# abb128/april-asr

Measured on AMD Instinct MI355X. Metric: audio_seconds_per_second (concurrent 16 kHz sessions x 1/RTF), aprilv0_en-us-sized streaming RNN-T, higher is better.
Workload: dtype f32

## Files before the change

### april_asr_amd/__init__.py

```python
import ctypes as C
import math
import struct
import weakref
from enum import IntEnum
from typing import Callable, List, Sequence

import numpy as np

from . import _ffi

__all__ = ["Result", "Token", "Model", "Session", "SessionGroup", "Bias", "Lm", "lm_info", "VadEvent", "resampler_taps", "decode_host", "vad_plan", "vad_host", "vad_events_host",
           "DtmfEvent", "dtmf_plan", "dtmf_tables", "dtmf_host", "dtmf_decide_host", "dtmf_events_host",
           "ToneEvent", "tone_plan", "tone_tables", "tone_host", "tone_decide_host", "tone_events_host", "tone_name",
           "snapshot_info"]


class Result(IntEnum):
    PARTIAL_RECOGNITION = 1
    FINAL_RECOGNITION = 2
    ERROR_CANT_KEEP_UP = 3
    SILENCE = 4


class VadEvent:
# ... 350 lines not shown
        k = len(rows_list)
        opts = (_ffi.AprilxVadOptions * k)(*[_vad_options(o) for o in options])
        n = np.array([len(r) for r in rows_list], np.int32)
        fr = np.zeros(k, np.int32) if first_row is None else np.ascontiguousarray(first_row, np.int32)
        rows = np.ascontiguousarray(np.concatenate([np.asarray(r, np.float32).reshape(len(r), -1) for r in rows_list]), np.float32)
        assert rows.shape[1] == self.dims.mel
        st = (_ffi.AprilxVadState * k)(*(states if states is not None else [vad_reset_state() for _ in range(k)]))
        b = np.zeros(int(n.sum()), np.uint8); e = np.zeros(int(n.sum()), np.float32)
        rc = self._L.aprilx_run_vad(self._handle, k, C.addressof(opts), n.ctypes.data, fr.ctypes.data, rows.ctypes.data, C.addressof(st), b.ctypes.data, e.ctypes.data)
        if rc != 0:
            raise ValueError("aprilx_run_vad refused its arguments")
        cuts = np.cumsum(n)[:-1]
        return np.split(b, cuts), np.split(e, cuts), [st[i] for i in range(k)]

    def run_dtmf(self, options, frames_list, powers: bool = True):
        k = len(frames_list)
        opts = (_ffi.AprilxDtmfOptions * k)(*[_dtmf_options(o) for o in options])
        n = np.array([len(f) for f in frames_list], np.int32)
        fr = np.ascontiguousarray(np.concatenate([np.asarray(f, np.int16).reshape(len(f), -1) for f in frames_list]), np.int16)
        codes = np.zeros(int(n.sum()), np.uint8); pw = np.zeros((int(n.sum()), 9), np.float32)
        if self._L.aprilx_run_dtmf(self._handle, C.addressof(opts), k, n.ctypes.data, fr.ctypes.data, codes.ctypes.data, pw.ctypes.data if powers else None) != 0:
            raise ValueError("aprilx_run_dtmf refused its arguments")
        cuts = np.cumsum(n)[:-1]
        return np.split(codes, cuts), np.split(pw, cuts)

    def run_dtmf_decide(self, options, powers9):
        q = np.ascontiguousarray(powers9, np.float32).reshape(-1, 9)
        codes = np.zeros(len(q), np.uint8)
        if self._L.aprilx_run_dtmf_decide(self._handle, C.byref(_dtmf_options(options)), len(q), q.ctypes.data, codes.ctypes.data) != 0:
            raise ValueError("aprilx_run_dtmf_decide refused its arguments")
        return codes

    def run_tones(self, options, frames_list, powers: bool = True):
        k = len(frames_list)
        opts = (_ffi.AprilxToneOptions * k)(*[_tone_options(o) for o in options])
        n = np.array([len(f) for f in frames_list], np.int32)
        fr = np.ascontiguousarray(np.concatenate([np.asarray(f, np.int16).reshape(len(f), -1) for f in frames_list]), np.int16)
        plan = tone_plan(self.dims.sample_rate, self.dims.fft_size, max(1, self.dims.frame_shift * 1000 // self.dims.sample_rate), options[0])
        rec = np.zeros((int(n.sum()), 2), np.uint16); pw = np.zeros((int(n.sum()), plan.F + 1), np.float32)
        if self._L.aprilx_run_tones(self._handle, C.addressof(opts), k, n.ctypes.data, fr.ctypes.data, rec.ctypes.data, pw.ctypes.data if powers else None) != 0:
            raise ValueError("aprilx_run_tones refused its arguments")
        cuts = np.cumsum(n)[:-1]
        return np.split(rec, cuts), np.split(pw, cuts)

    def run_tone_decide(self, options, powers):
        q = np.ascontiguousarray(powers, np.float32)
        q = q.reshape(len(q), -1)
        rec = np.zeros((len(q), 2), np.uint16)
        if self._L.aprilx_run_tone_decide(self._handle, C.byref(_tone_options(options)), len(q), q.ctypes.data, rec.ctypes.data) != 0:
            raise ValueError("aprilx_run_tone_decide refused its arguments")
        return rec

    def tone_stats(self, device_index: int = 0):
        return self._detector_stats(self._L.aprilx_model_tone_stats, device_index)

    def _detector_stats(self, entry, device_index):
        l, f, ms = C.c_uint64(0), C.c_uint64(0), C.c_double(0)
        if entry(self._handle, device_index, C.byref(l), C.byref(f), C.byref(ms)) != 0:
            raise ValueError("no such device")
        return int(l.value), int(f.value), float(ms.value)

    def dtmf_stats(self, device_index: int = 0):
        return self._detector_stats(self._L.aprilx_model_dtmf_stats, device_index)

    def vad_stats(self, device_index: int = 0):
        return self._detector_stats(self._L.aprilx_model_vad_stats, device_index)

    def snapshot_stats(self, device_index: int = 0):
        g, s, gm, sm = C.c_uint64(0), C.c_uint64(0), C.c_double(0), C.c_double(0)
        if self._L.aprilx_model_snapshot_stats(self._handle, device_index, C.byref(g), C.byref(s), C.byref(gm), C.byref(sm)) != 0:
            raise ValueError("no such device")
        return int(g.value), int(s.value), float(gm.value), float(sm.value)

    def stats(self, device_index: int = 0):
        s = _ffi.AprilxStats()
        self._L.aprilx_model_stats(self._handle, device_index, C.byref(s))
        return s

    def ramp_stats(self, device_index: int = 0):
        h, e = C.c_uint64(0), C.c_uint64(0)
        if self._L.aprilx_model_ramp_stats(self._handle, device_index, C.byref(h), C.byref(e)) != 0:
            raise ValueError("aprilx_model_ramp_stats refused the call")
        return int(h.value), int(e.value)

    def feed_latencies(self, device_index: int = 0, reset: bool = False) -> np.ndarray:
        n = int(self._L.aprilx_model_feed_latency(self._handle, device_index, None, 0, 0))
        out = np.zeros(n, np.float64)
        if n:
            n = int(self._L.aprilx_model_feed_latency(self._handle, device_index, out.ctypes.data, n, 1 if reset else 0))
        elif reset:
            self._L.aprilx_model_feed_latency(self._handle, device_index, None, 0, 1)
        return out[:n]

    def profile(self, enable):
        self._L.aprilx_model_profile(self._handle, int(enable))


BIAS_STRICT = 1


class Bias:

    def __init__(self, model: Model, phrases, boost: float = 2.0, flags: int = 0):
        self._L = model._L
        items = [(p, boost) if isinstance(p, (str, bytes)) else (p[0], p[1]) for p in phrases]
        raw = [p.encode("utf-8") if isinstance(p, str) else bytes(p) for p, _ in items]
        arr = (C.c_char_p * max(len(raw), 1))(*raw)
        boosts = (C.c_float * max(len(raw), 1))(*[float(b) for _, b in items])
        err = C.create_string_buffer(256)
        self._handle = self._L.aprilx_bias_create_ex(model._handle, len(raw), arr, boosts, int(flags), err, 256)
        self.message = err.value.decode("utf-8", "replace")
        if not self._handle:
            raise ValueError("bias set refused: " + self.message)
        st, ed = C.c_int32(0), C.c_int64(0)
        self.dropped = int(self._L.aprilx_bias_info(self._handle, C.byref(st), C.byref(ed)))
        self.states, self.n_edges = int(st.value), int(ed.value)
        self.flags = int(self._L.aprilx_bias_flags(self._handle))
        self.strict = bool(self.flags & BIAS_STRICT)

    def edges(self, state: int):
        n = int(self._L.aprilx_bias_edges(self._handle, int(state), None, None, None, 0))
        if n < 0:
            raise ValueError("no state %d" % state)
        tok = np.zeros(n, np.int32); nxt = np.zeros(n, np.int32); bonus = np.zeros(n, np.float32)
        if n:
            assert self._L.aprilx_bias_edges(self._handle, int(state), tok.ctypes.data, nxt.ctypes.data, bonus.ctypes.data, n) == n
        return tok, nxt, bonus

    def csr(self):
        parts = [self.edges(s) for s in range(self.states)]
        off = np.zeros(self.states + 1, np.int32)
        off[1:] = np.cumsum([p[0].size for p in parts])
        return (off,) + tuple(np.concatenate([p[i] for p in parts]) if parts else np.zeros(0) for i in range(3))

    def close(self):
        if getattr(self, "_handle", None):
            self._L.aprilx_bias_free(self._handle)
            self._handle = None

    def __del__(self):
        try:
            self.close()
        except Exception:
            pass


class Lm:

    def __init__(self, model: Model, text, order: int = 5):
        self._L = model._L
        raw = text.encode("utf-8") if isinstance(text, str) else bytes(text)
        err = C.create_string_buffer(256)
        self._handle = self._L.aprilx_lm_create(model._handle, raw, len(raw), int(order), err, 256)
        self.message = err.value.decode("utf-8", "replace")
        if not self._handle:
            raise ValueError("language model refused: " + self.message)
        for k, v in lm_info(self).items():
            setattr(self, k, v)

    def arrays(self):
        nn, na = self.nodes, self.arcs
        d = dict(node_off=np.zeros(nn + 1, np.int32), back=np.zeros(nn, np.int32), bow=np.zeros(nn, np.float32),
                 arc_byte=np.zeros(na, np.uint8), arc_logp=np.zeros(na, np.float32), arc_next=np.zeros(na, np.int32))
        unk = C.c_float(0)
        rc = self._L.aprilx_lm_arrays(self._handle, *[d[k].ctypes.data for k in ("node_off", "back", "bow", "arc_byte", "arc_logp", "arc_next")], C.byref(unk), nn, na)
        assert rc == 0
# ... 647 lines not shown
```

### april_asr_amd/_ffi.py

```python
import ctypes as C
import os

_HERE = os.path.dirname(os.path.abspath(__file__))
LIB_PATH = os.environ.get("APRIL_ASR_LIB") or os.path.join(_HERE, "libaprilasr.so")


class AprilSpeakerID(C.Structure):
    _fields_ = [("data", C.c_uint8 * 16)]


class AprilToken(C.Structure):
    _fields_ = [("token", C.c_char_p), ("logprob", C.c_float), ("flags", C.c_int),
                ("time_ms", C.c_size_t), ("reserved", C.c_void_p)]


HANDLER = C.CFUNCTYPE(None, C.c_void_p, C.c_int, C.c_size_t, C.POINTER(AprilToken))


class AprilConfig(C.Structure):
    _fields_ = [("speaker", AprilSpeakerID), ("handler", HANDLER), ("userdata", C.c_void_p), ("flags", C.c_int)]


class AprilxDims(C.Structure):
    _fields_ = [(n, C.c_int32) for n in ("n_layers", "d_model", "hidden", "ffn", "joiner", "vocab", "mel", "seg",
# ... 50 lines not shown
VAD_HANDLER = C.CFUNCTYPE(None, C.c_void_p, C.c_int, C.c_uint64)


class AprilxDtmfOptions(C.Structure):
    _fields_ = [("size", C.c_uint32), ("min_level_dbfs", C.c_float), ("twist_hi_db", C.c_float), ("twist_lo_db", C.c_float), ("rel_peak_db", C.c_float),
                ("min_share", C.c_float), ("min_tone_ms", C.c_uint32), ("min_pause_ms", C.c_uint32), ("flags", C.c_uint32)]


class AprilxDtmfInfo(C.Structure):
    _fields_ = [("Wd", C.c_int32), ("on_frames", C.c_int32), ("off_frames", C.c_int32), ("held", C.c_uint32),
                ("frames_seen", C.c_uint64), ("tone_frames", C.c_uint64), ("digits", C.c_uint64)]


class AprilxDtmfPlan(C.Structure):
    _fields_ = [("Wd", C.c_int32), ("half_w", C.c_float), ("min_power", C.c_float), ("twist_hi", C.c_float), ("twist_lo", C.c_float),
                ("rel_peak", C.c_float), ("min_share", C.c_float), ("on_frames", C.c_int32), ("off_frames", C.c_int32), ("reserved", C.c_int32)]


class AprilxDtmfMachine(C.Structure):
    _fields_ = [("held", C.c_int32), ("cand", C.c_int32), ("run", C.c_int32)]


DTMF_HANDLER = C.CFUNCTYPE(None, C.c_void_p, C.c_int, C.c_char, C.c_uint64)


class AprilxToneOptions(C.Structure):
    _fields_ = [("size", C.c_uint32), ("min_level_dbfs", C.c_float), ("second_db", C.c_float), ("min_share", C.c_float), ("tol_hz", C.c_uint32),
                ("min_tone_ms", C.c_uint32), ("min_pause_ms", C.c_uint32), ("flags", C.c_uint32)]


class AprilxToneInfo(C.Structure):
    _fields_ = [("W", C.c_int32), ("k_lo", C.c_int32), ("F", C.c_int32), ("on_frames", C.c_int32), ("off_frames", C.c_int32),
                ("held_f1", C.c_uint32), ("held_f2", C.c_uint32), ("reserved", C.c_uint32),
                ("frames_seen", C.c_uint64), ("tonal_frames", C.c_uint64), ("tones", C.c_uint64)]


class AprilxTonePlan(C.Structure):
    _fields_ = [("W", C.c_int32), ("k_lo", C.c_int32), ("F", C.c_int32), ("half_w", C.c_float), ("min_power", C.c_float), ("second_ratio", C.c_float),
                ("min_share", C.c_float), ("bin_hz", C.c_float), ("tol_hz", C.c_int32), ("on_frames", C.c_int32), ("off_frames", C.c_int32),
                ("reserved", C.c_int32)]


class AprilxToneMachine(C.Structure):
    _fields_ = [("held", C.c_int32), ("h1", C.c_int32), ("h2", C.c_int32), ("c1", C.c_int32), ("c2", C.c_int32), ("run", C.c_int32)]


TONE_HANDLER = C.CFUNCTYPE(None, C.c_void_p, C.c_int, C.c_uint32, C.c_uint32, C.c_uint64)


class AprilxInputFormat(C.Structure):
    _fields_ = [("size", C.c_uint32), ("encoding", C.c_uint32), ("channels", C.c_uint32), ("channel", C.c_int32)]


class AprilxSnapshotInfo(C.Structure):
    _fields_ = ([("size", C.c_uint32), ("version", C.c_uint32), ("blob_size", C.c_uint64), ("params_hash", C.c_uint64), ("token_hash", C.c_uint64),
                 ("bias_hash", C.c_uint64), ("bias_edges", C.c_int64), ("chunks", C.c_uint64), ("frames_seen", C.c_uint64), ("now_ms", C.c_uint64),
                 ("rows_written", C.c_uint64)]
                + [(n, C.c_int32) for n in ("n_layers", "d_model", "hidden", "ffn", "joiner", "vocab", "mel", "segment_size", "segment_step", "sample_rate",
                                            "frame_shift_ms", "blank_id")]
                + [(n, C.c_uint32) for n in ("precision", "f16_tile", "input_rate", "confidence_k", "has_format", "has_search_options", "has_vad", "has_dtmf",
                                             "has_tones", "has_bias", "bias_flags")]
                + [("bias_states", C.c_int32), ("ring_rows", C.c_uint32), ("reserved", C.c_uint32), ("format", AprilxInputFormat), ("search", AprilxSearchOptions),
                   ("vad", AprilxVadOptions), ("dtmf", AprilxDtmfOptions), ("tones", AprilxToneOptions), ("name", C.c_char * 64), ("description", C.c_char * 128)])


EXPORTED_REFERENCE_SYMBOLS = [
    "aam_api_init", "aam_create_model", "aam_get_name", "aam_get_description", "aam_get_language",
    "aam_get_sample_rate", "aam_free", "aas_create_session", "aas_feed_pcm16", "aas_flush",
    "aas_realtime_get_speedup", "aas_free",
]
EXPORTED_ENGINE_SYMBOLS = [
    "aprilx_model_dims", "aprilx_model_token", "aprilx_model_blob_size", "aprilx_model_export_blob",
    "aprilx_model_from_blob", "aprilx_model_save_blob", "aprilx_model_save_blob_f16", "aprilx_model_load_blob",
    "aprilx_broadcast_get_id", "aprilx_model_broadcast", "aprilx_model_load_info", "aprilx_feed_many", "aprilx_flush_many", "aprilx_session_drain", "aprilx_feed_many_pipelined", "aprilx_drain_many",
    "aprilx_run_encoder", "aprilx_run_decoder", "aprilx_run_joiner", "aprilx_run_fbank", "aprilx_run_decide", "aprilx_plan_gemm", "aprilx_gemm_plan_debug", "aprilx_run_gemm", "aprilx_stream_form",
    "aprilx_session_trace_logits", "aprilx_session_chunks", "aprilx_session_read_frames", "aprilx_session_context", "aprilx_model_stats", "aprilx_model_profile", "aprilx_model_feed_latency",
    "aprilx_greedy_create", "aprilx_greedy_step", "aprilx_greedy_finish", "aprilx_greedy_free", "aprilx_probe_file", "aprilx_model_load_host", "aprilx_model_fbank_tables", "aprilx_counting_handler",
    "aprilx_session_set_input_rate", "aprilx_session_input_rate", "aprilx_resampler_taps", "aprilx_resample",
    "aprilx_session_set_confidence", "aprilx_session_confidence", "aprilx_run_confidence",
    "aprilx_bias_create", "aprilx_bias_free", "aprilx_bias_info", "aprilx_bias_edges", "aprilx_session_set_bias", "aprilx_session_bias_state",
    "aprilx_run_decide_biased", "aprilx_greedy_set_bias", "aprilx_greedy_bias_state",
    "aprilx_bias_create_ex", "aprilx_bias_flags", "aprilx_run_confidence_biased",
    "aprilx_session_set_search_options", "aprilx_session_search_options", "aprilx_run_decide_opts", "aprilx_greedy_set_search_options",
    "aprilx_ramp_window", "aprilx_model_ramp_stats",
    "aprilx_session_set_input_format", "aprilx_session_input_format", "aprilx_session_feed_bytes", "aprilx_feed_many_bytes",
    "aprilx_decode_host", "aprilx_decode", "aprilx_model_decode_stats",
    "aprilx_session_set_vad", "aprilx_session_vad", "aprilx_vad_plan_tables", "aprilx_vad_host", "aprilx_vad_events_host", "aprilx_run_vad",
    "aprilx_model_vad_stats",
    "aprilx_session_set_dtmf", "aprilx_session_dtmf", "aprilx_dtmf_plan", "aprilx_dtmf_tables", "aprilx_dtmf_host", "aprilx_dtmf_decide_host",
    "aprilx_dtmf_events_host", "aprilx_run_dtmf", "aprilx_run_dtmf_decide", "aprilx_model_dtmf_stats",
    "aprilx_session_set_tones", "aprilx_session_tones", "aprilx_tone_plan", "aprilx_tone_tables", "aprilx_tone_host", "aprilx_tone_decide_host",
    "aprilx_tone_events_host", "aprilx_tone_name", "aprilx_run_tones", "aprilx_run_tone_decide", "aprilx_model_tone_stats",
    "aprilx_session_snapshot", "aprilx_session_restore", "aprilx_snapshot_info", "aprilx_snapshot_many", "aprilx_restore_many", "aprilx_model_snapshot_stats",
    "aprilx_lm_create", "aprilx_lm_free", "aprilx_lm_info", "aprilx_lm_arrays", "aprilx_lm_score_host", "aprilx_session_set_lm", "aprilx_session_lm_state",
    "aprilx_greedy_set_lm", "aprilx_greedy_lm_state", "aprilx_model_lm_stats", "aprilx_run_decide_lm", "aprilx_run_confidence_lm",
]

_lib = None
_inited = False


def lib():
    global _lib
    if _lib is not None:
        return _lib
    if not os.path.exists(LIB_PATH):
        raise ImportError("libaprilasr.so is not built: run `python -c 'import __graft_entry__ as g; g.build()'` "
                          "or `make -C april_asr_amd/csrc` (hipcc, gfx950). There is no CPU fallback.")
    L = C.CDLL(LIB_PATH)
    vp, sz = C.c_void_p, C.c_size_t
    L.aam_api_init.argtypes = [C.c_int]; L.aam_api_init.restype = None
    L.aam_create_model.argtypes = [C.c_char_p]; L.aam_create_model.restype = vp
    for f in ("aam_get_name", "aam_get_description", "aam_get_language"):
        getattr(L, f).argtypes = [vp]; getattr(L, f).restype = C.c_char_p
    L.aam_get_sample_rate.argtypes = [vp]; L.aam_get_sample_rate.restype = sz
    L.aam_free.argtypes = [vp]; L.aam_free.restype = None
    L.aas_create_session.argtypes = [vp, AprilConfig]; L.aas_create_session.restype = vp
    L.aas_feed_pcm16.argtypes = [vp, vp, sz]; L.aas_feed_pcm16.restype = None
    L.aas_flush.argtypes = [vp]; L.aas_flush.restype = None
    L.aas_realtime_get_speedup.argtypes = [vp]; L.aas_realtime_get_speedup.restype = C.c_float
    L.aas_free.argtypes = [vp]; L.aas_free.restype = None
    L.aprilx_model_dims.argtypes = [vp, C.POINTER(AprilxDims)]; L.aprilx_model_dims.restype = C.c_int
    L.aprilx_model_token.argtypes = [vp, C.c_int32]; L.aprilx_model_token.restype = C.c_char_p
    L.aprilx_model_blob_size.argtypes = [vp]; L.aprilx_model_blob_size.restype = sz
    L.aprilx_model_export_blob.argtypes = [vp, vp, sz]; L.aprilx_model_export_blob.restype = C.c_int
    L.aprilx_model_from_blob.argtypes = [vp, sz, C.c_int]; L.aprilx_model_from_blob.restype = vp
    L.aprilx_model_save_blob.argtypes = [vp, C.c_char_p]; L.aprilx_model_save_blob.restype = C.c_int
    L.aprilx_model_save_blob_f16.argtypes = [vp, C.c_char_p]; L.aprilx_model_save_blob_f16.restype = C.c_int
    L.aprilx_model_load_blob.argtypes = [C.c_char_p]; L.aprilx_model_load_blob.restype = vp
    L.aprilx_broadcast_get_id.argtypes = [vp, sz]; L.aprilx_broadcast_get_id.restype = C.c_int
    L.aprilx_model_broadcast.argtypes = [vp, C.c_int, C.c_int, vp]; L.aprilx_model_broadcast.restype = vp
    L.aprilx_model_load_info.argtypes = [vp, C.POINTER(AprilxLoadInfo)]; L.aprilx_model_load_info.restype = C.c_int
    L.aprilx_feed_many.argtypes = [sz, C.POINTER(vp), C.POINTER(vp), C.POINTER(sz)]; L.aprilx_feed_many.restype = None
    L.aprilx_flush_many.argtypes = [sz, C.POINTER(vp)]; L.aprilx_flush_many.restype = None
    L.aprilx_session_drain.argtypes = [vp]; L.aprilx_session_drain.restype = None
    L.aprilx_feed_many_pipelined.argtypes = [sz, C.POINTER(vp), C.POINTER(vp), C.POINTER(sz), C.c_int]; L.aprilx_feed_many_pipelined.restype = None
    L.aprilx_drain_many.argtypes = [sz, C.POINTER(vp)]; L.aprilx_drain_many.restype = None
    L.aprilx_run_encoder.argtypes = [vp, C.c_int] + [vp] * 6; L.aprilx_run_encoder.restype = C.c_int
    L.aprilx_run_decoder.argtypes = [vp, C.c_int, vp, vp]; L.aprilx_run_decoder.restype = C.c_int
    L.aprilx_run_joiner.argtypes = [vp, C.c_int, vp, vp, vp]; L.aprilx_run_joiner.restype = C.c_int
    L.aprilx_run_fbank.argtypes = [vp, C.c_int, vp, vp]; L.aprilx_run_fbank.restype = C.c_int
    L.aprilx_plan_gemm.argtypes = [C.c_int] * 6 + [vp]; L.aprilx_plan_gemm.restype = C.c_int
    L.aprilx_gemm_plan_debug.argtypes = [vp, vp]; L.aprilx_gemm_plan_debug.restype = C.c_int
    L.aprilx_run_gemm.argtypes = [vp] * 5; L.aprilx_run_gemm.restype = C.c_int
    L.aprilx_ramp_window.argtypes = [C.c_int] * 3 + [vp, C.c_int]; L.aprilx_ramp_window.restype = C.c_int
    L.aprilx_model_ramp_stats.argtypes = [vp, C.c_int, C.POINTER(C.c_uint64), C.POINTER(C.c_uint64)]; L.aprilx_model_ramp_stats.restype = C.c_int
    L.aprilx_stream_form.argtypes = [C.c_int] * 6; L.aprilx_stream_form.restype = C.c_int
    L.aprilx_run_decide.argtypes = [vp, C.c_int, C.c_int, vp, C.c_float, vp, C.c_int, vp, vp]; L.aprilx_run_decide.restype = C.c_int
    L.aprilx_session_trace_logits.argtypes = [vp, vp, sz, C.POINTER(sz)]; L.aprilx_session_trace_logits.restype = None
    L.aprilx_session_chunks.argtypes = [vp]; L.aprilx_session_chunks.restype = C.c_uint64
    L.aprilx_session_read_frames.argtypes = [vp, C.c_uint64, C.c_int, C.c_void_p]; L.aprilx_session_read_frames.restype = C.c_uint64
    L.aprilx_session_context.argtypes = [vp, vp, vp]; L.aprilx_session_context.restype = None
    L.aprilx_model_stats.argtypes = [vp, C.c_int, C.POINTER(AprilxStats)]; L.aprilx_model_stats.restype = None
    L.aprilx_model_feed_latency.argtypes = [vp, C.c_int, vp, C.c_int, C.c_int]; L.aprilx_model_feed_latency.restype = C.c_int
    L.aprilx_model_profile.argtypes = [vp, C.c_int]; L.aprilx_model_profile.restype = None
    L.aprilx_greedy_create.argtypes = [vp, HANDLER, vp]; L.aprilx_greedy_create.restype = vp
    L.aprilx_greedy_step.argtypes = [vp, C.c_int32, C.c_float, C.c_float, C.c_float, sz, C.POINTER(C.c_int32)]
    L.aprilx_greedy_step.restype = C.c_int
    L.aprilx_greedy_finish.argtypes = [vp]; L.aprilx_greedy_finish.restype = None
    L.aprilx_greedy_free.argtypes = [vp]; L.aprilx_greedy_free.restype = None
    L.aprilx_model_load_host.argtypes = [C.c_char_p]; L.aprilx_model_load_host.restype = vp
    L.aprilx_model_fbank_tables.argtypes = [vp, vp, vp]; L.aprilx_model_fbank_tables.restype = C.c_int
    L.aprilx_probe_file.argtypes = [C.c_char_p, C.c_char_p, sz]; L.aprilx_probe_file.restype = C.c_int
    L.aprilx_session_set_input_rate.argtypes = [vp, C.c_uint32]; L.aprilx_session_set_input_rate.restype = C.c_int
    L.aprilx_session_input_rate.argtypes = [vp]; L.aprilx_session_input_rate.restype = C.c_uint32
    L.aprilx_resampler_taps.argtypes = [C.c_uint32, C.c_uint32, vp, vp, sz]; L.aprilx_resampler_taps.restype = C.c_int
    L.aprilx_resample.argtypes = [vp, C.c_uint32, vp, sz, vp, sz]; L.aprilx_resample.restype = C.c_int64
    L.aprilx_session_set_confidence.argtypes = [vp, C.c_int]; L.aprilx_session_set_confidence.restype = C.c_int
    L.aprilx_session_confidence.argtypes = [vp]; L.aprilx_session_confidence.restype = C.c_int
    L.aprilx_run_confidence.argtypes = [vp, C.c_int, vp, C.c_int, vp]; L.aprilx_run_confidence.restype = C.c_int
    L.aprilx_bias_create.argtypes = [vp, sz, C.POINTER(C.c_char_p), C.POINTER(C.c_float), C.c_char_p, sz]; L.aprilx_bias_create.restype = vp
    L.aprilx_bias_create_ex.argtypes = [vp, sz, C.POINTER(C.c_char_p), C.POINTER(C.c_float), C.c_uint32, C.c_char_p, sz]; L.aprilx_bias_create_ex.restype = vp
    L.aprilx_bias_flags.argtypes = [vp]; L.aprilx_bias_flags.restype = C.c_int
    L.aprilx_run_confidence_biased.argtypes = [vp, C.c_int, vp, C.c_int, vp, vp, vp]; L.aprilx_run_confidence_biased.restype = C.c_int
    L.aprilx_bias_free.argtypes = [vp]; L.aprilx_bias_free.restype = None
    L.aprilx_lm_create.argtypes = [vp, vp, sz, C.c_int, C.c_char_p, sz]; L.aprilx_lm_create.restype = vp
    L.aprilx_lm_free.argtypes = [vp]; L.aprilx_lm_free.restype = None
    L.aprilx_lm_info.argtypes = [vp, C.POINTER(C.c_int32), C.POINTER(C.c_int32), C.POINTER(C.c_int64), C.POINTER(C.c_int32), C.POINTER(C.c_int32)]; L.aprilx_lm_info.restype = C.c_int
    L.aprilx_lm_arrays.argtypes = [vp] * 7 + [C.POINTER(C.c_float), sz, sz]; L.aprilx_lm_arrays.restype = C.c_int
    L.aprilx_lm_score_host.argtypes = [vp, C.c_int32, C.c_int32, C.POINTER(C.c_float), C.POINTER(C.c_int32)]; L.aprilx_lm_score_host.restype = C.c_int
    L.aprilx_session_set_lm.argtypes = [vp, vp, C.c_float, C.c_float]; L.aprilx_session_set_lm.restype = C.c_int
    L.aprilx_session_lm_state.argtypes = [vp, C.POINTER(C.c_int32), C.POINTER(C.c_int32)]; L.aprilx_session_lm_state.restype = C.c_int
    L.aprilx_greedy_set_lm.argtypes = [vp, vp, C.c_float, C.c_float]; L.aprilx_greedy_set_lm.restype = C.c_int
    L.aprilx_greedy_lm_state.argtypes = [vp]; L.aprilx_greedy_lm_state.restype = C.c_int
    L.aprilx_model_lm_stats.argtypes = [vp, C.c_int, C.POINTER(C.c_uint64), C.POINTER(C.c_int32), C.POINTER(C.c_uint64)]; L.aprilx_model_lm_stats.restype = C.c_int
    L.aprilx_run_decide_lm.argtypes = [vp, C.c_int, C.c_int, vp, C.c_float, vp, C.c_int, vp, vp, vp, vp, vp, vp, vp, C.c_float, C.c_float]; L.aprilx_run_decide_lm.restype = C.c_int
    L.aprilx_run_confidence_lm.argtypes = [vp, C.c_int, vp, C.c_int, vp, vp, vp, vp, C.c_float, C.c_float, vp]; L.aprilx_run_confidence_lm.restype = C.c_int
    L.aprilx_bias_info.argtypes = [vp, C.POINTER(C.c_int32), C.POINTER(C.c_int64)]; L.aprilx_bias_info.restype = C.c_int
    L.aprilx_bias_edges.argtypes = [vp, C.c_int32, vp, vp, vp, sz]; L.aprilx_bias_edges.restype = C.c_int
    L.aprilx_session_set_bias.argtypes = [vp, vp]; L.aprilx_session_set_bias.restype = C.c_int
    L.aprilx_session_bias_state.argtypes = [vp, C.POINTER(C.c_int32), C.POINTER(C.c_int32)]; L.aprilx_session_bias_state.restype = C.c_int
    L.aprilx_run_decide_biased.argtypes = [vp, C.c_int, C.c_int, vp, C.c_float, vp, C.c_int, vp, vp, vp, vp]; L.aprilx_run_decide_biased.restype = C.c_int
    L.aprilx_greedy_set_bias.argtypes = [vp, vp]; L.aprilx_greedy_set_bias.restype = C.c_int
    L.aprilx_greedy_bias_state.argtypes = [vp]; L.aprilx_greedy_bias_state.restype = C.c_int
    L.aprilx_session_set_search_options.argtypes = [vp, C.POINTER(AprilxSearchOptions)]; L.aprilx_session_set_search_options.restype = C.c_int
    L.aprilx_session_search_options.argtypes = [vp, C.POINTER(AprilxSearchOptions)]; L.aprilx_session_search_options.restype = C.c_int
    L.aprilx_run_decide_opts.argtypes = [vp, C.c_int, C.c_int, vp, C.c_float, vp, C.c_int, vp, vp, vp, vp, vp]; L.aprilx_run_decide_opts.restype = C.c_int
    L.aprilx_greedy_set_search_options.argtypes = [vp, C.POINTER(AprilxSearchOptions)]; L.aprilx_greedy_set_search_options.restype = C.c_int
    L.aprilx_session_set_input_format.argtypes = [vp, C.POINTER(AprilxInputFormat)]; L.aprilx_session_set_input_format.restype = C.c_int
    L.aprilx_session_input_format.argtypes = [vp, C.POINTER(AprilxInputFormat)]; L.aprilx_session_input_format.restype = C.c_int
    L.aprilx_session_feed_bytes.argtypes = [vp, vp, sz]; L.aprilx_session_feed_bytes.restype = C.c_int
    L.aprilx_feed_many_bytes.argtypes = [sz, C.POINTER(vp), C.POINTER(vp), C.POINTER(sz), C.c_int]; L.aprilx_feed_many_bytes.restype = C.c_int
    L.aprilx_decode_host.argtypes = [C.POINTER(AprilxInputFormat), vp, sz, vp, sz]; L.aprilx_decode_host.restype = C.c_int64
    L.aprilx_decode.argtypes = [vp, C.POINTER(AprilxInputFormat), vp, sz, vp, sz]; L.aprilx_decode.restype = C.c_int64
    L.aprilx_model_decode_stats.argtypes = [vp, C.c_int, C.POINTER(C.c_uint64), C.POINTER(C.c_uint64), C.POINTER(C.c_double)]; L.aprilx_model_decode_stats.restype = C.c_int
    L.aprilx_session_set_vad.argtypes = [vp, C.POINTER(AprilxVadOptions), VAD_HANDLER, vp]; L.aprilx_session_set_vad.restype = C.c_int
    L.aprilx_session_vad.argtypes = [vp, C.POINTER(AprilxVadOptions), C.POINTER(AprilxVadInfo)]; L.aprilx_session_vad.restype = C.c_int
    L.aprilx_vad_plan_tables.argtypes = [vp, C.c_int, C.c_int, C.c_int, C.c_int, C.POINTER(AprilxVadOptions), C.POINTER(AprilxVadPlan)]; L.aprilx_vad_plan_tables.restype = C.c_int
    L.aprilx_vad_host.argtypes = [C.POINTER(AprilxVadPlan), C.c_int, C.c_int, vp, C.POINTER(AprilxVadState), vp, vp]; L.aprilx_vad_host.restype = C.c_int
    L.aprilx_vad_events_host.argtypes = [C.POINTER(AprilxVadPlan), C.c_int, C.c_uint64, vp, sz, C.POINTER(C.c_int32), vp, vp, C.c_int]; L.aprilx_vad_events_host.restype = C.c_int
    L.aprilx_run_vad.argtypes = [vp, C.c_int, vp, vp, vp, vp, vp, vp, vp]; L.aprilx_run_vad.restype = C.c_int
    L.aprilx_model_vad_stats.argtypes = [vp, C.c_int, C.POINTER(C.c_uint64), C.POINTER(C.c_uint64), C.POINTER(C.c_double)]; L.aprilx_model_vad_stats.restype = C.c_int
    L.aprilx_session_set_dtmf.argtypes = [vp, C.POINTER(AprilxDtmfOptions), DTMF_HANDLER, vp]; L.aprilx_session_set_dtmf.restype = C.c_int
    L.aprilx_session_dtmf.argtypes = [vp, C.POINTER(AprilxDtmfOptions), C.POINTER(AprilxDtmfInfo)]; L.aprilx_session_dtmf.restype = C.c_int
    L.aprilx_dtmf_plan.argtypes = [C.c_int, C.c_int, C.c_int, C.POINTER(AprilxDtmfOptions), C.POINTER(AprilxDtmfPlan)]; L.aprilx_dtmf_plan.restype = C.c_int
    L.aprilx_dtmf_tables.argtypes = [C.c_int, C.c_int, vp, sz]; L.aprilx_dtmf_tables.restype = C.c_int
    L.aprilx_dtmf_host.argtypes = [C.POINTER(AprilxDtmfPlan), vp, C.c_int, vp, sz, vp, vp]; L.aprilx_dtmf_host.restype = C.c_int
    L.aprilx_dtmf_decide_host.argtypes = [C.POINTER(AprilxDtmfPlan), vp]; L.aprilx_dtmf_decide_host.restype = C.c_int
    L.aprilx_dtmf_events_host.argtypes = [C.POINTER(AprilxDtmfPlan), C.c_int, C.c_uint64, vp, sz, C.c_int, C.POINTER(AprilxDtmfMachine), vp, vp, vp, C.c_int]
    L.aprilx_dtmf_events_host.restype = C.c_int
    L.aprilx_run_dtmf.argtypes = [vp, vp, C.c_int, vp, vp, vp, vp]; L.aprilx_run_dtmf.restype = C.c_int
    L.aprilx_run_dtmf_decide.argtypes = [vp, C.POINTER(AprilxDtmfOptions), C.c_int, vp, vp]; L.aprilx_run_dtmf_decide.restype = C.c_int
    L.aprilx_model_dtmf_stats.argtypes = [vp, C.c_int, C.POINTER(C.c_uint64), C.POINTER(C.c_uint64), C.POINTER(C.c_double)]; L.aprilx_model_dtmf_stats.restype = C.c_int
    L.aprilx_session_set_tones.argtypes = [vp, C.POINTER(AprilxToneOptions), TONE_HANDLER, vp]; L.aprilx_session_set_tones.restype = C.c_int
    L.aprilx_session_tones.argtypes = [vp, C.POINTER(AprilxToneOptions), C.POINTER(AprilxToneInfo)]; L.aprilx_session_tones.restype = C.c_int
    L.aprilx_tone_plan.argtypes = [C.c_int, C.c_int, C.c_int, C.POINTER(AprilxToneOptions), C.POINTER(AprilxTonePlan)]; L.aprilx_tone_plan.restype = C.c_int
    L.aprilx_tone_tables.argtypes = [C.c_int, C.c_int, vp, sz]; L.aprilx_tone_tables.restype = C.c_int
    L.aprilx_tone_host.argtypes = [C.POINTER(AprilxTonePlan), vp, C.c_int, vp, sz, vp, vp]; L.aprilx_tone_host.restype = C.c_int
    L.aprilx_tone_decide_host.argtypes = [C.POINTER(AprilxTonePlan), vp]; L.aprilx_tone_decide_host.restype = C.c_int64
# ... 25 lines not shown
```

### april_asr_amd/csrc/engine.cc

```cpp
#include "engine.h"
#include <array>
#include <algorithm>
#include <cmath>
#include <chrono>
#include <cstdlib>
#include <cstring>
#include "common.h"
#include "env.h"
#include "rowepi_forms.h"

namespace aprilx {

static size_t align64(size_t x) { return (x + 63) & ~(size_t)63; }

void plan_layout(const NetDims &d, bool has_dec_conv_b, PackedLayout &L)
{
    L.dims = d;
    L.has_dec_conv_b = has_dec_conv_b;
    L.vocab_pad = (d.vocab + 31) & ~31;
    size_t off = 0;
    auto take = [&](size_t n) { size_t o = off; off = align64(off + n); return o; };
    L.k3 = (d.conv_ch[1] * 9 + 63) & ~63;
    L.conv_w[0] = take((size_t)d.conv_ch[0] * 9); L.conv_b[0] = take((size_t)d.conv_ch[0]);
    L.conv_w[1] = take((size_t)d.conv_ch[1] * d.conv_ch[0] * 9); L.conv_b[1] = take((size_t)d.conv_ch[1]);
    L.conv_w[2] = take((size_t)L.k3 * d.conv_ch[2]); L.conv_b[2] = take((size_t)d.conv_ch[2]);
    L.w_embed = take((size_t)d.embed_in * d.d_model); L.b_embed = take((size_t)d.d_model);
    L.layers.resize((size_t)d.n_layers);
    for (auto &l : L.layers) {
        l.wg = take((size_t)2 * d.d_model * 4 * d.hidden); l.bg = take((size_t)4 * d.hidden);
        l.whr = take((size_t)d.hidden * d.d_model);
        l.wff1 = take((size_t)d.d_model * d.ffn); l.bff1 = take((size_t)d.ffn);
        l.wff2 = take((size_t)d.ffn * d.d_model); l.bff2 = take((size_t)d.d_model);
    }
    L.w_encproj = take((size_t)d.d_model * d.joiner); L.b_encproj = take((size_t)d.joiner);
    L.emb = take((size_t)d.vocab * d.d_model);
    L.dec_conv = take((size_t)d.d_model * (d.d_model / d.dec_groups) * d.context);
    L.dec_conv_b = take((size_t)d.d_model);
    L.w_decproj = take((size_t)d.d_model * d.joiner); L.b_decproj = take((size_t)d.joiner);
    L.w_out = take((size_t)d.joiner * L.vocab_pad); L.b_out = take((size_t)L.vocab_pad);
    L.total = off;
}

std::vector<std::pair<size_t, size_t>> gemm_sections(const PackedLayout &L)
{
    const NetDims &d = L.dims;
    std::vector<std::pair<size_t, size_t>> v;
    v.emplace_back(L.w_embed, (size_t)d.embed_in * d.d_model);
    for (const PackedLayout::Layer &o : L.layers) {
        v.emplace_back(o.wg, (size_t)2 * d.d_model * 4 * d.hidden); v.emplace_back(o.whr, (size_t)d.hidden * d.d_model);
        v.emplace_back(o.wff1, (size_t)d.d_model * d.ffn); v.emplace_back(o.wff2, (size_t)d.ffn * d.d_model);
    }
    v.emplace_back(L.w_encproj, (size_t)d.d_model * d.joiner); v.emplace_back(L.w_decproj, (size_t)d.d_model * d.joiner);
    v.emplace_back(L.w_out, (size_t)d.joiner * L.vocab_pad);
    return v;
}

static void pack_mfma(const float *W, int K, int N, int Npad, const std::vector<int> *colmap, float *dst)
{
    const int KB = K / 16, NTt = Npad / 16;
    for (int t = 0; t < NTt; ++t)
        for (int kb = 0; kb < KB; ++kb)
            for (int lane = 0; lane < 64; ++lane) {
                const int np = t * 16 + (lane & 15);
                const int src = np < N ? (colmap ? (*colmap)[(size_t)np] : np) : -1;
                float *o = dst + (((size_t)t * KB + kb) * 64 + lane) * 4;
                for (int j = 0; j < 4; ++j) {
                    const int k = kb * 16 + (lane >> 4) * 4 + j;
                    o[j] = src >= 0 ? W[(size_t)k * N + src] : 0.0f;
                }
            }
}

void pack_weights(const HostModel &m, PackedLayout &L, std::vector<float> &blob)
{
    const NetDims &d = L.dims;
    blob.assign(L.total, 0.0f);
    float *B = blob.data();
    for (int i = 0; i < 3; ++i) {
        if (i < 2) memcpy(B + L.conv_w[i], m.conv_w[i].data(), m.conv_w[i].size() * 4);
        memcpy(B + L.conv_b[i], m.conv_b[i].data(), m.conv_b[i].size() * 4);
    }
    {
        const int kreal = d.conv_ch[1] * 9, c2 = d.conv_ch[2];
        std::vector<float> w3((size_t)L.k3 * c2, 0.0f);
        for (int o = 0; o < c2; ++o) for (int k = 0; k < kreal; ++k) w3[(size_t)k * c2 + o] = m.conv_w[2][(size_t)o * kreal + k];
        pack_mfma(w3.data(), L.k3, c2, c2, nullptr, B + L.conv_w[2]);
    }
    {
        const int c2 = d.conv_ch[2], F = d.f_out;
// ... 88 lines not shown
    HIP_CHECK(hipStreamCreateWithFlags(&s_stream_, hipStreamNonBlocking));
    search_stream_ = stream_;
    for (int i = 0; i < 32; ++i) { hipEvent_t e; HIP_CHECK(hipEventCreateWithFlags(&e, hipEventDisableTiming)); join_ev_.push_back(e); }
    split_streams_ = std::max(0, std::min(2, env_int("APRIL_SPLIT_STREAMS", 2)));
    const NetDims &d = L_.dims;
    w_ = dmalloc<float>(L_.total);
    if (blob_device) HIP_CHECK(hipMemcpy(w_, blob_device, L_.total * 4, hipMemcpyDeviceToDevice));
    else if (blob_host) HIP_CHECK(hipMemcpy(w_, blob_host, L_.total * 4, hipMemcpyHostToDevice));

    const size_t S = (size_t)cfg_.max_slots, MB = (size_t)cfg_.max_batch;
    ring_frames_ = std::max(P_.segment_size * 32, env_int("APRIL_RING_FRAMES", 8192));
    h_ = dmalloc<float>((size_t)d.n_layers * S * d.d_model);
    c_ = dmalloc<float>((size_t)d.n_layers * S * d.hidden);
    if (!env_str("APRIL_RING_FRAMES")) {
        size_t free_b = 0, total_b = 0;
        if (hipMemGetInfo(&free_b, &total_b) == hipSuccess && free_b > 0) {
            const size_t per_frame = S * (size_t)d.mel * sizeof(float);
            const size_t fit = (free_b / 4) / per_frame;
            if (fit < (size_t)ring_frames_) {
                const int shrunk = std::max(P_.segment_size * 32, (int)std::min<size_t>(fit, 8192) / 64 * 64);
                LOGW("engine: %zu MB of feature rings (%d frames x %zu slots) exceed a quarter of the %zu MB free on device %d: %d frames per session",
                     per_frame * (size_t)ring_frames_ >> 20, ring_frames_, S, free_b >> 20, cfg_.device, shrunk);
                ring_frames_ = shrunk;
            }
        } else (void)hipGetLastError();
        float *p = nullptr;
        if (hipMalloc((void **)&p, S * ring_frames_ * d.mel * sizeof(float)) == hipSuccess) ring_ = p;
        else {
            (void)hipGetLastError();
            const size_t asked = S * (size_t)ring_frames_ * d.mel * sizeof(float);
            ring_frames_ = std::max(P_.segment_size * 32, 2048);
            LOGW("engine: no room for %zu MB of feature rings, falling back to %d frames per session", asked >> 20, ring_frames_);
        }
    }
    if (!ring_) ring_ = dmalloc<float>(S * ring_frames_ * d.mel);
    eout_ = dmalloc<float>(S * d.joiner);
    dout_ = dmalloc<float>(S * d.joiner);
    gstate_ = dmalloc<GreedyState>(S);
    HIP_CHECK(hipMemset(h_, 0, (size_t)d.n_layers * S * d.d_model * 4));
    HIP_CHECK(hipMemset(c_, 0, (size_t)d.n_layers * S * d.hidden * 4));
    HIP_CHECK(hipMemset(ring_, 0, S * ring_frames_ * d.mel * 4));
    HIP_CHECK(hipMemset(eout_, 0, S * d.joiner * 4));
    HIP_CHECK(hipMemset(dout_, 0, S * d.joiner * 4));
    {
        std::vector<GreedyState> init(S);
        for (auto &g : init) { g.ctx0 = P_.blank_id; g.ctx1 = P_.blank_id; g.last_tok = -1; g.last_emit_ms = 0; }
        HIP_CHECK(hipMemcpy(gstate_, init.data(), S * sizeof(GreedyState), hipMemcpyHostToDevice));
    }
    cls_ = dmalloc<uint8_t>((size_t)d.vocab);
    HIP_CHECK(hipMemcpy(cls_, tok_class.data(), (size_t)d.vocab, hipMemcpyHostToDevice));

    kz_embed_ = pick_kz(d.embed_in, d.d_model);
    kz_hr_ = pick_kz(d.hidden, d.d_model);
    kz_ff2_ = pick_kz(d.ffn, d.d_model);
    kz_proj_ = pick_kz(d.d_model, d.joiner);
    kz_out_ = pick_kz(d.joiner, L_.vocab_pad);
    {
        const bool want = cfg_.precision == 1 && env_int("APRIL_F16_TILE", 1) != 0;
        f16_tile_ = want && d.d_model % 128 == 0 && d.hidden % 128 == 0 && d.ffn % 128 == 0 && d.hidden % 16 == 0;
        if (f16_tile_) {
            kzx_hr_ = pick_kz(d.hidden, d.d_model, 32); kzx_ff2_ = pick_kz(d.ffn, d.d_model, 32);
            for (int p = 0; p < 2; ++p) y16_buf_[p] = dmalloc<uint16_t>(MB * d.d_model);
            y16_ = y16_buf_[0];
            for (int p = 0; p < 2; ++p) { xb16_buf_[p] = dmalloc<uint16_t>(MB * d.d_model); u16_buf_[p] = dmalloc<uint16_t>(MB * d.hidden); ff16_buf_[p] = dmalloc<uint16_t>(MB * d.ffn); }
            xb16_ = xb16_buf_[0]; u16_ = u16_buf_[0]; ff16_ = ff16_buf_[0];
            h16_ = dmalloc<uint16_t>((size_t)d.n_layers * S * d.d_model);
            HIP_CHECK(hipMemset(h16_, 0, (size_t)d.n_layers * S * d.d_model * 2));
        }
    }
    ws_mstride_ = cfg_.max_batch;
    const size_t ws_n = (size_t)std::max({kz_embed_ * d.d_model, kz_hr_ * d.d_model, kz_ff2_ * d.d_model, kz_proj_ * d.joiner, kz_out_ * L_.vocab_pad});
    ws_ = dmalloc<float>(ws_n * MB);
    ws_g_ = dmalloc<float>((size_t)std::max(kz_proj_ * d.joiner, kz_out_ * L_.vocab_pad) * MB);
    xin_ = dmalloc<float>(MB * d.embed_in);
    a3_ = dmalloc<float>(MB * d.f_out * L_.k3);
    HIP_CHECK(hipMemset(a3_, 0, MB * d.f_out * L_.k3 * 4));
    for (int p = 0; p < 2; ++p) { y_buf_[p] = dmalloc<float>(MB * d.d_model); ssq_buf_[p] = dmalloc<float>(MB * (d.d_model / SSQ_COLS)); }
    y_ = y_buf_[0]; ssq_ = ssq_buf_[0];
    ws_fe_ = dmalloc<float>((size_t)kz_embed_ * d.d_model * MB);
    ws_sr_ = dmalloc<float>((size_t)std::max(kz_proj_ * d.joiner, d.d_model) * MB);
    for (int p = 0; p < 2; ++p) { xb_buf_[p] = dmalloc<float>(MB * d.d_model); u_buf_[p] = dmalloc<float>(MB * d.hidden); ff_buf_[p] = dmalloc<float>(MB * d.ffn); }
    xb_ = xb_buf_[0]; u_ = u_buf_[0]; ff_ = ff_buf_[0];
    ramp_mode_ = env_int("APRIL_RAMP_MERGE", 1);
    if (ramp_mode_ < 0 || ramp_mode_ > 2) ramp_mode_ = 1;
    ramp_d_ = dmalloc<RampState>(1); HIP_CHECK(hipMemset(ramp_d_, 0, sizeof(RampState)));
    de_ = dmalloc<float>(MB * d.d_model);
    HIP_CHECK(hipMemset(de_, 0, MB * d.d_model * 4));
    logits_ = dmalloc<float>(3 * MB * d.vocab);
    logits_h_ = hmalloc<float>(3 * MB * d.vocab);
    ring_cap_ = std::max<size_t>((size_t)1 << 20, 3 * MB * 8 + 2 * S); ring_h_ = hmalloc<int>(2 * ring_cap_);
    step_cap_ = 1 << 14; step_off_h_ = hmalloc<int>((size_t)2 * step_cap_); rec_off_h_ = hmalloc<int>((size_t)2 * step_cap_);
    rec_cap_ = std::max<size_t>((size_t)1 << 20, 3 * MB * 8); rec_d_ = dmalloc<StepRecord>(2 * rec_cap_); rec_h_ = hmalloc<StepRecord>(2 * rec_cap_);
    for (int i = 0; i < 2; ++i) HIP_CHECK(hipEventCreateWithFlags(&flight_done_[i], hipEventDisableTiming));
    counter_d_ = dmalloc<int>(1);
    for (int p = 0; p < 2; ++p) {
        rec_off_buf_[p] = dmalloc<int>(1); flags_buf_[p] = dmalloc<int>(8); step_buf_[p] = dmalloc<int>(4 * MB);
        HIP_CHECK(hipMemset(rec_off_buf_[p], 0, 4)); HIP_CHECK(hipMemset(flags_buf_[p], 0, 32));
    }
    rec_off_d_ = rec_off_buf_[0]; flags_d_ = flags_buf_[0]; step_d_ = step_buf_[0];
    active_d_ = dmalloc<int>(MB); dirty_d_ = dmalloc<int>(MB);
    dec_slots_d_ = dmalloc<int>(std::max(S, MB));
    HIP_CHECK(hipMemset(counter_d_, 0, 4));

    upload_tables(ft);
    use_graphs_ = env_int("APRIL_NO_GRAPHS", 0) == 0;
    if (const int n = env_int("APRIL_GRAPH_CACHE_CAP", 0))
        step_graphs_.cap = lm_graphs_.cap = lm_search_graphs_.cap = sw_plan_cap_ = (size_t)std::max(n, 2), sw_graphs_.cap = 4 * sw_plan_cap_;
    free_.reserve(S);
    for (int i = cfg_.max_slots - 1; i >= 0; --i) free_.push_back(i);
    LOGI("engine: device %d, %d slots, max batch %d, weights %.1f MB, kz(embed,hr,ff2,proj,out)=%d,%d,%d,%d,%d",
         cfg_.device, cfg_.max_slots, cfg_.max_batch, L_.total * 4.0 / 1e6, kz_embed_, kz_hr_, kz_ff2_, kz_proj_, kz_out_);
}

void Engine::finish_weights()
{
    HipLegacyLock legacy;
    HIP_CHECK(hipSetDevice(cfg_.device));
    if (cfg_.precision == 1 && !wh_) {
        wh_ = dmalloc<uint16_t>(L_.total);
        for (const auto &sec : gemm_sections(L_)) launch_cvt_f16(w_ + sec.first, wh_ + sec.first, sec.second, nullptr);
        if (f16_tile_) {
            const NetDims &d = L_.dims;
            wx_ = dmalloc<uint16_t>(L_.total);
            for (const PackedLayout::Layer &o : L_.layers) {
                launch_repack_x32(w_ + o.wg, wx_ + o.wg, 2 * d.d_model, 4 * d.hidden, nullptr);
                launch_repack_x32(w_ + o.whr, wx_ + o.whr, d.hidden, d.d_model, nullptr);
                launch_repack_x32(w_ + o.wff1, wx_ + o.wff1, d.d_model, d.ffn, nullptr);
                launch_repack_x32(w_ + o.wff2, wx_ + o.wff2, d.ffn, d.d_model, nullptr);
            }
        }
        HIP_CHECK(hipDeviceSynchronize());
    }
    if (!conv_wt_) {
        const NetDims &d = L_.dims;
        conv_wt_ = dmalloc<float>((size_t)9 * d.conv_ch[0] + (size_t)9 * d.conv_ch[0] * d.conv_ch[1]);
        launch_conv_weight_transpose(w_ + L_.conv_w[0], w_ + L_.conv_w[1], d.conv_ch[0], d.conv_ch[1], conv_wt_, conv_wt_ + (size_t)9 * d.conv_ch[0], nullptr);
        HIP_CHECK(hipDeviceSynchronize());
    }
    build_dec_table();
}

void Engine::build_dec_table()
{
    if (dec_table_) return;
    const NetDims &d = L_.dims;
    const size_t limit_mb = (size_t)std::max(0, env_int("APRIL_DEC_TABLE_MB", 2048));
    const size_t rows = (size_t)d.vocab * (size_t)d.vocab;
    if (d.context != 2 || rows * (size_t)d.joiner * 4 > limit_mb * 1024 * 1024 || rows * (size_t)d.joiner * 4 >= ((size_t)1 << 32)) return;
    const int MB = cfg_.max_batch;
    float *table = dmalloc<float>(rows * (size_t)d.joiner);
    std::vector<int> iota((size_t)MB), ctx((size_t)MB * 2);
    for (int i = 0; i < MB; ++i) iota[(size_t)i] = i;
    int *ctx_d = dmalloc<int>((size_t)MB * 2);
    HIP_CHECK(hipMemcpy(dec_slots_d_, iota.data(), (size_t)MB * 4, hipMemcpyHostToDevice));
    for (size_t base = 0; base < rows; base += (size_t)MB) {
        const int n = (int)std::min<size_t>((size_t)MB, rows - base);
        for (int i = 0; i < n; ++i) { const size_t r = base + (size_t)i; ctx[(size_t)2 * i] = (int)(r / (size_t)d.vocab); ctx[(size_t)2 * i + 1] = (int)(r % (size_t)d.vocab); }
        HIP_CHECK(hipMemcpy(ctx_d, ctx.data(), (size_t)n * 8, hipMemcpyHostToDevice));
        DecEmbedArgs a; a.dec = dec_params(); a.ctx = ctx_d; a.M = n; a.out = de_; a.ldo = d.d_model;
        launch_dec_embed(a, stream_);
        run_decproj(n, dec_slots_d_, nullptr, nullptr, 1, table + base * (size_t)d.joiner);
        HIP_CHECK(hipStreamSynchronize(stream_));
    }
    (void)hipFree(ctx_d);
    dec_table_ = table;
    LOGI("engine: decoder table %zu rows x %d (%.0f MB)", rows, d.joiner, rows * (double)d.joiner * 4 / 1e6);
}

Engine::~Engine()
{
    HipLegacyLock legacy;
    (void)hipSetDevice(cfg_.device);
    (void)hipStreamSynchronize(f_stream_); (void)hipStreamSynchronize(stream_); (void)hipStreamSynchronize(s_stream_);
    dump_stream_trace();
    if (ramp_d_ && ramp_eligible_.load() > 0) {
        unsigned h = 0;
        if (hipMemcpy(&h, &ramp_d_->hosted, sizeof h, hipMemcpyDeviceToHost) == hipSuccess) LOGI("engine: ramp merge: %u of %llu hostable split feeds were hosted by their predecessor", h, (unsigned long long)ramp_eligible_.load());
    }
    for (StreamTrace &t : trace_) for (hipEvent_t e : t.ev) if (e) (void)hipEventDestroy(e);
    if (trace_base_) (void)hipEventDestroy(trace_base_);
    for (hipEvent_t e : join_ev_) (void)hipEventDestroy(e);
    for (auto &e : ev_pool_) { (void)hipEventDestroy(e.a); (void)hipEventDestroy(e.b); }
    drop_graphs(); free_sw_plans(); if (gclk_slots_) (void)hipFree(gclk_slots_);
    if (lm_stream_) { (void)hipStreamSynchronize(lm_stream_); (void)hipStreamDestroy(lm_stream_); }
    for (hipEvent_t e : lm_events_) (void)hipEventDestroy(e);
    if (zargs_h_) { (void)hipHostFree(zargs_h_); (void)hipFree(zargs_d_); }
    for (int i = 0; i < 3; ++i) if (zargs_done_[i]) (void)hipEventDestroy(zargs_done_[i]);
    for (void *p : {(void *)lm_now_d_, (void *)lm_rows_d_, (void *)lm_rec_off_d_}) if (p) (void)hipFree(p);
    conf_k_.release(); bias_set_.release(); bias_desc_.release(); opt_.release();
    if (conf_d_) (void)hipFree(conf_d_);
    if (conf_h_) (void)hipHostFree(conf_h_);
    for (auto &b : bias_sets_) if (b.dev) (void)hipFree(b.dev);
    if (bias_state_d_) (void)hipFree(bias_state_d_);
    lm_slot_.release(); lm_desc_.release();
    for (auto &e : lm_models_) if (e.dev) (void)hipFree(e.dev);
    if (lm_state_d_) (void)hipFree(lm_state_d_);
    for (void *p : {(void *)vad_state_d_, (void *)pass_out_d_}) if (p) (void)hipFree(p);
    for (PassBlock &k : pass_blocks_) (void)hipHostFree(k.h);
    if (snap_d_) (void)hipFree(snap_d_);
    if (snap_h_) (void)hipHostFree(snap_h_);
    if (ws_g_) (void)hipFree(ws_g_);
    if (conv_wt_) (void)hipFree(conv_wt_);
    if (dec_table_) (void)hipFree(dec_table_);
    if (p_lm_) (void)hipFree(p_lm_);
    for (int p = 0; p < 2; ++p)
        for (void *q : {(void *)eout_lm_buf_[p], (void *)y16_buf_[p], (void *)y_buf_[p], (void *)ssq_buf_[p], (void *)xb_buf_[p], (void *)u_buf_[p], (void *)ff_buf_[p],
                        (void *)xb16_buf_[p], (void *)u16_buf_[p], (void *)ff16_buf_[p], (void *)rec_off_buf_[p], (void *)flags_buf_[p], (void *)step_buf_[p]}) if (q) (void)hipFree(q);
    if (ws_fe_) (void)hipFree(ws_fe_);
    if (ws_sr_) (void)hipFree(ws_sr_);
    for (void *p : {(void *)wx_, (void *)h16_, (void *)ramp_d_}) if (p) (void)hipFree(p);
    for (void *p : {(void *)w_, (void *)wh_, (void *)h_, (void *)c_, (void *)ring_, (void *)eout_, (void *)dout_, (void *)gstate_, (void *)cls_, (void *)ws_, (void *)xin_,
                    (void *)a3_, (void *)de_, (void *)logits_, (void *)rec_d_, (void *)counter_d_,
                    (void *)active_d_, (void *)dirty_d_, (void *)dec_slots_d_,
                    (void *)ds_pcm_[0], (void *)ds_pcm_[1]})
        if (p) (void)hipFree(p);
    for (void *p : {(void *)ring_h_, (void *)step_off_h_, (void *)rec_off_h_, (void *)rec_h_, (void *)logits_h_, (void *)hs_pcm_[0], (void *)hs_pcm_[1]})
        if (p) (void)hipHostFree(p);
    for (int b = 0; b < 2; ++b) if (fb_done_[b]) (void)hipEventDestroy(fb_done_[b]);
    for (int b = 0; b < 2; ++b) if (flight_done_[b]) (void)hipEventDestroy(flight_done_[b]);
    for (void *p : table_allocs_) (void)hipFree(p);
    (void)hipStreamDestroy(stream_); (void)hipStreamDestroy(f_stream_); (void)hipStreamDestroy(s_stream_);
}

void Engine::upload_tables(const FbankHostTables &ft)
{
    auto up = [&](const void *src, size_t bytes) {
        void *p = nullptr;
        HIP_CHECK(hipMalloc(&p, std::max<size_t>(bytes, 16)));
        if (bytes) HIP_CHECK(hipMemcpy(p, src, bytes, hipMemcpyHostToDevice));
        table_allocs_.push_back(p);
        return p;
    };
    ft_.window = (const float *)up(ft.window.data(), ft.window.size() * 4);
    ft_.mel = (const float *)up(ft.mel.data(), ft.mel.size() * 4);
    ft_.mel_lo = (const int *)up(ft.mel_lo.data(), ft.mel_lo.size() * 4);
    ft_.mel_hi = (const int *)up(ft.mel_hi.data(), ft.mel_hi.size() * 4);
    ft_.nfct = (int)ft.factors.size();
    for (int k = 0; k < ft_.nfct; ++k) {
        ft_.fct[k] = ft.factors[(size_t)k];
        ft_.tw[k] = (const double *)up(ft.tw[(size_t)k].data(), ft.tw[(size_t)k].size() * 8);
        ft_.tws[k] = ft.tws[(size_t)k].empty() ? nullptr : (const double *)up(ft.tws[(size_t)k].data(), ft.tws[(size_t)k].size() * 8);
    }
    ft_.padded = ft.padded; ft_.nbins = ft.nbins;
    pad_value_ = ft.pad_value;
}

int Engine::alloc_slot()
{
    std::lock_guard<std::mutex> g(slot_mu_);
    if (free_.empty() && !zero_pending_.empty()) zero_pending_slots();
    if (free_.empty()) return -1;
    const int s = free_.back();
    free_.pop_back();
    ++live_;
    return s;
}

void Engine::zero_pending_slots()
{
    if (zero_pending_.empty()) return;
    if (hipSetDevice(cfg_.device) == hipSuccess) {
        std::lock_guard<std::mutex> cg(capture_mu_);
        m_touched();
        const NetDims &d = L_.dims;
        for (size_t o = 0; o < zero_pending_.size(); o += 64) {
            ZeroSlotArgs z;
            z.h = h_; z.c = c_; z.n_layers = d.n_layers; z.slots = (size_t)cfg_.max_slots; z.d_model = d.d_model; z.hidden = d.hidden;
            z.eout = eout_; z.dout = dout_; z.joiner = d.joiner; z.state = gstate_; z.blank = P_.blank_id; z.h16 = h16_;
            z.n_list = (int)std::min<size_t>(64, zero_pending_.size() - o);
            for (int i = 0; i < z.n_list; ++i) z.list[i] = zero_pending_[o + (size_t)i];
            launch_zero_slot(z, stream_);
        }
    }
    for (int s : zero_pending_) free_.push_back(s);
    zero_pending_.clear();
}

void Engine::free_slot(int slot)
{
    set_slot_confidence(slot, 0); set_slot_bias(slot, nullptr); set_slot_lm(slot, nullptr, 0.0f, 0.0f); set_slot_search_options(slot, SearchOpt{0u, 0.0f});
    std::lock_guard<std::mutex> g(slot_mu_);
    zero_pending_.push_back(slot);
    --live_;
    if (zero_pending_.size() >= 256) zero_pending_slots();
}

void Engine::sync_streams()
{
    HIP_CHECK(hipStreamSynchronize(f_stream_)); HIP_CHECK(hipStreamSynchronize(stream_)); HIP_CHECK(hipStreamSynchronize(s_stream_));
}

void Engine::sync()
{
    m_touched();
    sync_streams();
    f_unseen_by_m_ = s_unseen_by_m_ = m_unseen_by_f_ = m_unseen_by_s_ = false;
    if (profiling_) collect_timing();
}

template <typename Chain> static hipGraphExec_t capture_graph(hipStream_t st, Chain &&chain)
{
    hipGraph_t graph = nullptr;
    hipGraphExec_t exec = nullptr;
    HipLegacyLock capture_guard;
    HIP_CHECK(hipStreamBeginCapture(st, hipStreamCaptureModeRelaxed));
    chain();
    HIP_CHECK(hipStreamEndCapture(st, &graph));
    HIP_CHECK(hipGraphInstantiate(&exec, graph, nullptr, nullptr, 0));
    HIP_CHECK(hipGraphDestroy(graph));
    return exec;
}

void GraphCache::clear()
{
    if (!map_.empty()) LOGI("engine: %s graphs emptied (%zu entries)", name, map_.size());
    for (auto &g : map_) (void)hipGraphExecDestroy(g.second);
    map_.clear(); uses_.clear();
}

template <typename Chain> hipGraphExec_t Engine::cached_graph(GraphCache &cache, const GraphCache::Key &key, hipStream_t st, Chain &&chain)
{
    if (!cache.find(key)) cache.insert(key, capture_graph(st, chain));
    return cache.find(key);
}

template <typename Capture> void Engine::capture_both_parities(Capture &&capture)
{
    const int par = flight_parity_;
    m_touched();
    for (int q : {1 - par, par}) { select_parity(q); capture(); }
}

Engine::StreamTrace *Engine::trace_slot()
{
    static const char *path = env_str("APRIL_STREAM_TRACE");
    if (!path) return nullptr;
    if (!trace_base_) { HIP_CHECK(hipEventCreate(&trace_base_)); HIP_CHECK(hipEventRecord(trace_base_, stream_)); }
    if (trace_.size() >= 4096) return nullptr;
    trace_.emplace_back();
    StreamTrace &t = trace_.back();
    for (hipEvent_t &e : t.ev) HIP_CHECK(hipEventCreate(&e));
    return &t;
}

void Engine::dump_stream_trace()
{
    const char *path = env_str("APRIL_STREAM_TRACE");
    if (!path || trace_.empty()) return;
    FILE *f = fopen(path, "w");
    if (!f) return;
    fprintf(f, "# one line per split feed; times in us since the first split feed; FE = index fetch + conv + embed on stream F, LY = layer wavefront on M, SR = encoder_proj + search on S\n");
    fprintf(f, "# feed sessions chunks  FE_start FE_end  LY_start LY_end  SR_start SR_end   overlap: FE inside the previous feed's LY window? SR inside the next feed's LY window?\n");
    std::vector<std::array<float, 6>> ts;
    for (StreamTrace &t : trace_) {
        std::array<float, 6> a{};
        bool ok = t.used;
        for (int i = 0; i < 6 && ok; ++i) ok = hipEventElapsedTime(&a[(size_t)i], trace_base_, t.ev[i]) == hipSuccess;
        if (ok) ts.push_back(a); else (void)hipGetLastError();
    }
    for (size_t i = 0; i < ts.size(); ++i) {
        const auto &a = ts[i];
        const bool fe_in_prev = i > 0 && a[0] * 1e3f < ts[i - 1][3] * 1e3f && a[1] * 1e3f > ts[i - 1][2] * 1e3f;
        const bool sr_in_next = i + 1 < ts.size() && a[5] > ts[i + 1][2] && a[4] < ts[i + 1][3];
        fprintf(f, "%4zu %5d %2d  %10.1f %10.1f  %10.1f %10.1f  %10.1f %10.1f   %s %s\n", i, trace_[i].m, trace_[i].T, a[0] * 1e3, a[1] * 1e3, a[2] * 1e3, a[3] * 1e3, a[4] * 1e3, a[5] * 1e3,
                fe_in_prev ? "FE<prevLY" : "-", sr_in_next ? "SR<nextLY" : "-");
    }
    fclose(f);
}

void Engine::join(hipStream_t waiter, hipStream_t src)
{
    hipEvent_t e = join_ev_[join_pos_++ % join_ev_.size()];
    HIP_CHECK(hipEventRecord(e, src));
    HIP_CHECK(hipStreamWaitEvent(waiter, e, 0));
}

void Engine::general_prologue()
{
    m_touched();
    if (f_unseen_by_m_) { join(stream_, f_stream_); f_unseen_by_m_ = false; }
    if (s_unseen_by_m_) { join(stream_, s_stream_); s_unseen_by_m_ = false; }
    m_unseen_by_f_ = m_unseen_by_s_ = true;
    flight_tail_s_ = false;
}

void Engine::set_profiling(bool on) { std::lock_guard<std::mutex> cg(capture_mu_); sync(); profiling_ = on; }
void Engine::reset_timing() { for (auto &t : timing_) t = KernelTiming(); }
void Engine::set_gates_clock(bool on)
{
    std::lock_guard<std::mutex> cg(capture_mu_);
    HIP_CHECK(hipSetDevice(cfg_.device));
    sync();
    if (on) {
        if (!gclk_slots_) gclk_slots_ = dmalloc<unsigned long long>((size_t)GCLK_SLOTS * STAMP_WORDS);
        HIP_CHECK(hipMemsetAsync(gclk_slots_, 0, (size_t)GCLK_SLOTS * STAMP_WORDS * 8, stream_));
        HIP_CHECK(hipStreamSynchronize(stream_));
        gclk_ms_ = 0; gclk_launches_ = 0; gclk_rows_ = 0;
        for (int i = 0; i < 4; ++i) { gclk_ms_n_[i] = 0; gclk_launches_n_[i] = 0; }
        gclk_ = true;
        return;
    }
    collect_gates_clock(); gclk_ = false;
}
void Engine::collect_gates_clock()
{
    if (!gclk_ || !gclk_slots_) return;
    std::vector<unsigned long long> h((size_t)GCLK_SLOTS * STAMP_WORDS);
    HIP_CHECK(hipMemcpyAsync(h.data(), gclk_slots_, h.size() * 8, hipMemcpyDeviceToHost, stream_)); HIP_CHECK(hipStreamSynchronize(stream_));
    for (auto &kv : sw_plans_)
        for (size_t i = 0; i < kv.second.stamp_slots.size(); ++i) {
            const auto &sl = kv.second.stamp_slots[i];
            const unsigned long long ticks = h[(size_t)sl.first * STAMP_WORDS + 2], n = h[(size_t)sl.first * STAMP_WORDS + 3];
            gclk_ms_ += (double)ticks * 1e-5; gclk_launches_ += (long)n; gclk_rows_ += (long)n * sl.second;
            const int bn = std::min(std::max(kv.second.stamp_n[i], 1), 4) - 1;
            gclk_ms_n_[bn] += (double)ticks * 1e-5; gclk_launches_n_[bn] += (long)n;
        }
}
void Engine::timed_begin(int cls)
{
    ++launch_count_;
    if (!profiling_) return;
    if (ev_used_ == ev_pool_.size()) { Ev e; HIP_CHECK(hipEventCreate(&e.a)); HIP_CHECK(hipEventCreate(&e.b)); e.cls = cls; ev_pool_.push_back(e); }
    ev_pool_[ev_used_].cls = cls;
    if (cls == T_GATES) gemm_profile_next_launch(ev_pool_[ev_used_].a, ev_pool_[ev_used_].b);
    else HIP_CHECK(hipEventRecord(ev_pool_[ev_used_].a, stream_));
}
void Engine::timed_end(int cls)
{
    if (!profiling_) return;
    if (cls == T_GATES) {
        if (gemm_profile_pending()) { gemm_profile_next_launch(nullptr, nullptr); return; }
    } else HIP_CHECK(hipEventRecord(ev_pool_[ev_used_].b, stream_));
    ++ev_used_;
}
void Engine::collect_timing()
{
    for (size_t i = 0; i < ev_used_; ++i) {
        float ms = 0;
        if (hipEventElapsedTime(&ms, ev_pool_[i].a, ev_pool_[i].b) == hipSuccess) { timing_[ev_pool_[i].cls].ms += ms; timing_[ev_pool_[i].cls].launches++; }
    }
    ev_used_ = 0;
}

const uint8_t *Engine::fbank(int n_frames, const FbankFrameDesc *desc, const std::pair<const int16_t *, size_t> *parts, size_t n_parts, size_t n_pcm, HostPool *pool,
                             const FrontPass &pass)
{
    if (n_frames <= 0) return nullptr;
    const int n_rs = std::max(pass.n_rs, 0), n_dc = std::max(pass.n_dc, 0), n_vd = std::max(pass.n_vd, 0), n_dt = std::max(pass.n_dt, 0);
// ... 530 lines not shown
            zargs_pos_ += items.size(); items.clear();
        };
        auto by_len = [&](auto make) {
            for (int pass = 0; pass < 2; ++pass) {
                for (const Act &x : act) if (((x.t1 - x.t0) == blk) == (pass == 0)) items.push_back(make(x));
                flush();
            }
        };
        by_len([&](const Act &x) { return args_gates(x.l, (size_t)x.t0 * m, (x.t1 - x.t0) * m, GATES_X); });
        for (int i = 0; i < blk; ++i) {
            for (const Act &x : act) if (x.t0 + i < x.t1) items.push_back(args_gates(x.l, (size_t)(x.t0 + i) * m, m, GATES_H));
            flush();
            for (const Act &x : act) if (x.t0 + i < x.t1) items.push_back(args_whr(x.l, (size_t)(x.t0 + i) * m, m));
            flush();
        }
        by_len([&](const Act &x) { return args_ff1(x.l, (size_t)x.t0 * m, (x.t1 - x.t0) * m); });
        by_len([&](const Act &x) { return args_ff2(x.l, (size_t)x.t0 * m, (x.t1 - x.t0) * m); });
        plan_end[(size_t)W] = plan.size();
    }
    lap(0);
    if (zargs_pos_ > first)
        HIP_CHECK(hipMemcpyAsync(zargs_d_ + first, zargs_h_ + first, (zargs_pos_ - first) * sizeof(GemmArgs), hipMemcpyHostToDevice, cs));
    lap(1);
    for (int W = 0; W <= NB + L; ++W) {
        if (W < NB) encoder_front((size_t)W * blk * m, (std::min(T, (W + 1) * blk) - W * blk) * m, step_d_ + 3 * MB, nullptr, cs, ws_);
        lap(2);
        for (size_t k = W ? plan_end[(size_t)W - 1] : 0; k < plan_end[(size_t)W]; ++k) launch_gemm_z(zargs_h_ + plan[k].off, plan[k].n, zargs_d_ + plan[k].off, cs);
        lap(3);
        const int bp = W - L - 1;
        if (bp >= 0) {
            const int t0 = bp * blk, t1 = std::min(T, t0 + blk), len = t1 - t0;
            lm_stage_proj(m, t0, t1, cs, ws_);
            hipEvent_t e = lm_events_[1 + (size_t)(bp % (int)(lm_events_.size() - 1))];
            HIP_CHECK(hipEventRecord(e, cs));
            HIP_CHECK(hipStreamWaitEvent(stream_, e, 0));
            BlockSetupArgs bs;
            bs.now_src = step_d_ + 2 * MB + (size_t)t0 * m; bs.now_dst = lm_now_d_; bs.rows_dst = lm_rows_d_; bs.row0 = t0 * m; bs.count = len * m;
            bs.rec_off_step = rec_off_d_; bs.rec_off_block = lm_rec_off_d_; bs.rec_add = t0 * 3 * m; bs.flags = flags_d_; bs.n_flags = 8;
            launch_block_setup(bs, stream_);
            lap(4);
            auto search = [&]() {
                for (int i = 0; i < len; ++i) {
                    GreedyIo io;
                    io.gen = i + 1; io.now = lm_now_d_ + (size_t)i * m; io.eout = eout_lm_; io.eout_rows = lm_rows_d_ + (size_t)i * m;
                    io.rec_off = lm_rec_off_d_; io.rec_slot0 = i * 3;
                    io.dump = dump_logits ? logits_ + (size_t)(t0 + i) * 3 * m * d.vocab : nullptr;
                    run_greedy_rounds(m, io);
                }
            };
            if (!use_graphs_ || dump_logits) { search(); continue; }
            const GraphCache::Key key = graph_key(m, len);
            if (!lm_search_graphs_.find(key) && lm_search_graphs_.full()) { HIP_CHECK(hipStreamSynchronize(stream_));  lm_search_graphs_.clear(); }
            HIP_CHECK(hipGraphLaunch(cached_graph(lm_search_graphs_, key, stream_, search), stream_));
            lap(5);
        }
    }
    HIP_CHECK(hipEventRecord(zargs_done_[zslot], cs));
    zargs_busy_[zslot] = true;
    if (timing) fprintf(stderr, "lm wavefront %d x %d: host us: args %.0f, arg copy %.0f, front end %.0f, layer launches %.0f, proj + events + setup %.0f, search graph %.0f\n",
                        m, T, tacc[0], tacc[1], tacc[2], tacc[3], tacc[4], tacc[5]);
}

static bool lm_gates_split_on()
{
    static const bool on = env_int("APRIL_GATES_SPLIT", 1) != 0;
    return on;
}

Engine::SwPlan &Engine::sw_plan(int m, int T)
{
    const GraphCache::Key key = sw_key(m, T);
    auto it = sw_plans_.find(key);
    if (it != sw_plans_.end()) return it->second;
    if (sw_plans_.size() >= sw_plan_cap_) {
        sync();
        HipLegacyLock evict_guard;
        collect_gates_clock(); free_sw_plans();
        if (gclk_slots_) { HIP_CHECK(hipMemsetAsync(gclk_slots_, 0, (size_t)GCLK_SLOTS * STAMP_WORDS * 8, stream_)); HIP_CHECK(hipStreamSynchronize(stream_)); }
        gclk_used_ = 0;
    }
    SwPlan &p = sw_plans_[key];
    build_sw_chain(p, p.one, m, T, false);
    if (ramp_mode_ != 0 && !gclk_) build_sw_chain(p, p.split, m, T, true);
    return p;
}

std::vector<RampStep> ramp_window(int L, int T, int R, int max_problems)
{
    std::vector<RampStep> w;
    if (L <= 2 * R || T < 1 || R < 1) return w;
    for (int j = 1; j <= R; ++j) {
        RampStep s; s.macro = L + T - 1 - R + j;
        for (int l = 0; l < L; ++l) { const int t = s.macro - 1 - l; if (t >= 0 && t < T) ++s.own; }
        for (int t = 0; t < j; ++t) s.guests.push_back(std::make_pair(j - 1 - t, t));
        if (s.own + (int)s.guests.size() > max_problems) return std::vector<RampStep>();
        w.push_back(s);
    }
    return w;
}

void Engine::ramp_counts(uint64_t *hosted, uint64_t *eligible)
{
    unsigned h = 0;
    {
        HipLegacyLock legacy;
        if (hipSetDevice(cfg_.device) == hipSuccess) HIP_CHECK(hipMemcpy(&h, &ramp_d_->hosted, sizeof h, hipMemcpyDeviceToHost));
    }
    *hosted = h; *eligible = ramp_eligible_.load(std::memory_order_relaxed);
}

void Engine::build_sw_chain(SwPlan &p, SwPlan::Chain &c, int m, int T, bool ramp)
{
    const NetDims &d = L_.dims;
    const int L = d.n_layers;
    const int par = flight_parity_;
    auto needs_rows = [&](int kind, int n) {
        if (kind != 1 && kind != 3) return 0;
        GemmArgs g = kind == 1 ? args_whr(0, 0, m) : args_ff2(0, 0, m);
        g.force_fullk = 0; g.zcount = n;
        const GemmPlan p = gemm_plan(g);
        return p.mode == GM_TILE && !p.fused ? p.planes : 0;
    };
    std::vector<RampStep> window;
    if (ramp && m <= RAMP_MAX_M && T <= RAMP_MAX_T) {
        window = ramp_window(L, T, RAMP_R);
        for (const RampStep &s : window) if (needs_rows(1, s.own + (int)s.guests.size()) || needs_rows(3, s.own + (int)s.guests.size())) { window.clear(); break; }
    }
    if (ramp) p.hosts = !window.empty();
    std::vector<GemmArgs> items;
    std::vector<RowArgs> rows;
    for (int W = 0; W <= T + L; ++W) {
        const RampStep *host = nullptr; int wj = 0;
        for (size_t j = 0; j < window.size(); ++j) if (window[j].macro == W) { host = &window[j]; wj = (int)j; }
        if (host && wj == 0) { SwPlan::Batch b; b.off = c.host.size(); b.n = 0; b.macro = W; b.kind = 4; b.roff = c.rhost.size(); b.rn = 0; c.batches.push_back(b); }
        for (int kind = 0; kind < 4; ++kind) {
            items.clear(); rows.clear();
            int n_act = 0;
            for (int l = 0; l < L; ++l) { const int t = W - 1 - l; if (t >= 0 && t < T) ++n_act; }
            if (n_act == 0) continue;
            if (host) n_act += (int)host->guests.size();
            const int planes = needs_rows(kind, n_act);
            const bool split = planes > 0;
            auto problem = [&](int l, int t, const int *run_flag) {
                const size_t r0 = (size_t)t * m;
                GemmArgs g = kind == 0 ? args_gates(l, r0, m, GATES_ALL) : kind == 1 ? args_whr(l, r0, m) : kind == 2 ? args_ff1(l, r0, m) : args_ff2(l, r0, m);
                if (kind == 0 && cfg_.precision == 0) g.tile_ok = gates_tile_rows((long)m * n_act) ? 2 : 0;
                if (run_flag) { g.run_flag = run_flag; g.run_gen = 1; }
                if (split) {
                    float *ws = ws_ + r0 * d.d_model;
                    rows.push_back(row_form(g, ws, ws_mstride_, planes));
                    g = partial_form(g, ws, ws_mstride_);
                } else if (f16_tile_) g.force_fullk = 0;
                items.push_back(g);
            };
            for (int l = 0; l < L; ++l) {
                const int t = W - 1 - l;
                if (t < 0 || t >= T) continue;
                problem(l, t, ramp && W <= RAMP_R ? &ramp_d_->head_live[par] : nullptr);
            }
            if (host) {
                select_parity(1 - par);
                for (const auto &lt : host->guests) problem(lt.first, lt.second, &ramp_d_->guest_live[par][wj][lt.second]);
                select_parity(par);
            }
            std::vector<int> groups;
            {
                int left = (int)items.size();
                const bool cut = kind == 0 && cfg_.precision == 0 && left >= 4 && !gates_tile_rows((long)m * n_act) && lm_gates_split_on();
                while (cut && left > 0) { const int take = (left == 4 || left == 2) ? 2 : (left >= 3 ? 3 : left); groups.push_back(take); left -= take; }
                if (groups.empty()) groups.push_back((int)items.size());
            }
            size_t first = 0;
            for (size_t gi = 0; gi < groups.size(); ++gi) {
                const int gn = groups[gi];
                if (kind == 0 && !ramp && gclk_ && gclk_slots_ && gclk_used_ < GCLK_SLOTS) {
                    p.stamp_slots.push_back(std::make_pair(gclk_used_, (long)m * gn)); p.stamp_n.push_back(gn);
                    for (int i = 0; i < gn; ++i) items[first + (size_t)i].stamp = gclk_slots_ + (size_t)gclk_used_ * STAMP_WORDS;
                    ++gclk_used_;
                } else if (kind == 0 && !ramp && gclk_ && gclk_slots_ && !gclk_warned_) {
                    gclk_warned_ = true; LOGW("engine: the gates clock is out of stamp slots (%d): the gates launches of further plans are not timed", GCLK_SLOTS);
                }
                SwPlan::Batch b; b.off = c.host.size(); b.n = gn; b.macro = W; b.kind = kind; b.roff = c.rhost.size(); b.rn = gi == 0 ? (int)rows.size() : 0;
                c.host.resize(c.host.size() + (size_t)gn);
                stage_gemm_z(items.data() + first, gn, c.host.data() + b.off);
                if (gi == 0) c.rhost.insert(c.rhost.end(), rows.begin(), rows.end());
                c.batches.push_back(b);
                first += (size_t)gn;
            }
        }
    }
    m_touched();
    c.dev = dmalloc<GemmArgs>(c.host.size());
    HIP_CHECK(hipMemcpyAsync(c.dev, c.host.data(), c.host.size() * sizeof(GemmArgs), hipMemcpyHostToDevice, stream_));
    if (!c.rhost.empty()) {
        c.rdev = dmalloc<RowArgs>(c.rhost.size());
        HIP_CHECK(hipMemcpyAsync(c.rdev, c.rhost.data(), c.rhost.size() * sizeof(RowArgs), hipMemcpyHostToDevice, stream_));
    }
}

void Engine::free_sw_plans()
{
    if (!sw_plans_.empty()) LOGI("engine: feed wavefront plans emptied (%zu plans)", sw_plans_.size());
    for (auto &p : sw_plans_) for (SwPlan::Chain *c : {&p.second.one, &p.second.split}) { if (c->dev) (void)hipFree(c->dev); if (c->rdev) (void)hipFree(c->rdev); }
    sw_graphs_.clear(); sw_plans_.clear();
}

void Engine::run_sw_chain(int m, int T, bool dump_logits, const SwPlan &p, int part, hipStream_t st)
{
    const NetDims &d = L_.dims;
    const int MB = cfg_.max_batch;
    if (part < 0 || part == 0) {
        launch_advance(advance_args(m, T), st);
        encoder_front(0, m * T, step_d_ + 3 * MB, nullptr, st, part == 0 ? ws_fe_ : ws_);
    }
    if (part < 0 || part == 1) {
        static const int cls_of[4] = {T_GATES, T_GEMM_OTHER, T_GEMM_OTHER, T_GEMM_OTHER};
        const SwPlan::Chain &c = p.layers(part == 1);
        for (size_t bi = 0; bi < c.batches.size(); ++bi) {
            const SwPlan::Batch &b = c.batches[bi];
            if (b.kind == 4) { launch_ramp_latch(ramp_d_, flight_parity_, m, st); continue; }
            timed_begin(cls_of[b.kind]); launch_gemm_z(c.host.data() + b.off, b.n, c.dev + b.off, st); timed_end(cls_of[b.kind]);
            if (b.rn > 0) { timed_begin(T_ROW); launch_row_z(c.rhost.data() + b.roff, b.rn, c.rdev + b.roff, st); timed_end(T_ROW); }
        }
        if (part < 0) lm_stage_proj(m, 0, T, st, ws_);
    }
    if (part < 0 || part == 2) {
        if (part == 2) lm_stage_proj(m, 0, T, st, ws_sr_);
        hipStream_t keep = search_stream_;
        search_stream_ = st;
        for (int t = 0; t < T; ++t) run_greedy_rounds(m, dump_logits, t, eout_lm_ + (size_t)t * m * d.joiner);
        search_stream_ = keep;
    }
}

int Engine::lm_step(int m, int T, const int *slots, const int *ring_tails, const int *now_ms, float *logits_out, int mode)
{
    const int rows = m * T;
    if (m <= 0 || T <= 0 || rows > cfg_.max_batch || !flight_has_room(rows + m, 1)) { LOGE("engine: layer-major step %d x %d does not fit (max batch %d)", m, T, cfg_.max_batch); abort(); }
    HIP_CHECK(hipSetDevice(cfg_.device));
    const NetDims &d = L_.dims;
    if (!p_lm_) {
        p_lm_ = dmalloc<float>((size_t)cfg_.max_batch * 4 * d.hidden);
        for (int p = 0; p < 2; ++p) eout_lm_buf_[p] = dmalloc<float>((size_t)cfg_.max_batch * d.joiner);
        eout_lm_ = eout_lm_buf_[flight_parity_];
    }
    if (!lm_stream_) {
        HIP_CHECK(hipStreamCreateWithFlags(&lm_stream_, hipStreamNonBlocking));
        for (int i = 0; i < 9; ++i) { hipEvent_t e; HIP_CHECK(hipEventCreateWithFlags(&e, hipEventDisableTiming)); lm_events_.push_back(e); }
        for (int i = 0; i < 3; ++i) HIP_CHECK(hipEventCreateWithFlags(&zargs_done_[i], hipEventDisableTiming));
        lm_now_d_ = dmalloc<int>((size_t)cfg_.max_batch); lm_rows_d_ = dmalloc<int>((size_t)cfg_.max_batch); lm_rec_off_d_ = dmalloc<int>(1);
    }
    const int k = stage_step(m, T, slots, ring_tails, now_ms);
    std::lock_guard<std::mutex> cg(capture_mu_);
    mode == 1 ? run_feed_wavefront(m, T, logits_out != nullptr) : run_layer_major(m, T, logits_out != nullptr);
    if (logits_out) read_back_logits(k, rows, logits_out);
    return k;
}

void Engine::run_feed_wavefront(int m, int T, bool dump_logits)
{
    sw_plan(m, T);
    const bool graphs = use_graphs_ && !profiling_ && !dump_logits && (sw_graphs_.find(sw_key(m, T)) || sw_graphs_.find(sw_key(m, T, 1)) || sw_graphs_.use(m, T) >= 2);
    const bool split = graphs && split_streams_ > 0 && overlap_hint_ && flight_steps_ == 1 && !gclk_;
    const hipStream_t on[3] = {split_streams_ >= 2 ? f_stream_ : stream_, stream_, s_stream_};
    if (graphs && !sw_graphs_.find(sw_key(m, T, split ? 1 : 0)))
        capture_both_parities([&]() {
            const SwPlan &pl = sw_plan(m, T);
            if (split) for (int part = 0; part < 3; ++part) cached_graph(sw_graphs_, sw_key(m, T, 1 + part), on[part], [&]() { run_sw_chain(m, T, false, pl, part, on[part]); });
            else cached_graph(sw_graphs_, sw_key(m, T), stream_, [&]() { run_sw_chain(m, T, false, pl, -1, stream_); });
        });
    if (split) { launch_split_feed(m, T, on[0]); return; }
    general_prologue();
    if (graphs) { HIP_CHECK(hipGraphLaunch(sw_graphs_.find(sw_key(m, T)), stream_)); return; }
    launch_count_ = 0; run_sw_chain(m, T, dump_logits, sw_plan(m, T), -1, stream_); kernels_per_step_ = (launch_count_ + 1 + T - 1) / T;
}

void Engine::launch_split_feed(int m, int T, hipStream_t fe)
{
    if (fe == f_stream_) {
        if (m_unseen_by_f_) { join(f_stream_, stream_); m_unseen_by_f_ = false; }
    } else if (f_unseen_by_m_) { join(stream_, f_stream_); f_unseen_by_m_ = false; }
    if (m_unseen_by_s_) { join(s_stream_, stream_); m_unseen_by_s_ = false; }
    StreamTrace *tr = trace_slot();
    auto part = [&](int i, hipStream_t st) {
        if (tr) HIP_CHECK(hipEventRecord(tr->ev[2 * i], st));
        HIP_CHECK(hipGraphLaunch(sw_graphs_.find(sw_key(m, T, 1 + i)), st));
        if (tr) HIP_CHECK(hipEventRecord(tr->ev[2 * i + 1], st));
    };
    part(0, fe);
    if (ramp_mode_ != 0) {
        const bool hostable = ramp_mode_ == 1 && fe == f_stream_ && m_quiet_.load(std::memory_order_acquire);
        if (hostable) ramp_eligible_.fetch_add(1, std::memory_order_relaxed);
        launch_ramp_ready(ramp_d_, flight_parity_, m, T, hostable ? 1 : 0, fe);
    }
    if (fe == f_stream_) { join(stream_, f_stream_); f_unseen_by_m_ = false; }
    part(1, stream_);
    if (ramp_mode_ != 0) m_quiet_.store(true, std::memory_order_release);
    join(s_stream_, stream_); part(2, s_stream_);
    if (tr) { tr->m = m; tr->T = T; tr->used = true; }
    s_unseen_by_m_ = true; flight_tail_s_ = true;
    if (fe != f_stream_) m_unseen_by_f_ = true;
}

void Engine::run_layer_major(int m, int T, bool dump_logits)
{
    general_prologue();
    const bool wavefront = lm_wavefront_on() && !profiling_ && T > LM_WAVEFRONT_MIN_CHUNKS &&
                           gemm_plan(args_whr(0, 0, m)).fused && gemm_plan(args_ff2(0, 0, m)).fused;
    if (wavefront) { run_lm_wavefront(m, T, dump_logits); return; }
    if (!use_graphs_ || profiling_ || dump_logits) { launch_count_ = 0; run_lm_chain(m, T, dump_logits); kernels_per_step_ = launch_count_ + 1; return; }
    const GraphCache::Key key = graph_key(m, T);
    if (!lm_graphs_.find(key) && lm_graphs_.full()) { sync(); lm_graphs_.clear(); }
    HIP_CHECK(hipGraphLaunch(cached_graph(lm_graphs_, key, stream_, [&]() { run_lm_chain(m, T, false); }), stream_));
}

int Engine::stage_step(int m, int T, const int *slots, const int *ring_tails, const int *now_ms)
{
    const size_t rows = (size_t)m * (size_t)std::max(T, 1);
    const int k = next_step_index(); int *blk = ring_h_ + ring_pos_;
    memcpy(blk, slots, (size_t)m * 4); memcpy(blk + m, ring_tails, rows * 4); memcpy(blk + m + rows, now_ms, rows * 4);
    for (int t = 0; t < T; ++t) memcpy(blk + m + 2 * rows + (size_t)t * m, slots, (size_t)m * 4);
    step_off_h_[k] = (int)ring_pos_; rec_off_h_[k] = (int)rec_pos_;
    ring_pos_ += (size_t)m + (T ? 3 : 2) * rows; rec_pos_ += 3 * rows;
    if (conf_k_.on()) note_conf_step(k, slots, m, 3 * rows);
    return k;
}

void Engine::read_back_logits(int k, int rows, float *out)
{
    const size_t n = (size_t)3 * rows * L_.dims.vocab;
    HIP_CHECK(hipMemcpyAsync(logits_h_, logits_, n * 4, hipMemcpyDeviceToHost, stream_));
    HIP_CHECK(hipMemcpyAsync(rec_h_ + rec_off_h_[k], rec_d_ + rec_off_h_[k], (size_t)3 * rows * sizeof(StepRecord), hipMemcpyDeviceToHost, stream_));
    sync();
    memcpy(out, logits_h_, n * 4);
}

void Engine::drop_graphs()
{
    for (GraphCache *c : {&step_graphs_, &lm_graphs_, &lm_search_graphs_, &sw_graphs_}) c->clear();
}

BiasDesc Engine::upload_bias(const BiasSet &set, void **dev, hipStream_t st)
{
    auto pad = [](size_t b) { return (b + 15) & ~(size_t)15; };
    const size_t ns = set.state_off.size() * 4, ne = std::max<size_t>(set.edge_tok.size(), 1) * 4;
    char *p = nullptr;
    HIP_CHECK(hipMalloc((void **)&p, pad(ns) + 3 * pad(ne)));
    BiasDesc d;
    d.state_off = (const int32_t *)p; d.edge_tok = (const int32_t *)(p + pad(ns)); d.edge_next = (const int32_t *)(p + pad(ns) + pad(ne));
    d.edge_bonus = (const float *)(p + pad(ns) + 2 * pad(ne)); d.n_states = set.states(); d.flags = (int32_t)set.flags;
    HIP_CHECK(hipMemcpyAsync((void *)d.state_off, set.state_off.data(), ns, hipMemcpyHostToDevice, st));
    if (!set.edge_tok.empty()) {
        const size_t b = set.edge_tok.size() * 4;
        HIP_CHECK(hipMemcpyAsync((void *)d.edge_tok, set.edge_tok.data(), b, hipMemcpyHostToDevice, st));
        HIP_CHECK(hipMemcpyAsync((void *)d.edge_next, set.edge_next.data(), b, hipMemcpyHostToDevice, st));
        HIP_CHECK(hipMemcpyAsync((void *)d.edge_bonus, set.edge_bonus.data(), b, hipMemcpyHostToDevice, st));
    }
    *dev = p;
    return d;
}

void Engine::apply_slot_tables()
{
    std::lock_guard<std::mutex> bg(bias_q_.mutex());
    const auto bias_todo = bias_q_.take_locked();
    std::lock_guard<std::mutex> lg(lm_q_.mutex());
    const auto lm_todo = lm_q_.take_locked();
    const auto conf_todo = conf_q_.take();
    const auto opt_todo = opt_q_.take();
    const size_t S = (size_t)cfg_.max_slots;
    auto in_range = [S](int slot) { return slot >= 0 && (size_t)slot < S; };
    const bool conf_first = !conf_k_.on() && std::any_of(conf_todo.begin(), conf_todo.end(), [](const std::pair<int, int> &t) { return t.second > 0; });
    const bool bias_first = !bias_set_.on() && std::any_of(bias_todo.begin(), bias_todo.end(), [](const std::pair<int, int> &t) { return t.second >= 0; });
    const bool opt_first = !opt_.on() && std::any_of(opt_todo.begin(), opt_todo.end(), [](const std::pair<int, SearchOpt> &t) { return t.second.endpoint_ms != 0; });
    const bool lm_first = !lm_slot_.on() && std::any_of(lm_todo.begin(), lm_todo.end(), [](const std::pair<int, LmSlot> &t) { return t.second.model >= 0; });
    std::lock_guard<std::mutex> cg(capture_mu_);
    if (conf_first || bias_first || opt_first || lm_first) {
        HipLegacyLock legacy;
        sync();
        drop_graphs();
        if (conf_first) {
            conf_k_.alloc(S, 0);
            conf_d_ = dmalloc<ConfRecord>(2 * rec_cap_); conf_h_ = hmalloc<ConfRecord>(2 * rec_cap_);
            LOGI("engine: confidences on (side ring %.0f MB on the device and pinned)", 2.0 * rec_cap_ * sizeof(ConfRecord) / 1e6);
// ... 66 lines not shown
                lm_desc_.h[i] = LmDesc();
                e.set.reset();
                models = true;
            }
        }
        for (const auto &t : lm_todo) {
            if (!in_range(t.first)) continue;
            lm_slot_.h[t.first] = t.second;
            HIP_CHECK(hipMemcpyAsync(lm_state_d_ + t.first, &lm_slot_.h[t.first].start, 4, hipMemcpyHostToDevice, stream_));
        }
        if (models) lm_desc_.upload(stream_);
        lm_slot_.upload(stream_);
    }
}

LmDesc Engine::upload_lm(const LmSet &set, void **dev, hipStream_t st)
{
    auto pad = [](size_t b) { return (b + 15) & ~(size_t)15; };
    const size_t nn = (size_t)set.nodes(), na = std::max<size_t>((size_t)set.arcs(), 1), nt = std::max<size_t>(set.tok_bytes.size(), 1), nv = set.tok_off.size();
    const size_t sz[8] = {pad((nn + 1) * 4), pad(nn * 4), pad(nn * 4), pad(na * 4), pad(na * 4), pad(na), pad(nv * 4), pad(nt)};
    size_t off[9] = {0};
    for (int i = 0; i < 8; ++i) off[i + 1] = off[i] + sz[i];
    char *p = nullptr;
    HIP_CHECK(hipMalloc((void **)&p, off[8]));
    LmDesc d;
    d.node_off = (const int32_t *)(p + off[0]); d.back = (const int32_t *)(p + off[1]); d.bow = (const float *)(p + off[2]);
    d.arc_logp = (const float *)(p + off[3]); d.arc_next = (const int32_t *)(p + off[4]); d.arc_byte = (const uint8_t *)(p + off[5]);
    d.tok_off = (const int32_t *)(p + off[6]); d.tok_bytes = (const uint8_t *)(p + off[7]);
    d.n_nodes = set.nodes(); d.start = set.start; d.unk_logp = set.unk_logp;
    auto put = [&](const void *dst, const void *src, size_t bytes) { if (bytes) HIP_CHECK(hipMemcpyAsync((void *)dst, src, bytes, hipMemcpyHostToDevice, st)); };
    put(d.node_off, set.node_off.data(), (nn + 1) * 4); put(d.back, set.back.data(), nn * 4); put(d.bow, set.bow.data(), nn * 4);
    put(d.arc_logp, set.arc_logp.data(), set.arc_logp.size() * 4); put(d.arc_next, set.arc_next.data(), set.arc_next.size() * 4); put(d.arc_byte, set.arc_byte.data(), set.arc_byte.size());
    put(d.tok_off, set.tok_off.data(), nv * 4); put(d.tok_bytes, set.tok_bytes.data(), set.tok_bytes.size());
    *dev = p;
    return d;
}

int Engine::read_lm_state(int slot)
{
    if (!lm_q_.ever()) return 0;
    std::lock_guard<std::mutex> lg(lm_q_.mutex());
    if (lm_q_.pending_locked(slot)) { const int i = lm_slot_model_[(size_t)slot]; return i >= 0 ? lm_models_[(size_t)i].set->start : 0; }
    HipLegacyLock legacy;
    HIP_CHECK(hipSetDevice(cfg_.device));
    sync_streams();
    int v = 0;
    if (lm_state_d_) HIP_CHECK(hipMemcpy(&v, lm_state_d_ + slot, 4, hipMemcpyDeviceToHost));
    return v;
}

int Engine::read_bias_state(int slot)
{
    if (!bias_q_.ever()) return 0;
    std::lock_guard<std::mutex> bg(bias_q_.mutex());
    if (bias_q_.pending_locked(slot)) return 0;
    HipLegacyLock legacy;
    HIP_CHECK(hipSetDevice(cfg_.device));
    sync_streams();
    int v = 0;
    if (bias_state_d_) HIP_CHECK(hipMemcpy(&v, bias_state_d_ + slot, 4, hipMemcpyDeviceToHost));
    return v;
}

void Engine::note_conf_step(int k, const int *slots, int m, size_t records)
{
    bool any = false;
    for (int i = 0; i < m && !any; ++i) any = conf_k_.h[slots[i]] != 0;
    if (!any) return;
    const size_t first = (size_t)rec_off_h_[k];
    if (!conf_spans_.empty() && conf_spans_.back().first + conf_spans_.back().second == first) conf_spans_.back().second += records;
    else conf_spans_.push_back(std::make_pair(first, records));
}

void Engine::select_parity(int p)
{
    flight_parity_ = p;
    xb_ = xb_buf_[p]; u_ = u_buf_[p]; ff_ = ff_buf_[p]; xb16_ = xb16_buf_[p]; u16_ = u16_buf_[p]; ff16_ = ff16_buf_[p];
    y_ = y_buf_[p]; ssq_ = ssq_buf_[p]; y16_ = y16_buf_[p]; step_d_ = step_buf_[p]; flags_d_ = flags_buf_[p]; rec_off_d_ = rec_off_buf_[p]; eout_lm_ = eout_lm_buf_[p];
}

void Engine::begin_flight()
{
    HIP_CHECK(hipSetDevice(cfg_.device));
    const int p = flight_parity_ = next_parity_; next_parity_ ^= 1;
    if (flight_open_[p]) { HIP_CHECK(hipEventSynchronize(flight_done_[p])); flight_open_[p] = false; }
    if (conf_q_.has_pending() || bias_q_.has_pending() || opt_q_.has_pending() || lm_q_.has_pending()) apply_slot_tables();
    conf_spans_.clear();
    ring_base_ = (size_t)p * ring_cap_; rec_base_ = (size_t)p * rec_cap_;
    ring_pos_ = ring_base_; rec_pos_ = rec_base_; flight_steps_ = 0;
    select_parity(p);
    flight_tail_s_ = false;
    { std::lock_guard<std::mutex> g(slot_mu_); zero_pending_slots(); }
}

bool Engine::flight_has_room(int rows, int nsteps) const
{
    return flight_steps_ + nsteps <= step_cap_ && ring_pos_ + (size_t)3 * rows + (size_t)cfg_.max_slots <= ring_base_ + ring_cap_ && rec_pos_ + (size_t)3 * rows <= rec_base_ + rec_cap_;
}

int Engine::step(int m, const int *slots, const int *ring_tails, const int *now_ms, float *logits_out)
{
    if (m <= 0 || m > cfg_.max_batch || !flight_has_room(m, 1)) { LOGE("engine: step of %d rows does not fit (max batch %d)", m, cfg_.max_batch); abort(); }
    const int k = stage_step(m, 0, slots, ring_tails, now_ms);
    std::lock_guard<std::mutex> cg(capture_mu_);
    general_prologue();
    const GraphCache::Key key = graph_key(m);
    if (use_graphs_ && !profiling_ && !logits_out && (step_graphs_.find(key) || step_graphs_.use(m) >= 2)) {
        if (!step_graphs_.find(key)) {
            if (step_graphs_.full()) { sync(); step_graphs_.clear(); }
            capture_both_parities([&]() { cached_graph(step_graphs_, graph_key(m), stream_, [&]() { run_chain(m, false); }); });
        }
        HIP_CHECK(hipGraphLaunch(step_graphs_.find(key), stream_));
        return k;
    }
    launch_count_ = 0; run_chain(m, logits_out != nullptr); kernels_per_step_ = launch_count_ + 1;
    if (logits_out) read_back_logits(k, m, logits_out);
    return k;
}

void Engine::decode_rows(int n, const int *slots, int op)
{
    if (n <= 0) return;
    if (dec_table_ && op == 0) return;
    HIP_CHECK(hipSetDevice(cfg_.device));
    const NetDims &d = L_.dims;
    const int MB = cfg_.max_batch;
    std::lock_guard<std::mutex> cg(capture_mu_);
    general_prologue();
    for (int o = 0; o < n; o += MB) {
        const int m = std::min(MB, n - o);
        if (ring_pos_ + (size_t)m > ring_base_ + ring_cap_) { LOGE("engine: index ring exhausted"); abort(); }
        int *blk = ring_h_ + ring_pos_;
        memcpy(blk, slots + o, (size_t)m * 4);
        ring_pos_ += (size_t)m;
        HIP_CHECK(hipMemcpyAsync(dec_slots_d_, blk, (size_t)m * 4, hipMemcpyHostToDevice, stream_));
        DecRowsArgs a; a.slot_idx = dec_slots_d_; a.M = m; a.op = op; a.blank = P_.blank_id; a.state = gstate_; a.dec = dec_params(); a.de_out = dec_table_ ? nullptr : de_; a.ld_de = d.d_model;
        a.bias_state = bias_state_d_;
        a.lm_slot = lm_slot_.d; a.lm_state = lm_state_d_;
        timed_begin(T_DEC); launch_dec_rows(a, stream_); timed_end(T_DEC);
        if (!dec_table_) run_decproj(m, dec_slots_d_, nullptr, nullptr, 1);
    }
}

int Engine::close_flight()
{
    HIP_CHECK(hipSetDevice(cfg_.device));
    std::lock_guard<std::mutex> cg(capture_mu_);
    hipStream_t tail = s_stream_;
    if (!(flight_tail_s_ && s_unseen_by_m_)) {
        tail = stream_;
        if (f_unseen_by_m_) { join(stream_, f_stream_); f_unseen_by_m_ = false; }
        if (s_unseen_by_m_) { join(stream_, s_stream_); s_unseen_by_m_ = false; }
    } else if (pass_bytes_flight_) join(s_stream_, f_stream_);
    pass_bytes_flight_ = false;
    if (rec_pos_ > rec_base_) HIP_CHECK(hipMemcpyAsync(rec_h_ + rec_base_, rec_d_ + rec_base_, (rec_pos_ - rec_base_) * sizeof(StepRecord), hipMemcpyDeviceToHost, tail));
    for (const auto &sp : conf_spans_) {
        HIP_CHECK(hipMemcpyAsync(conf_h_ + sp.first, conf_d_ + sp.first, sp.second * sizeof(ConfRecord), hipMemcpyDeviceToHost, tail));
        conf_copied_.fetch_add(sp.second, std::memory_order_relaxed);
    }
    conf_spans_.clear();
    HIP_CHECK(hipEventRecord(flight_done_[flight_parity_], tail));
    flight_open_[flight_parity_] = true;
    return flight_parity_;
}

bool Engine::flight_done(int parity)
{
    const hipError_t e = hipEventQuery(flight_done_[parity]);
    if (e == hipSuccess) return true;
    if (e != hipErrorNotReady) HIP_CHECK(e);
    (void)hipGetLastError();
    return false;
}

void Engine::wait_flight(int parity)
{
    HIP_CHECK(hipSetDevice(cfg_.device));
    HIP_CHECK(hipEventSynchronize(flight_done_[parity]));
    if (profiling_) sync();
}

void Engine::end_flight() { wait_flight(close_flight()); }

void Engine::zero_slots(int n)
{
    const NetDims &d = L_.dims;
    for (int i = 0; i < n; ++i) {
        ZeroSlotArgs z;
        z.h = h_; z.c = c_; z.n_layers = d.n_layers; z.slots = (size_t)cfg_.max_slots; z.d_model = d.d_model; z.hidden = d.hidden;
        z.eout = eout_; z.dout = dout_; z.joiner = d.joiner; z.state = gstate_; z.blank = P_.blank_id; z.slot = i; z.h16 = h16_;
        launch_zero_slot(z, stream_);
    }
    HIP_CHECK(hipStreamSynchronize(stream_));
}

void Engine::debug_encoder(int n, const float *x, const float *h, const float *c, float *eout, float *h2, float *c2)
{
    std::lock_guard<std::mutex> cg(capture_mu_);
    HipLegacyLock legacy;
    HIP_CHECK(hipSetDevice(cfg_.device));
    const NetDims &d = L_.dims;
    const size_t S = (size_t)cfg_.max_slots;
    if (n > cfg_.max_batch || n > cfg_.max_slots) { LOGE("debug_encoder: n too large"); abort(); }
    std::vector<int> slots((size_t)n);
    for (int i = 0; i < n; ++i) slots[(size_t)i] = i;
    float *xd = dmalloc<float>((size_t)n * d.seg * d.mel);
    HIP_CHECK(hipMemcpy(xd, x, (size_t)n * d.seg * d.mel * 4, hipMemcpyHostToDevice));
    for (int i = 0; i < n; ++i)
        for (int l = 0; l < d.n_layers; ++l) {
            HIP_CHECK(hipMemcpy(h_ + ((size_t)l * S + i) * d.d_model, h + ((size_t)i * d.n_layers + l) * d.d_model, (size_t)d.d_model * 4, hipMemcpyHostToDevice));
            HIP_CHECK(hipMemcpy(c_ + ((size_t)l * S + i) * d.hidden, c + ((size_t)i * d.n_layers + l) * d.hidden, (size_t)d.hidden * 4, hipMemcpyHostToDevice));
        }
    HIP_CHECK(hipMemcpy(step_d_, slots.data(), (size_t)n * 4, hipMemcpyHostToDevice));
    if (f16_tile_)
        for (int l = 0; l < d.n_layers; ++l) launch_cvt_f16(h_ + (size_t)l * S * d.d_model, h16_ + (size_t)l * S * d.d_model, (size_t)n * d.d_model, stream_);
    run_encoder_rows(n, xd);
    sync();
    for (int i = 0; i < n; ++i) {
        HIP_CHECK(hipMemcpy(eout + (size_t)i * d.joiner, eout_ + (size_t)i * d.joiner, (size_t)d.joiner * 4, hipMemcpyDeviceToHost));
        for (int l = 0; l < d.n_layers; ++l) {
            HIP_CHECK(hipMemcpy(h2 + ((size_t)i * d.n_layers + l) * d.d_model, h_ + ((size_t)l * S + i) * d.d_model, (size_t)d.d_model * 4, hipMemcpyDeviceToHost));
            HIP_CHECK(hipMemcpy(c2 + ((size_t)i * d.n_layers + l) * d.hidden, c_ + ((size_t)l * S + i) * d.hidden, (size_t)d.hidden * 4, hipMemcpyDeviceToHost));
        }
    }
    (void)hipFree(xd);
    zero_slots(n);
}

void Engine::debug_decoder(int n, const int64_t *ctx, float *dout)
{
    std::lock_guard<std::mutex> cg(capture_mu_);
    HipLegacyLock legacy;
    HIP_CHECK(hipSetDevice(cfg_.device));
    const NetDims &d = L_.dims;
    if (n > cfg_.max_batch) { LOGE("debug_decoder: n too large"); abort(); }
    if (dec_table_) {
        bool in_range = true;
        for (int i = 0; i < n * 2; ++i) if (ctx[i] < 0 || ctx[i] >= d.vocab) in_range = false;
        if (in_range) {
            sync();
            for (int i = 0; i < n; ++i)
                HIP_CHECK(hipMemcpy(dout + (size_t)i * d.joiner, dec_table_ + ((size_t)ctx[2 * i] * d.vocab + (size_t)ctx[2 * i + 1]) * d.joiner, (size_t)d.joiner * 4, hipMemcpyDeviceToHost));
            return;
        }
    }
    std::vector<int> slots((size_t)n), c32((size_t)n * d.context);
    for (int i = 0; i < n; ++i) { slots[(size_t)i] = i; for (int t = 0; t < d.context; ++t) c32[(size_t)i * d.context + t] = (int)ctx[(size_t)i * d.context + t]; }
    int *ctx_d = dmalloc<int>(c32.size());
    HIP_CHECK(hipMemcpy(ctx_d, c32.data(), c32.size() * 4, hipMemcpyHostToDevice));
    HIP_CHECK(hipMemcpy(dec_slots_d_, slots.data(), (size_t)n * 4, hipMemcpyHostToDevice));
    DecEmbedArgs a; a.dec = dec_params(); a.ctx = ctx_d; a.M = n; a.out = de_; a.ldo = d.d_model;
    launch_dec_embed(a, stream_);
    run_decproj(n, dec_slots_d_, nullptr, nullptr, 1);
    sync();
    HIP_CHECK(hipMemcpy(dout, dout_, (size_t)n * d.joiner * 4, hipMemcpyDeviceToHost));
    (void)hipFree(ctx_d);
    zero_slots(n);
}

void Engine::debug_joiner(int n, const float *eout, const float *dout, float *logits)
// ... 363 lines not shown
```

### april_asr_amd/csrc/engine.h

```cpp
#pragma once
#include <hip/hip_runtime.h>
#include <atomic>
#include <cstdint>
#include <deque>
#include <array>
#include <functional>
#include <map>
#include <memory>
#include <mutex>
#include <string>
#include <utility>
#include <vector>
#include "bias.h"
#include "lm.h"
#include "fbank_tables.h"
#include "resample.h"
#include "input_format.h"
#include "kernels.h"
#include "host_pool.h"
#include "slot_queue.h"
#include "staging_layout.h"
#include "model_loader.h"

namespace aprilx {

struct PackedLayout {
    NetDims dims;
    size_t conv_w[3], conv_b[3];
    int k3 = 0;
    size_t w_embed, b_embed;
    struct Layer { size_t wg, bg, whr, wff1, bff1, wff2, bff2; };
    std::vector<Layer> layers;
    size_t w_encproj, b_encproj, emb, dec_conv, dec_conv_b, w_decproj, b_decproj, w_out, b_out;
    size_t total = 0;
    int vocab_pad = 0;
    bool has_dec_conv_b = false;
    std::vector<float> norm_eps;
    float embed_eps = 0;
};
void plan_layout(const NetDims &d, bool has_dec_conv_b, PackedLayout &L);
std::vector<std::pair<size_t, size_t>> gemm_sections(const PackedLayout &L);
void pack_weights(const HostModel &m, PackedLayout &L, std::vector<float> &blob);

std::recursive_mutex &hip_legacy_mutex();
struct HipLegacyLock { std::lock_guard<std::recursive_mutex> g; HipLegacyLock() : g(hip_legacy_mutex()) {} };

struct EngineConfig {
    int device = 0;
    int max_slots = 4096;
    int max_batch = 2048;
    int precision = 0;
};

struct KernelTiming { double ms = 0; long launches = 0; };

struct GraphCache {
    using Key = std::array<int, 3>;
    const char *name; size_t cap;
    bool full() const { return map_.size() >= cap; }
    hipGraphExec_t find(const Key &k) const { auto it = map_.find(k); return it == map_.end() ? nullptr : it->second; }
    void insert(const Key &k, hipGraphExec_t g) { map_[k] = g; }
    int use(int m, int T = 0) { return ++uses_[std::make_pair(m, T)]; }
    void clear();
    std::map<Key, hipGraphExec_t> map_; std::map<std::pair<int, int>, int> uses_;
};

struct RampStep { int macro = 0, own = 0; std::vector<std::pair<int, int>> guests; };
std::vector<RampStep> ramp_window(int L, int T, int R, int max_problems = 3);

template <typename T> struct DeviceTable {
    T *d = nullptr, *h = nullptr; size_t n = 0;
    bool on() const { return h != nullptr; }
    void alloc(size_t count, const T &off);
    void upload(hipStream_t st) const;
    void release();
};

struct FrontPass {
    int n_rs = 0; ResampleDesc *rs = nullptr; const ResampleSpec *const *rs_specs = nullptr;
    const std::pair<const int16_t *, size_t> *in_parts = nullptr; size_t n_in_parts = 0, n_in = 0;
    int n_dc = 0; const DecodeDesc *dc = nullptr;
    const std::pair<const uint8_t *, size_t> *raw_parts = nullptr; size_t n_raw_parts = 0, n_raw = 0;
    int n_vd = 0; const VadDesc *vd = nullptr; size_t vad_bytes = 0;
    int n_dt = 0; const DtmfDesc *dt = nullptr; size_t dtmf_bytes = 0;
    int n_tn = 0; const ToneDesc *tn = nullptr; size_t tone_bytes = 0;
    size_t tone_at() const { return (vad_bytes + dtmf_bytes + 3) / 4 * 4; }
};

struct DecideRequest {
    int n = 0, op = 0;
    const float *logits = nullptr;
    float early_emit = 1.0f; const int *now_ms = nullptr ; int round = 0;
    int32_t *state_io = nullptr;
    StepRecord *rec_out = nullptr;
    const BiasSet *set = nullptr; int32_t *bias_state_io = nullptr;
    const SearchOpt *opts = nullptr;
    const LmSet *lm = nullptr; int32_t *lm_state_io = nullptr; float lm_weight = 0.0f, lm_bonus = 0.0f;
    int conf_k = 0; ConfRecord *conf_out = nullptr;
    static DecideRequest round_of(int n, int op, const float *logits, float early_emit, const int32_t *now_ms, int round, int32_t *state_io, void *records_out)
    {
        DecideRequest q;
        q.n = n; q.op = op; q.logits = logits; q.early_emit = early_emit; q.now_ms = (const int *)now_ms; q.round = round; q.state_io = state_io; q.rec_out = (StepRecord *)records_out;
// ... 75 lines not shown
            if (!set) return true;
            bias_slot_set_.assign((size_t)cfg_.max_slots, -1); bias_sets_.resize(kBiasSets);
        }
        int idx = -1;
        if (set) {
            if (set->vocab != L_.dims.vocab || set->vocab > kBiasMaxVocab) return false;
            for (int i = 0; i < kBiasSets && idx < 0; ++i) if (bias_sets_[(size_t)i].set == set) idx = i;
            for (int i = 0; i < kBiasSets && idx < 0; ++i) if (!bias_sets_[(size_t)i].set) idx = i;
            if (idx < 0) return false;
            bias_sets_[(size_t)idx].set = set;
            ++bias_sets_[(size_t)idx].users;
        }
        const int old = bias_slot_set_[(size_t)slot];
        if (old < 0 && idx < 0) return true;
        if (old >= 0) --bias_sets_[(size_t)old].users;
        bias_slot_set_[(size_t)slot] = idx;
        bias_q_.push_locked(slot, idx, idx >= 0);
        return true;
    }
    int read_bias_state(int slot);
    bool set_slot_lm(int slot, const std::shared_ptr<const LmSet> &set, float weight, float token_bonus)
    {
        std::lock_guard<std::mutex> g(lm_q_.mutex());
        if (slot < 0 || slot >= cfg_.max_slots) return false;
        if (lm_slot_model_.empty()) {
            if (!set) return true;
            lm_slot_model_.assign((size_t)cfg_.max_slots, -1); lm_models_.resize(kLmModels);
        }
        int idx = -1;
        if (set) {
            if (set->vocab != L_.dims.vocab || set->vocab > kLmMaxVocab) return false;
            for (int i = 0; i < kLmModels && idx < 0; ++i) if (lm_models_[(size_t)i].set == set) idx = i;
            for (int i = 0; i < kLmModels && idx < 0; ++i) if (!lm_models_[(size_t)i].set) idx = i;
            if (idx < 0) return false;
            lm_models_[(size_t)idx].set = set;
            ++lm_models_[(size_t)idx].users;
        }
        const int old = lm_slot_model_[(size_t)slot];
        if (old < 0 && idx < 0) return true;
        if (old >= 0) --lm_models_[(size_t)old].users;
        lm_slot_model_[(size_t)slot] = idx;
        lm_q_.push_locked(slot, LmSlot{idx, idx >= 0 ? weight : 0.0f, idx >= 0 ? token_bonus : 0.0f, set ? set->start : 0}, idx >= 0);
        return true;
    }
    int read_lm_state(int slot);
    void lm_counts(uint64_t *launches, int32_t *resident, uint64_t *uploads) const
    {
        *launches = lm_launches_.load(std::memory_order_relaxed); *resident = lm_resident_.load(std::memory_order_relaxed); *uploads = lm_uploads_.load(std::memory_order_relaxed);
    }
    void set_slot_search_options(int slot, SearchOpt o) { opt_q_.push(slot, o, o.endpoint_ms != 0); }
    void sync();
    void sync_streams();

    void debug_encoder(int n, const float *x, const float *h, const float *c, float *eout, float *h2, float *c2);
    void debug_decoder(int n, const int64_t *ctx, float *dout);
    void debug_joiner(int n, const float *eout, const float *dout, float *logits);
    void debug_decide(const DecideRequest &q);
    void debug_fbank(int n_frames, const int16_t *pcm_frames , float *out );
    void debug_resample(const ResampleSpec *spec, const int16_t *pcm, size_t n, int16_t *out);
    void debug_decode(uint32_t encoding, uint32_t channels, int32_t channel, const void *data, size_t n_frames, int16_t *out);
    void read_ring(int slot, int row, int n_rows, float *out);
    void read_greedy_state(int slot, GreedyState *out);

    enum { SNAP_H = 0, SNAP_C = 1, SNAP_H16 = 2, SNAP_EOUT = 3, SNAP_DOUT = 4, SNAP_GSTATE = 5, SNAP_BIAS = 6, SNAP_VAD = 7, SNAP_RING = 8, SNAP_ARRAYS = 9 };
    struct SnapLayout {
        struct Arr { uint32_t layers = 0, row_bytes = 0, off = 0; } arr[SNAP_ARRAYS];
        uint32_t fixed = 0;
        uint32_t block_bytes(int ring_rows) const { return fixed + ((uint32_t)ring_rows * arr[SNAP_RING].row_bytes + 15u) / 16u * 16u; }
    };
    SnapLayout snapshot_layout() const;
    bool snapshot_gather(int n, SnapRec *recs, uint8_t *const *blocks_out);
    bool snapshot_scatter(int n, SnapRec *recs, const uint8_t *const *blocks);
    void snapshot_counts(uint64_t *gathers, uint64_t *scatters) const
    {
        *gathers = snap_gathers_.load(std::memory_order_relaxed); *scatters = snap_scatters_.load(std::memory_order_relaxed);
    }

    void set_profiling(bool on);
    void set_gates_clock(bool on);
    void gates_clock(double *ms, long *launches, long *rows) const { *ms = gclk_ms_; *launches = gclk_launches_; *rows = gclk_rows_; }
    void gates_clock_by_n(double *ms4, long *launches4) const { for (int i = 0; i < 4; ++i) { ms4[i] = gclk_ms_n_[i]; launches4[i] = gclk_launches_n_[i]; } }
    KernelTiming timing(int cls) const { return timing_[cls]; }
    void ramp_counts(uint64_t *hosted, uint64_t *eligible);
    void reset_timing();
    enum { T_GATES = 0, T_GEMM_OTHER = 1, T_ROW = 2, T_CONV = 3, T_FBANK = 4, T_DEC = 5, T_RESAMPLE = 6, T_DECODE = 7, T_VAD = 8, T_DTMF = 9, T_TONE = 10,
           T_SNAP_GATHER = 11, T_SNAP_SCATTER = 12, T_COUNT = 13 };
    long kernels_per_step() const { return kernels_per_step_.load(std::memory_order_relaxed); }

private:
    void upload_tables(const FbankHostTables &ft);
    void zero_slots(int n);
    void run_encoder_rows(int n, const float *x_direct);
    void encoder_front(size_t r0, int rows, const int *row_slots, const float *x_direct, hipStream_t st, float *ws);
    void lm_stage_layer(int l, int m, int t0, int t1, hipStream_t st);
    void lm_stage_proj(int m, int t0, int t1, hipStream_t st, float *ws);
    enum { GATES_ALL = 0xF, GATES_X = 0x3, GATES_H = 0xC };
    RowScale in_scale(int l, size_t r0) const;
    GemmArgs args_gates(int l, size_t r0, int rows, int waves) const;
    GemmArgs args_whr(int l, size_t r0, int rows) const;
    GemmArgs args_ff1(int l, size_t r0, int rows) const;
    GemmArgs args_ff2(int l, size_t r0, int rows) const;
    GemmArgs args_encproj(size_t r0, int rows, const int *slot_idx, float *out) const;
    AdvanceArgs advance_args(int m, int T) const;
    struct GreedyIo {
        int gen = 1;
        const int *now = nullptr;
        const float *eout = nullptr;
        const int *eout_rows = nullptr;
        const int *rec_off = nullptr; int rec_slot0 = 0;
        float *dump = nullptr;
    };
    void run_greedy_rounds(int n, bool dump_logits, int chunk = 0, const float *eout_rows = nullptr);
    void run_greedy_rounds(int n, const GreedyIo &io);
    void run_lm_chain(int m, int T, bool dump_logits);
    void run_lm_wavefront(int m, int T, bool dump_logits);
    struct SwPlan {
        struct Batch { size_t off; int n, macro, kind; size_t roff; int rn; };
        struct Chain { std::vector<GemmArgs> host; GemmArgs *dev = nullptr; std::vector<Batch> batches; std::vector<RowArgs> rhost; RowArgs *rdev = nullptr; };
        Chain one;
        Chain split;
        bool hosts = false;
        const Chain &layers(bool split_feed) const { return split_feed && !split.batches.empty() ? split : one; }
        std::vector<std::pair<int, long>> stamp_slots; std::vector<int> stamp_n;
    };
    GraphCache::Key graph_key(int m, int T = 0, int part = 0) const { return {m, T, flight_parity_ * 4 + part}; }
    GraphCache::Key sw_key(int m, int T, int part = 0) const { return graph_key(gclk_ ? -m : m, T, part); }
    SwPlan &sw_plan(int m, int T);
    void build_sw_chain(SwPlan &p, SwPlan::Chain &c, int m, int T, bool ramp);
    void free_sw_plans();
    void run_sw_chain(int m, int T, bool dump_logits, const SwPlan &p, int part, hipStream_t st);
    int stage_step(int m, int T, const int *slots, const int *ring_tails, const int *now_ms); void read_back_logits(int k, int rows, float *out);
    template <typename Chain> hipGraphExec_t cached_graph(GraphCache &cache, const GraphCache::Key &key, hipStream_t st, Chain &&chain);
    template <typename Capture> void capture_both_parities(Capture &&capture);
    void run_feed_wavefront(int m, int T, bool dump_logits); void run_layer_major(int m, int T, bool dump_logits); void launch_split_feed(int m, int T, hipStream_t fe);
    struct StreamTrace { hipEvent_t ev[6] = {nullptr, nullptr, nullptr, nullptr, nullptr, nullptr}; int m = 0, T = 0; bool used = false; };
    std::deque<StreamTrace> trace_; hipEvent_t trace_base_ = nullptr;
    StreamTrace *trace_slot();
    void dump_stream_trace();
    void select_parity(int p);
    void join(hipStream_t waiter, hipStream_t src);
    void general_prologue();
    int next_step_index() { ++flight_steps_; return (int)(step_seq_++ & (uint64_t)(2 * step_cap_ - 1)); }
    void launch_rowepi(GemmArgs fused_form, float *ws, hipStream_t st, bool force = false, int cls = T_GEMM_OTHER);
    bool gates_tile_rows(long rows) const;
    void run_decproj(int n, const int *d_slots, const int *row_mask, const int *run_flag, int run_gen, float *out = nullptr);
    void build_dec_table();
    void run_chain(int m, bool dump_logits);
    void collect_gates_clock();
    void timed_begin(int cls);
    void timed_end(int cls);
    void collect_timing();
    DecEmbedParams dec_params() const;

    EngineConfig cfg_;
    PackedLayout L_;
    ModelParams P_;
    hipStream_t stream_ = nullptr;
    float *w_ = nullptr;
    uint16_t *wh_ = nullptr;
    void lin(GemmArgs &g, size_t off) const { if (wh_) { g.wp = wh_ + off; g.wt = 1; } else { g.wp = w_ + off; g.wt = 0; } }
    bool f16_tile_ = false;
    uint16_t *wx_ = nullptr;
    uint16_t *y16_ = nullptr, *xb16_ = nullptr, *u16_ = nullptr, *ff16_ = nullptr;
    uint16_t *h16_ = nullptr;
    int kzx_hr_ = 1, kzx_ff2_ = 1;
    void lin16(GemmArgs &g, size_t off) const { g.wp = wx_ + off; g.wt = 1; g.tile_ok = 2; }
    int kz_hr() const { return f16_tile_ ? kzx_hr_ : kz_hr_; }
    int kz_ff2() const { return f16_tile_ ? kzx_ff2_ : kz_ff2_; }
    float *h_ = nullptr, *c_ = nullptr, *ring_ = nullptr, *eout_ = nullptr, *dout_ = nullptr;
    GreedyState *gstate_ = nullptr;
    float *dec_table_ = nullptr;
    uint8_t *cls_ = nullptr;
    int ring_frames_ = 0;
    float *xin_ = nullptr, *a3_ = nullptr, *y_ = nullptr, *ssq_ = nullptr, *xb_ = nullptr, *u_ = nullptr, *ff_ = nullptr, *ws_ = nullptr, *ws_g_ = nullptr, *de_ = nullptr;
    float *logits_ = nullptr;
    float *p_lm_ = nullptr, *eout_lm_ = nullptr;
    int *ring_h_ = nullptr; size_t ring_cap_ = 0, ring_pos_ = 0;
    int *step_off_h_ = nullptr, *rec_off_h_ = nullptr; int step_cap_ = 0;
    StepRecord *rec_d_ = nullptr, *rec_h_ = nullptr; size_t rec_cap_ = 0, rec_pos_ = 0;
    int flight_parity_ = 0, next_parity_ = 0; size_t ring_base_ = 0, rec_base_ = 0; int flight_steps_ = 0;
    uint64_t step_seq_ = 0;
    hipEvent_t flight_done_[2] = {nullptr, nullptr};
    SlotQueue<int> conf_q_; DeviceTable<uint8_t> conf_k_;
    ConfRecord *conf_d_ = nullptr, *conf_h_ = nullptr;
    std::vector<std::pair<size_t, size_t>> conf_spans_;
    std::atomic<uint64_t> conf_copied_{0};
    void apply_slot_tables();
    void drop_graphs();
    struct BiasEntry { std::shared_ptr<const BiasSet> set; int users = 0; void *dev = nullptr; };
    SlotQueue<int> bias_q_; DeviceTable<int32_t> bias_set_;
    std::vector<BiasEntry> bias_sets_;
    std::vector<int> bias_slot_set_;
    int32_t *bias_state_d_ = nullptr;
    DeviceTable<BiasDesc> bias_desc_;
    SlotQueue<SearchOpt> opt_q_; DeviceTable<SearchOpt> opt_;
    BiasDesc upload_bias(const BiasSet &set, void **dev, hipStream_t st);
    struct LmEntry { std::shared_ptr<const LmSet> set; int users = 0; void *dev = nullptr; };
    SlotQueue<LmSlot> lm_q_; DeviceTable<LmSlot> lm_slot_;
    std::vector<LmEntry> lm_models_;
    std::vector<int> lm_slot_model_;
    int32_t *lm_state_d_ = nullptr;
    DeviceTable<LmDesc> lm_desc_;
    std::atomic<uint64_t> lm_launches_{0}, lm_uploads_{0};
    std::atomic<int32_t> lm_resident_{0};
    LmDesc upload_lm(const LmSet &set, void **dev, hipStream_t st);
    void note_conf_step(int k, const int *slots, int m, size_t records);
    bool flight_open_[2] = {false, false};
    hipStream_t f_stream_ = nullptr, s_stream_ = nullptr, search_stream_ = nullptr;
    std::vector<hipEvent_t> join_ev_; size_t join_pos_ = 0;
    bool f_unseen_by_m_ = false, s_unseen_by_m_ = false, m_unseen_by_f_ = false, m_unseen_by_s_ = false, flight_tail_s_ = false;
    bool overlap_hint_ = false;
    int split_streams_ = 2;
    int ramp_mode_ = 1;
    RampState *ramp_d_ = nullptr;
    std::atomic<bool> m_quiet_{false};
    void m_touched() { m_quiet_.store(false, std::memory_order_release); }
    std::atomic<uint64_t> ramp_eligible_{0};
    float *xb_buf_[2] = {nullptr, nullptr}, *u_buf_[2] = {nullptr, nullptr}, *ff_buf_[2] = {nullptr, nullptr};
    uint16_t *xb16_buf_[2] = {nullptr, nullptr}, *u16_buf_[2] = {nullptr, nullptr}, *ff16_buf_[2] = {nullptr, nullptr};
    float *y_buf_[2] = {nullptr, nullptr}, *ssq_buf_[2] = {nullptr, nullptr}, *eout_lm_buf_[2] = {nullptr, nullptr}, *ws_fe_ = nullptr, *ws_sr_ = nullptr;
    uint16_t *y16_buf_[2] = {nullptr, nullptr};
    int *step_buf_[2] = {nullptr, nullptr}, *flags_buf_[2] = {nullptr, nullptr}, *rec_off_buf_[2] = {nullptr, nullptr};
    int *counter_d_ = nullptr, *step_d_ = nullptr, *active_d_ = nullptr, *dirty_d_ = nullptr, *rec_off_d_ = nullptr, *flags_d_ = nullptr;
    int *dec_slots_d_ = nullptr;
    float *logits_h_ = nullptr;
    int16_t *hs_pcm_[2] = {nullptr, nullptr}, *ds_pcm_[2] = {nullptr, nullptr};
    StagingCaps fb_caps_;
    int fb_flip_ = 0;
    hipEvent_t fb_done_[2] = {nullptr, nullptr};
    std::vector<size_t> part_off_;
    std::atomic<uint64_t> dc_launches_{0}, dc_frames_{0};
    VadState *vad_state_d_ = nullptr;
    uint8_t *pass_out_d_ = nullptr; size_t pass_out_cap_ = 0;
    struct PassBlock { uint8_t *h = nullptr; size_t cap = 0; bool busy = false; };
    std::vector<PassBlock> pass_blocks_;
    bool pass_bytes_flight_ = false;
    std::atomic<uint64_t> vad_launches_{0}, vad_frames_{0};
    const float *dt_tables_ = nullptr; int dt_wd_ = 0;
    std::atomic<uint64_t> dt_launches_{0}, dt_frames_{0};
    const float *dtmf_tables();
    const float *tn_tables_ = nullptr; int tn_w_ = 0, tn_f_ = 0;
    std::atomic<uint64_t> tn_launches_{0}, tn_frames_{0};
    const float *tone_tables();
    bool snapshot_copy(int n, SnapRec *recs, uint8_t *const *blocks, bool scatter);
    char *snap_d_ = nullptr, *snap_h_ = nullptr; size_t snap_cap_ = 0;
    std::atomic<uint64_t> snap_gathers_{0}, snap_scatters_{0};
    std::mutex rs_mu_;
    std::map<const ResampleSpec *, const float *> rs_tables_;
    const float *resample_table(const ResampleSpec *spec);
    FbankTables ft_;
    std::vector<void *> table_allocs_;
    float pad_value_ = 0;
    std::vector<int> free_, zero_pending_;
    void zero_pending_slots();
    std::atomic<int> live_{0};
    std::mutex slot_mu_;
    std::mutex capture_mu_;
    int kz_embed_ = 1, kz_hr_ = 1, kz_ff2_ = 1, kz_proj_ = 1, kz_out_ = 1;
    int ws_mstride_ = 0;
    float *conv_wt_ = nullptr;
    bool use_graphs_ = true;
    GraphCache step_graphs_{"chunk step", 256};
    GraphCache lm_graphs_{"layer-major chain", 32};
    GraphCache lm_search_graphs_{"long-feed search", 64};
    GraphCache sw_graphs_{"feed wavefront", 4 * 64};
    size_t sw_plan_cap_ = 64;
    std::map<GraphCache::Key, SwPlan> sw_plans_;
    hipStream_t lm_stream_ = nullptr;
    std::vector<hipEvent_t> lm_events_;
    GemmArgs *zargs_h_ = nullptr, *zargs_d_ = nullptr; size_t zargs_region_ = 0, zargs_pos_ = 0;
    hipEvent_t zargs_done_[3] = {nullptr, nullptr, nullptr}; bool zargs_busy_[3] = {false, false, false}; int zargs_next_ = 0;
    int *lm_now_d_ = nullptr, *lm_rows_d_ = nullptr, *lm_rec_off_d_ = nullptr;
    std::atomic<long> kernels_per_step_{0};
    long launch_count_ = 0;
    bool profiling_ = false;
    bool gclk_ = false, gclk_warned_ = false; unsigned long long *gclk_slots_ = nullptr; int gclk_used_ = 0;
    static constexpr int GCLK_SLOTS = 2048;
    double gclk_ms_ = 0; long gclk_launches_ = 0, gclk_rows_ = 0; double gclk_ms_n_[4] = {0, 0, 0, 0}; long gclk_launches_n_[4] = {0, 0, 0, 0};
    struct Ev { hipEvent_t a, b; int cls; };
    std::vector<Ev> ev_pool_; size_t ev_used_ = 0;
    KernelTiming timing_[T_COUNT];
};

}
```

### april_asr_amd/csrc/kernels.h

```cpp
#pragma once
#include <hip/hip_runtime.h>
#include <cstdint>
#include "vad.h"
#include "dtmf.h"
#include "tone.h"
#include "gemm_plan.h"

namespace aprilx {



constexpr int SSQ_COLS = 32;

struct RowScale {
    const float *ssq = nullptr;
    int groups = 0;
    float inv_n = 0.0f;
    float eps = 0.0f;
};

struct GreedyState { int32_t ctx0, ctx1; int32_t last_tok; uint32_t last_emit_ms; };

constexpr int STAMP_WORDS = 144, STAMP_ENDS = 8, STAMP_NENDS = 64, STAMP_SUBS = 72;

// ... 9 lines not shown
    int wt = 0;
    int M = 0, N = 0, K = 0;
    int kz = 1;
    int zs = 1;
    int mode = GM_SLAB;
    int epi = EPI_PARTIAL;
    float *out = nullptr; int ldo = 0;
    void *out16 = nullptr;
    void *state16 = nullptr;
    int m_stride = 0;
    const float *bias = nullptr;
    float *c_state = nullptr;
    const int *slot_idx = nullptr;
    int hidden = 0;
    float *state = nullptr; int ld_state = 0;
    const float *resid = nullptr; int ldr = 0;
    RowScale r_scale;
    float *ssq_out = nullptr;
    const int *row_mask = nullptr;
    const int *run_flag = nullptr;
    int run_gen = 1;
    int wave_mask = 0xF;
    const float *p_add = nullptr; int ldp = 0;
    int force_fullk = 0;
    int zcount = 1;
    int tile_ok = 0;
    int asm_loop = 0;
    unsigned long long *trace = nullptr;
    unsigned long long *stamp = nullptr;
    int debug = 0;
};
void launch_gemm(const GemmArgs &g, hipStream_t s);
void gemm_profile_next_launch(hipEvent_t start, hipEvent_t stop);
bool gemm_profile_pending();
void launch_gemm_tile(const GemmArgs &g, int mt, int nt, const GemmArgs *dev_args, int n, hipStream_t s);
int gemm_kw_waves(const GemmArgs &g);
bool gemm_pp_ok(const GemmArgs &g, int mt);
void launch_gemm_pp(const GemmArgs &g, int mt, const GemmArgs *dev_args, int n, hipStream_t s);
bool gemm_pw_ok(const GemmArgs &g);
void launch_gemm_pw(const GemmArgs &g, const GemmArgs *dev_args, int n, hipStream_t s);
void gemm_pp_pin(int enable, int mt);
void launch_gemm_kw(const GemmArgs &g, int mt, int nt, const GemmArgs *dev_args, int n, hipStream_t s);
void gemm_kw_pin(int enable, int mt);
int recur_form(const GemmArgs &g);
void launch_recur(const GemmArgs &g, int form, const GemmArgs *dev_args, int n, hipStream_t s);
void stage_gemm_z(const GemmArgs *items, int n, GemmArgs *staged);
void launch_gemm_z(const GemmArgs *staged, int n, const GemmArgs *dev_args, hipStream_t s);
GemmPlan gemm_plan(const GemmArgs &g);
GemmQuery gemm_query(const GemmArgs &g);
void gemm_tile_pin(int enable, int mt, int zs);

enum RowMode {
    ROW_HR = 0,
    ROW_RESID_SSQ = 1,
    ROW_SLOT_STORE = 2
};
struct RowArgs {
    int mode = ROW_HR;
    const float *ws = nullptr; int parts = 1; int m_stride = 0; int N = 0; int M = 0;
    const float *bias = nullptr;
    const float *resid = nullptr; int ldr = 0;
    RowScale r_scale;
    float *out = nullptr; int ldo = 0;
    const int *slot_idx = nullptr;
    float *state = nullptr; int ld_state = 0;
    float *ssq_out = nullptr;
    void *out16 = nullptr, *state16 = nullptr;
    const int *row_mask = nullptr;
    const int *run_flag = nullptr;
    int run_gen = 1;
};
void launch_row(const RowArgs &r, hipStream_t s);
void launch_row_z(const RowArgs *host_args, int n, const RowArgs *dev_args, hipStream_t s);

constexpr int RAMP_R = 2;
struct RampState {
    unsigned long long ready[2];
    int head_live[2];
    int guest_live[2][RAMP_R][RAMP_R];
    unsigned generation;
    unsigned hosted;
};
constexpr int RAMP_MAX_M = 0xFFFFF, RAMP_MAX_T = 0xFF;
void launch_ramp_ready(RampState *rs, int q, int m, int T, int hostable, hipStream_t s);
void launch_ramp_latch(RampState *rs, int p, int m, hipStream_t s);

struct StepRecord { int32_t idx; float max_val; float blank_val; uint32_t flags; };
constexpr int kConfMaxAlt = 8;
struct ConfRecord { float lse; float blank_val; int32_t n_alt; uint32_t reserved; int32_t alt_id[kConfMaxAlt]; float alt_logit[kConfMaxAlt]; };
static_assert(sizeof(ConfRecord) == 80, "ConfRecord is 20 x 32 bit");
enum { REC_VALID = 1, REC_BLANK = 2, REC_CTX = 4 };
enum TokClassBits { TKC_WORD_START = 1, TKC_SENT_END = 2, TKC_COMMA = 4, TKC_DOT = 8, TKC_DIGIT_START = 16 };

struct BiasDesc { const int32_t *state_off = nullptr, *edge_tok = nullptr, *edge_next = nullptr; const float *edge_bonus = nullptr; int32_t n_states = 0, flags = 0; };

struct SearchOpt { uint32_t endpoint_ms; float blank_penalty; };
static_assert(sizeof(SearchOpt) == 8, "SearchOpt is 2 x 32 bit");

struct LmDesc {
    const int32_t *node_off = nullptr, *back = nullptr, *arc_next = nullptr, *tok_off = nullptr;
    const float *bow = nullptr, *arc_logp = nullptr;
    const uint8_t *arc_byte = nullptr, *tok_bytes = nullptr;
    int32_t n_nodes = 0, start = 0; float unk_logp = 0.0f; int32_t reserved = 0;
};
struct LmSlot { int32_t model; float w, b; int32_t start; };
static_assert(sizeof(LmSlot) == 16, "LmSlot is 4 x 32 bit: one load");

struct DecEmbedParams {
    const float *emb = nullptr;
    const float *conv_w = nullptr;
    const float *conv_b = nullptr;
    int d = 0, groups = 0, context = 0, vocab = 0;
};

struct DecideArgs {
    const float *ws = nullptr; int parts = 1; int m_stride = 0; int N = 0; int M = 0;
    int n_valid = 0;
    const float *bias = nullptr;
    int blank = 0;
    float early_emit = 0.0f;
    const int *slot_idx = nullptr;
    const int *now_ms = nullptr;
    int *active = nullptr;
    int gen = 1;
    int rec_slot = 0;
    int *dirty = nullptr;
    const uint8_t *tok_class = nullptr;
    GreedyState *state = nullptr;
    StepRecord *rec = nullptr;
    StepRecord *rec_ring = nullptr;
    const int *rec_off = nullptr; int round = 0;
    float *logits_dump = nullptr;
    DecEmbedParams dec;
    float *de_out = nullptr; int ld_de = 0;
    int *run_flags = nullptr;
    int *rerun_flags = nullptr;
    const uint8_t *conf_k = nullptr;
    ConfRecord *conf_ring = nullptr;
    ConfRecord *conf = nullptr; int conf_k_all = 0;
    const int32_t *bias_set = nullptr;
    int32_t *bias_state = nullptr;
    const BiasDesc *bias_desc = nullptr;
    const SearchOpt *opt = nullptr;
    const LmSlot *lm_slot = nullptr;
    int32_t *lm_state = nullptr;
    const LmDesc *lm_desc = nullptr;
};
void launch_decide(const DecideArgs &a, hipStream_t s);

struct DecRowsArgs {
    const int *slot_idx = nullptr; int M = 0;
    int op = 0; int blank = 0;
    GreedyState *state = nullptr;
    DecEmbedParams dec;
    float *de_out = nullptr; int ld_de = 0;
    int32_t *bias_state = nullptr;
    const LmSlot *lm_slot = nullptr;
    int32_t *lm_state = nullptr;
};
void launch_dec_rows(const DecRowsArgs &a, hipStream_t s);

struct DecEmbedArgs {
    DecEmbedParams dec;
    const int *ctx = nullptr;
    int M = 0;
    float *out = nullptr; int ldo = 0;
};
void launch_dec_embed(const DecEmbedArgs &a, hipStream_t s);
// ... 181 lines not shown
```

### april_asr_amd/csrc/kernels_misc.hip

```cpp
#include "kernels.h"
#include "device_utils.h"
#include "env.h"
#include <algorithm>
#include <cstdio>
#include <cstdlib>
#include <type_traits>

namespace aprilx {

template <int MODE>
__device__ __forceinline__ void row_body(const RowArgs &r)
{
    if (r.run_flag && *r.run_flag != r.run_gen) return;
    const int m = blockIdx.x;
    const int tid = threadIdx.x;
    const int slot = r.slot_idx ? r.slot_idx[m] : m;
    if (MODE == ROW_SLOT_STORE) { if (r.row_mask && !r.row_mask[m]) return; }
    float rs = 1.0f;
    const bool scaled = MODE == ROW_HR || (MODE == ROW_SLOT_STORE && r.r_scale.ssq != nullptr);
    if (scaled) rs = row_scale(r.r_scale, m);
    const int nq = r.N >> 2;
    for (int q0 = 0; q0 < nq; q0 += 256) {
        const int q = q0 + tid;
        const bool ok = q < nq;
        const int n = q * 4;
        f32x4 s = f32x4{0.f, 0.f, 0.f, 0.f};
        if (ok) s = tree_sum4(r.ws, r.parts, r.m_stride, r.N, m, n);
        if (MODE == ROW_HR) {
            if (ok) {
                const HrTail t = hr_tail(s, *reinterpret_cast<const f32x4 *>(r.resid + (size_t)m * r.ldr + n), rs);
                *reinterpret_cast<f32x4 *>(r.state + (size_t)slot * r.ld_state + n) = t.state;
                *reinterpret_cast<f32x4 *>(r.out + (size_t)m * r.ldo + n) = t.out;
                if (r.state16) *reinterpret_cast<h4 *>(reinterpret_cast<_Float16 *>(r.state16) + (size_t)slot * r.ld_state + n) = to_h4(t.state);
                if (r.out16) *reinterpret_cast<h4 *>(reinterpret_cast<_Float16 *>(r.out16) + (size_t)m * r.ldo + n) = to_h4(t.out);
            }
        } else if (MODE == ROW_RESID_SSQ) {
            f32x4 y = f32x4{0.f, 0.f, 0.f, 0.f};
            if (ok) {
                const f32x4 res = r.resid ? *reinterpret_cast<const f32x4 *>(r.resid + (size_t)m * r.ldr + n) : f32x4{0.f, 0.f, 0.f, 0.f};
                y = resid_tail(s, *reinterpret_cast<const f32x4 *>(r.bias + n), res, r.resid != nullptr);
                *reinterpret_cast<f32x4 *>(r.out + (size_t)m * r.ldo + n) = y;
                if (r.out16) *reinterpret_cast<h4 *>(reinterpret_cast<_Float16 *>(r.out16) + (size_t)m * r.ldo + n) = to_h4(y);
            }
            float ss;
            if (granule_ssq_store(y, ok, q, ss)) r.ssq_out[(size_t)m * (r.N / SSQ_COLS) + n / SSQ_COLS] = ss;
        } else {
            if (ok) {
                const f32x4 b = *reinterpret_cast<const f32x4 *>(r.bias + n);
                *reinterpret_cast<f32x4 *>(r.out + (size_t)slot * r.ldo + n) = scaled ? slot_value(s, rs, b) : slot_value(s, b);
            }
        }
    }
}

template <int MODE>
__global__ __launch_bounds__(256) void row_kernel(RowArgs r) { row_body<MODE>(r); }

template <int MODE>
__global__ __launch_bounds__(256) void row_zkernel(const RowArgs *__restrict__ zargs)
{
    const RowArgs r = zargs[blockIdx.y];
    row_body<MODE>(r);
}

void launch_row(const RowArgs &r, hipStream_t s)
{
    dim3 grid((unsigned)r.M), block(256);
    switch (r.mode) {
    case ROW_HR: hipLaunchKernelGGL(row_kernel<ROW_HR>, grid, block, 0, s, r); break;
    case ROW_RESID_SSQ: hipLaunchKernelGGL(row_kernel<ROW_RESID_SSQ>, grid, block, 0, s, r); break;
    default: hipLaunchKernelGGL(row_kernel<ROW_SLOT_STORE>, grid, block, 0, s, r); break;
    }
}

void launch_row_z(const RowArgs *host_args, int n, const RowArgs *dev_args, hipStream_t s)
{
    if (n <= 0) return;
    const RowArgs &r = host_args[0];
    for (int i = 1; i < n; ++i)
        if (host_args[i].mode != r.mode || host_args[i].M != r.M || host_args[i].N != r.N || host_args[i].parts != r.parts) {
            fprintf(stderr, "libapril(mi355x): launch_row_z: the problems of one launch must have one shape\n"); abort();
        }
    dim3 grid((unsigned)r.M, (unsigned)n), block(256);
    switch (r.mode) {
    case ROW_HR: hipLaunchKernelGGL(row_zkernel<ROW_HR>, grid, block, 0, s, dev_args); break;
    case ROW_RESID_SSQ: hipLaunchKernelGGL(row_zkernel<ROW_RESID_SSQ>, grid, block, 0, s, dev_args); break;
    default: hipLaunchKernelGGL(row_zkernel<ROW_SLOT_STORE>, grid, block, 0, s, dev_args); break;
    }
}

__global__ __launch_bounds__(64) void ramp_ready_kernel(RampState *rs, int q, int m, int T, int hostable)
{
    if (threadIdx.x != 0) return;
    __hip_atomic_store(&rs->head_live[q], 1, __ATOMIC_RELAXED, __HIP_MEMORY_SCOPE_AGENT);
    const unsigned g = __hip_atomic_load(&rs->generation, __ATOMIC_RELAXED, __HIP_MEMORY_SCOPE_AGENT) + 1u;
    __hip_atomic_store(&rs->generation, g, __ATOMIC_RELAXED, __HIP_MEMORY_SCOPE_AGENT);
    __builtin_amdgcn_fence(__ATOMIC_RELEASE, "agent");
    asm volatile("s_waitcnt vmcnt(0)" ::: "memory");
    const unsigned long long rec = ((unsigned long long)g << 32) | ((unsigned long long)(unsigned)m << 12) | ((unsigned long long)(unsigned)T << 4) | (unsigned long long)(hostable & 1);
    __hip_atomic_store(&rs->ready[q], rec, __ATOMIC_RELAXED, __HIP_MEMORY_SCOPE_AGENT);
}

__global__ __launch_bounds__(64) void ramp_latch_kernel(RampState *rs, int p, int m)
{
    if (threadIdx.x != 0) return;
    const unsigned long long mine = __hip_atomic_load(&rs->ready[p], __ATOMIC_RELAXED, __HIP_MEMORY_SCOPE_AGENT);
    const unsigned long long next = __hip_atomic_load(&rs->ready[1 - p], __ATOMIC_RELAXED, __HIP_MEMORY_SCOPE_AGENT);
    const unsigned g = (unsigned)(mine >> 32);
    const int next_m = (int)((next >> 12) & RAMP_MAX_M), next_T = (int)((next >> 4) & RAMP_MAX_T);
    const bool host = (unsigned)(next >> 32) == g + 1u && next_m == m && (int)((mine >> 12) & RAMP_MAX_M) == m && (next & 1ull) != 0;
    if (host) {
        __builtin_amdgcn_fence(__ATOMIC_ACQUIRE, "agent");
        __hip_atomic_store(&rs->head_live[1 - p], 0, __ATOMIC_RELAXED, __HIP_MEMORY_SCOPE_AGENT);
        rs->hosted += 1u;
    }
    for (int j = 1; j <= RAMP_R; ++j)
        for (int t = 0; t < RAMP_R; ++t) rs->guest_live[p][j - 1][t] = (host && t < j && t < next_T) ? 1 : 0;
}

void launch_ramp_ready(RampState *rs, int q, int m, int T, int hostable, hipStream_t s)
{
    hipLaunchKernelGGL(ramp_ready_kernel, dim3(1), dim3(64), 0, s, rs, q, m, T, hostable);
}
void launch_ramp_latch(RampState *rs, int p, int m, hipStream_t s)
{
    hipLaunchKernelGGL(ramp_latch_kernel, dim3(1), dim3(64), 0, s, rs, p, m);
}

__device__ __forceinline__ void dec_embed_row(const DecEmbedParams &p, int tok0, int tok1, float *out)
{
    const int cg = p.d / p.groups;
    for (int o = threadIdx.x; o < p.d; o += 256) {
        const int g0 = (o / cg) * cg;
        const float *w = p.conv_w + (size_t)o * cg * p.context;
        float acc = 0.0f;
        for (int ci = 0; ci < cg; ++ci) {
            acc += p.emb[(size_t)tok0 * p.d + g0 + ci] * w[ci * p.context + 0];
            acc += p.emb[(size_t)tok1 * p.d + g0 + ci] * w[ci * p.context + 1];
        }
        if (p.conv_b) acc += p.conv_b[o];
        out[o] = acc > 0.0f ? acc : 0.0f;
    }
}

#include "kernels_bias.inc"
#include "kernels_lm.inc"
#include "kernels_confidence.inc"

template <bool CONF, bool BIAS, bool OPT, bool LM = false>
__device__ __forceinline__ void decide_body(const DecideArgs &a)
{
    extern __shared__ __attribute__((aligned(16))) unsigned char bias_lds[];
    __shared__ float s_best[4], s_blank[4];
    __shared__ int s_idx[4];
    __shared__ int s_ctx[3];
    if (a.round > 0 && a.run_flags && a.run_flags[a.round] != a.gen) return;
    const int m = blockIdx.x;
    const int tid = threadIdx.x;
    StepRecord *rec = a.rec ? a.rec + m : a.rec_ring + (size_t)a.rec_off[0] + (size_t)a.rec_slot * a.M + m;
    if (a.round > 0 && a.active[m] != a.gen) {
        if (tid == 0) { rec->idx = -1; rec->max_val = 0.0f; rec->blank_val = 0.0f; rec->flags = 0; a.dirty[m] = 0; }
        return;
    }
    float best = -9999999999.0f;
    int best_i = -1;
    float blank_v = 0.0f;
    BiasRow br;
    if (BIAS) bias_row_begin(a, m, bias_lds, br);
    typename std::conditional<LM, LmRow, LmNoRow>::type lr;
    if constexpr (LM) lm_row_begin(a, m, bias_lds, br, lr);
    if (BIAS && br.bonus) bias_scan(a, m, br, best, best_i, blank_v);
    else
    for (int n = tid; n < a.n_valid; n += 256) {
        const float v = tree_sum(a.ws, a.parts, a.m_stride, a.N, m, n) + a.bias[n];
        if (a.logits_dump) a.logits_dump[(size_t)m * a.n_valid + n] = v;
        if (n == a.blank) blank_v = v;
        else if (v > best) { best = v; best_i = n; }
    }
#pragma unroll
    for (int off = 32; off > 0; off >>= 1) {
        const float ov = __shfl_xor(best, off);
        const int oi = __shfl_xor(best_i, off);
        const bool take = (oi >= 0) && (best_i < 0 || ov > best || (ov == best && oi < best_i));
        if (take) { best = ov; best_i = oi; }
        blank_v += __shfl_xor(blank_v, off);
    }
    const int wave = tid >> 6;
    if ((tid & 63) == 0) { s_best[wave] = best; s_idx[wave] = best_i; s_blank[wave] = blank_v; }
    __syncthreads();
    if (tid == 0) {
        float b = s_best[0]; int bi = s_idx[0];
        for (int w = 1; w < 4; ++w) {
            const float ov = s_best[w]; const int oi = s_idx[w];
            if (oi >= 0 && (bi < 0 || ov > b || (ov == b && oi < bi))) { b = ov; bi = oi; }
        }
        float bl = s_blank[(a.blank & 255) >> 6];
        rec->idx = bi; rec->max_val = b; rec->blank_val = bl;

        const int slot = a.slot_idx[m];
        GreedyState st = a.state[slot];
        SearchOpt so; so.endpoint_ms = 0u; so.blank_penalty = 0.0f;
        if (OPT) { so = a.opt[slot]; if (so.endpoint_ms) bl = bl - so.blank_penalty; }
        int tok = bi; float tv = b;
        if (tok < 0) { tok = a.blank == 0 ? 1 : 0; tv = -9999999999.0f; }
        const bool cleared = st.ctx1 == a.blank;
        const bool same = st.ctx1 == tok;
        const float ee = same ? 0.0f : a.early_emit;
        bool is_blank = (bl - ee) > tv;
        const unsigned tc = a.tok_class[tok];
// ... 449 lines not shown
```

### april_asr_amd/csrc/ramp_api.cc

```cpp
#include <vector>
#include "../../include/april_api.h"
#include "../../include/aprilx_engine.h"
#include "common.h"
#include "session.h"
#include "api_handles.h"

using namespace aprilx;

extern "C" {

int aprilx_ramp_window(int L, int T, int R, int32_t *out, int cap)
{
    if (L <= 0 || T <= 0 || R <= 0 || !out) return -1;
    const std::vector<RampStep> w = ramp_window(L, T, R);
    const int stride = 3 + 2 * R;
    if ((int)w.size() * stride > cap) return -1;
    for (size_t i = 0; i < w.size(); ++i) {
        int32_t *o = out + i * (size_t)stride;
        for (int k = 0; k < stride; ++k) o[k] = -1;
        o[0] = w[i].macro; o[1] = w[i].own; o[2] = (int32_t)w[i].guests.size();
        for (size_t g = 0; g < w[i].guests.size() && (int)g < R; ++g) { o[3 + 2 * g] = w[i].guests[g].first; o[4 + 2 * g] = w[i].guests[g].second; }
    }
    return (int)w.size();
}
int aprilx_model_ramp_stats(AprilASRModel model, int device_index, uint64_t *ramp_hosted, uint64_t *ramp_eligible)
{
    if (!model || device_index < 0 || device_index >= (int)model->m.engines.size() || !ramp_hosted || !ramp_eligible) return -1;
    model->m.engines[(size_t)device_index]->ramp_counts(ramp_hosted, ramp_eligible);
    return 0;
}

}
```

### include/aprilx_engine.h

```cpp
#ifndef APRILX_ENGINE_H
#define APRILX_ENGINE_H
#include "april_api.h"

#ifdef __cplusplus
extern "C" {
#endif

typedef struct AprilxDims {
    int32_t n_layers, d_model, hidden, ffn, joiner, vocab, mel, seg, seg_step, context;
    int32_t fft_size, frame_shift, sample_rate, blank_id, n_devices;
    int32_t precision;
    int32_t d_model_file;
    int64_t param_count;
} AprilxDims;
APRIL_EXPORT int aprilx_model_dims(AprilASRModel model, AprilxDims *out);
APRIL_EXPORT const char *aprilx_model_token(AprilASRModel model, int32_t id);

typedef struct AprilxLoadInfo {
    double broadcast_ms;
    double comm_init_ms;
    uint64_t broadcast_bytes;
    int32_t ranks;
    int32_t used_rccl;
} AprilxLoadInfo;
// ... 186 lines not shown
    float min_share;
    uint32_t tol_hz;
    uint32_t min_tone_ms, min_pause_ms;
    uint32_t flags;
} AprilxToneOptions;
enum { APRILX_TONE_ON = 1, APRILX_TONE_OFF = 2 };
typedef void (*AprilxToneHandler)(void *userdata, int kind, uint32_t f1_hz, uint32_t f2_hz, uint64_t time_ms);
typedef struct AprilxToneInfo {
    int32_t W, k_lo, F, on_frames, off_frames;
    uint32_t held_f1, held_f2;
    uint32_t reserved;
    uint64_t frames_seen;
    uint64_t tonal_frames;
    uint64_t tones;
} AprilxToneInfo;
typedef struct AprilxTonePlan {
    int32_t W, k_lo, F; float half_w, min_power, second_ratio, min_share, bin_hz; int32_t tol_hz, on_frames, off_frames, reserved;
} AprilxTonePlan;
typedef struct AprilxToneMachine { int32_t held, h1, h2, c1, c2, run; } AprilxToneMachine;
APRIL_EXPORT int aprilx_session_set_tones(AprilASRSession session, const AprilxToneOptions *options, AprilxToneHandler handler, void *userdata);
APRIL_EXPORT int aprilx_session_tones(AprilASRSession session, AprilxToneOptions *options_out, AprilxToneInfo *out);
APRIL_EXPORT int aprilx_tone_plan(int sample_rate, int fft_size, int frame_shift_ms, const AprilxToneOptions *options, AprilxTonePlan *plan_out);
APRIL_EXPORT int aprilx_tone_tables(int sample_rate, int fft_size, float *out, size_t cap);
APRIL_EXPORT int aprilx_tone_host(const AprilxTonePlan *plan, const float *tables, int n, const int16_t *frames, size_t ld, uint16_t *records_out,
                                  float *powers_out);
APRIL_EXPORT int64_t aprilx_tone_decide_host(const AprilxTonePlan *plan, const float *powers);
APRIL_EXPORT int aprilx_tone_events_host(const AprilxTonePlan *plan, int frame_shift_ms, uint64_t t0, const uint16_t *records, size_t n, int flush,
                                         AprilxToneMachine *machine, int32_t *kinds_out, uint32_t *f1_out, uint32_t *f2_out, uint64_t *times_out, int cap);
APRIL_EXPORT const char *aprilx_tone_name(uint32_t f1_hz, uint32_t f2_hz, uint32_t tol_hz);
APRIL_EXPORT int aprilx_run_tones(AprilASRModel model, const AprilxToneOptions *options, int n_runs, const int32_t *n, const int16_t *frames,
                                  uint16_t *records_out, float *powers_out);
APRIL_EXPORT int aprilx_run_tone_decide(AprilASRModel model, const AprilxToneOptions *options, int n, const float *powers, uint16_t *records_out);
APRIL_EXPORT int aprilx_model_tone_stats(AprilASRModel model, int device_index, uint64_t *launches, uint64_t *frames, double *ms);

typedef struct AprilxSnapshotInfo {
    uint32_t size;
    uint32_t version;
    uint64_t blob_size;
    uint64_t params_hash;
    uint64_t token_hash;
    uint64_t bias_hash;
    int64_t bias_edges;
    uint64_t chunks, frames_seen, now_ms, rows_written;
    int32_t n_layers, d_model, hidden, ffn, joiner, vocab, mel, segment_size, segment_step, sample_rate, frame_shift_ms, blank_id;
    uint32_t precision;
    uint32_t f16_tile;
    uint32_t input_rate;
    uint32_t confidence_k;
    uint32_t has_format, has_search_options, has_vad, has_dtmf, has_tones, has_bias;
    uint32_t bias_flags; int32_t bias_states;
    uint32_t ring_rows;
    uint32_t reserved;
    AprilxInputFormat format;
    AprilxSearchOptions search;
    AprilxVadOptions vad;
    AprilxDtmfOptions dtmf;
    AprilxToneOptions tones;
    char name[64], description[128];
} AprilxSnapshotInfo;
APRIL_EXPORT int64_t aprilx_session_snapshot(AprilASRSession session, void *dst, size_t cap);
APRIL_EXPORT int aprilx_session_restore(AprilASRSession session, const void *blob, size_t size, char *err, size_t err_cap);
APRIL_EXPORT int aprilx_snapshot_info(const void *blob, size_t size, AprilxSnapshotInfo *out);
APRIL_EXPORT int aprilx_snapshot_many(size_t n, AprilASRSession *sessions, void *const *dsts, const size_t *caps, int64_t *sizes_out);
APRIL_EXPORT int aprilx_restore_many(size_t n, AprilASRSession *sessions, const void *const *blobs, const size_t *sizes, int *status_out);
APRIL_EXPORT int aprilx_model_snapshot_stats(AprilASRModel model, int device_index, uint64_t *gathers, uint64_t *scatters, double *gather_ms, double *scatter_ms);

typedef struct AprilxStats {
    uint64_t ticks, steps, chunks, rounds, frames, max_batch_seen;
    double kernel_ms[6];
    uint64_t kernel_launches[6];
    double host_ms[8];
    uint64_t flights;
    uint64_t replay_mismatch;
    uint64_t kernels_per_step;
    uint64_t lm_steps, lm_chunks;
    uint64_t wave_steps, wave_chunks;
    double gates_clock_ms; uint64_t gates_clock_launches, gates_clock_rows;
    double gates_clock_ms_by_n[4]; uint64_t gates_clock_launches_by_n[4];
    double resample_ms; uint64_t resample_launches;
    uint64_t confidence_records;
} AprilxStats;
APRIL_EXPORT void aprilx_model_stats(AprilASRModel model, int device_index, AprilxStats *out);
APRIL_EXPORT int aprilx_model_ramp_stats(AprilASRModel model, int device_index, uint64_t *ramp_hosted, uint64_t *ramp_eligible);
APRIL_EXPORT int aprilx_model_feed_latency(AprilASRModel model, int device_index, double *out_ms, int cap, int reset);
APRIL_EXPORT void aprilx_model_profile(AprilASRModel model, int enable);

typedef struct AprilxGreedy_i *AprilxGreedy;
APRIL_EXPORT AprilxGreedy aprilx_greedy_create(AprilASRModel model, AprilRecognitionResultHandler handler, void *userdata);
APRIL_EXPORT int aprilx_greedy_step(AprilxGreedy g, int32_t idx, float max_val, float blank_val, float early_emit,
                                    size_t now_ms, int32_t *ctx_out);
APRIL_EXPORT void aprilx_greedy_finish(AprilxGreedy g);
APRIL_EXPORT void aprilx_greedy_free(AprilxGreedy g);
APRIL_EXPORT int aprilx_greedy_set_bias(AprilxGreedy g, AprilxBias bias);
APRIL_EXPORT int aprilx_greedy_bias_state(AprilxGreedy g);
APRIL_EXPORT int aprilx_greedy_set_search_options(AprilxGreedy g, const AprilxSearchOptions *options);
APRIL_EXPORT int aprilx_greedy_set_lm(AprilxGreedy g, AprilxLm lm, float weight, float token_bonus);
APRIL_EXPORT int aprilx_greedy_lm_state(AprilxGreedy g);

APRIL_EXPORT void aprilx_counting_handler(void *userdata, AprilResultType type, size_t count, const AprilToken *tokens);

APRIL_EXPORT AprilASRModel aprilx_model_load_host(const char *model_path);
APRIL_EXPORT int aprilx_model_fbank_tables(AprilASRModel model, float *window, float *mel);

APRIL_EXPORT int aprilx_probe_file(const char *path, char *err, size_t err_cap);

#ifdef __cplusplus
}
#endif
#endif
```

Baseline: 20030.

## Defer split-feed layer graph until ramp latch reports, launch headless variant when hosted

In ramp mode 1, the layer-wavefront graph of a split feed is no longer enqueued right away. The host waits for the predecessor's latch kernel to write its outcome to a coherent pinned host word. If the predecessor already hosted the ramp head, a prebuilt headless layer chain is launched that skips the first RAMP_R+1 wavefront steps, so no guard-flag predicated GEMMs are needed. Otherwise the full chain is launched. This removes the device-side head_live guarding and redundant head work, but adds host spin-waiting, a mutex, extra graph variants and settle calls on many paths, which can stall host enqueueing.

```diff
diff --git a/april_asr_amd/__init__.py b/april_asr_amd/__init__.py
--- a/april_asr_amd/__init__.py
+++ b/april_asr_amd/__init__.py
@@ -456,6 +456,12 @@
         if self._L.aprilx_model_ramp_stats(self._handle, device_index, C.byref(h), C.byref(e)) != 0:
             raise ValueError("aprilx_model_ramp_stats refused the call")
         return int(h.value), int(e.value)
+
+    def ramp_stats2(self, device_index: int = 0):
+        out = (C.c_uint64 * 5)()
+        if self._L.aprilx_model_ramp_stats2(self._handle, device_index, out) != 0:
+            raise ValueError("aprilx_model_ramp_stats2 refused the call")
+        return dict(zip(("hosted", "eligible", "headless", "settled_wait", "settled_other"), (int(v) for v in out)))
 
     def feed_latencies(self, device_index: int = 0, reset: bool = False) -> np.ndarray:
         n = int(self._L.aprilx_model_feed_latency(self._handle, device_index, None, 0, 0))
diff --git a/april_asr_amd/_ffi.py b/april_asr_amd/_ffi.py
--- a/april_asr_amd/_ffi.py
+++ b/april_asr_amd/_ffi.py
@@ -156,7 +156,7 @@
     "aprilx_run_decide_biased", "aprilx_greedy_set_bias", "aprilx_greedy_bias_state",
     "aprilx_bias_create_ex", "aprilx_bias_flags", "aprilx_run_confidence_biased",
     "aprilx_session_set_search_options", "aprilx_session_search_options", "aprilx_run_decide_opts", "aprilx_greedy_set_search_options",
-    "aprilx_ramp_window", "aprilx_model_ramp_stats",
+    "aprilx_ramp_window", "aprilx_model_ramp_stats", "aprilx_model_ramp_stats2",
     "aprilx_session_set_input_format", "aprilx_session_input_format", "aprilx_session_feed_bytes", "aprilx_feed_many_bytes",
     "aprilx_decode_host", "aprilx_decode", "aprilx_model_decode_stats",
     "aprilx_session_set_vad", "aprilx_session_vad", "aprilx_vad_plan_tables", "aprilx_vad_host", "aprilx_vad_events_host", "aprilx_run_vad",
@@ -219,6 +219,7 @@
     L.aprilx_run_gemm.argtypes = [vp] * 5; L.aprilx_run_gemm.restype = C.c_int
     L.aprilx_ramp_window.argtypes = [C.c_int] * 3 + [vp, C.c_int]; L.aprilx_ramp_window.restype = C.c_int
     L.aprilx_model_ramp_stats.argtypes = [vp, C.c_int, C.POINTER(C.c_uint64), C.POINTER(C.c_uint64)]; L.aprilx_model_ramp_stats.restype = C.c_int
+    L.aprilx_model_ramp_stats2.argtypes = [vp, C.c_int, C.POINTER(C.c_uint64)]; L.aprilx_model_ramp_stats2.restype = C.c_int
     L.aprilx_stream_form.argtypes = [C.c_int] * 6; L.aprilx_stream_form.restype = C.c_int
     L.aprilx_run_decide.argtypes = [vp, C.c_int, C.c_int, vp, C.c_float, vp, C.c_int, vp, vp]; L.aprilx_run_decide.restype = C.c_int
     L.aprilx_session_trace_logits.argtypes = [vp, vp, sz, C.POINTER(sz)]; L.aprilx_session_trace_logits.restype = None
diff --git a/april_asr_amd/csrc/engine.cc b/april_asr_amd/csrc/engine.cc
--- a/april_asr_amd/csrc/engine.cc
+++ b/april_asr_amd/csrc/engine.cc
@@ -5,6 +5,7 @@
 #include <chrono>
 #include <cstdlib>
 #include <cstring>
+#include <thread>
 #include "common.h"
 #include "env.h"
 #include "rowepi_forms.h"
@@ -259,8 +260,12 @@
     for (int p = 0; p < 2; ++p) { xb_buf_[p] = dmalloc<float>(MB * d.d_model); u_buf_[p] = dmalloc<float>(MB * d.hidden); ff_buf_[p] = dmalloc<float>(MB * d.ffn); }
     xb_ = xb_buf_[0]; u_ = u_buf_[0]; ff_ = ff_buf_[0];
     ramp_mode_ = env_int("APRIL_RAMP_MERGE", 1);
-    if (ramp_mode_ < 0 || ramp_mode_ > 2) ramp_mode_ = 1;
+    if (ramp_mode_ < 0 || ramp_mode_ > 3) ramp_mode_ = 1;
     ramp_d_ = dmalloc<RampState>(1); HIP_CHECK(hipMemset(ramp_d_, 0, sizeof(RampState)));
+    if (ramp_mode_ == 1) {
+        HipLegacyLock legacy;
+        HIP_CHECK(hipHostMalloc((void **)&ramp_word_h_, sizeof *ramp_word_h_, hipHostMallocCoherent)); *ramp_word_h_ = 0;
+    }
     de_ = dmalloc<float>(MB * d.d_model);
     HIP_CHECK(hipMemset(de_, 0, MB * d.d_model * 4));
     logits_ = dmalloc<float>(3 * MB * d.vocab);
@@ -282,7 +287,7 @@
     upload_tables(ft);
     use_graphs_ = env_int("APRIL_NO_GRAPHS", 0) == 0;
     if (const int n = env_int("APRIL_GRAPH_CACHE_CAP", 0))
-        step_graphs_.cap = lm_graphs_.cap = lm_search_graphs_.cap = sw_plan_cap_ = (size_t)std::max(n, 2), sw_graphs_.cap = 4 * sw_plan_cap_;
+        step_graphs_.cap = lm_graphs_.cap = lm_search_graphs_.cap = sw_plan_cap_ = (size_t)std::max(n, 2), sw_graphs_.cap = 5 * sw_plan_cap_;
     free_.reserve(S);
     for (int i = cfg_.max_slots - 1; i >= 0; --i) free_.push_back(i);
     LOGI("engine: device %d, %d slots, max batch %d, weights %.1f MB, kz(embed,hr,ff2,proj,out)=%d,%d,%d,%d,%d",
@@ -348,11 +353,14 @@
 {
     HipLegacyLock legacy;
     (void)hipSetDevice(cfg_.device);
+    settle_pending_layers(true, RampDefer::BY_OTHER);
     (void)hipStreamSynchronize(f_stream_); (void)hipStreamSynchronize(stream_); (void)hipStreamSynchronize(s_stream_);
     dump_stream_trace();
     if (ramp_d_ && ramp_eligible_.load() > 0) {
         unsigned h = 0;
         if (hipMemcpy(&h, &ramp_d_->hosted, sizeof h, hipMemcpyDeviceToHost) == hipSuccess) LOGI("engine: ramp merge: %u of %llu hostable split feeds were hosted by their predecessor", h, (unsigned long long)ramp_eligible_.load());
+        if (defer_.deferred) LOGI("engine: ramp merge: %llu layer graphs deferred, %llu launched headless; settled by the flight wait %llu, by another entry %llu", (unsigned long long)defer_.deferred,
+                                  (unsigned long long)defer_.headless, (unsigned long long)defer_.settled_by[RampDefer::BY_WAIT], (unsigned long long)defer_.settled_by[RampDefer::BY_OTHER]);
     }
     for (StreamTrace &t : trace_) for (hipEvent_t e : t.ev) if (e) (void)hipEventDestroy(e);
     if (trace_base_) (void)hipEventDestroy(trace_base_);
@@ -385,6 +393,7 @@
                         (void *)xb16_buf_[p], (void *)u16_buf_[p], (void *)ff16_buf_[p], (void *)rec_off_buf_[p], (void *)flags_buf_[p], (void *)step_buf_[p]}) if (q) (void)hipFree(q);
     if (ws_fe_) (void)hipFree(ws_fe_);
     if (ws_sr_) (void)hipFree(ws_sr_);
+    if (ramp_word_h_) (void)hipHostFree(ramp_word_h_);
     for (void *p : {(void *)wx_, (void *)h16_, (void *)ramp_d_}) if (p) (void)hipFree(p);
     for (void *p : {(void *)w_, (void *)wh_, (void *)h_, (void *)c_, (void *)ring_, (void *)eout_, (void *)dout_, (void *)gstate_, (void *)cls_, (void *)ws_, (void *)xin_,
                     (void *)a3_, (void *)de_, (void *)logits_, (void *)rec_d_, (void *)counter_d_,
@@ -464,6 +473,7 @@
 
 void Engine::sync_streams()
 {
+    settle_pending_layers(true, RampDefer::BY_OTHER);
     HIP_CHECK(hipStreamSynchronize(f_stream_)); HIP_CHECK(hipStreamSynchronize(stream_)); HIP_CHECK(hipStreamSynchronize(s_stream_));
 }
 
@@ -527,7 +537,7 @@
     FILE *f = fopen(path, "w");
     if (!f) return;
     fprintf(f, "# one line per split feed; times in us since the first split feed; FE = index fetch + conv + embed on stream F, LY = layer wavefront on M, SR = encoder_proj + search on S\n");
-    fprintf(f, "# feed sessions chunks  FE_start FE_end  LY_start LY_end  SR_start SR_end   overlap: FE inside the previous feed's LY window? SR inside the next feed's LY window?\n");
+    fprintf(f, "# feed sessions chunks  FE_start FE_end  LY_start LY_end  SR_start SR_end   overlap: FE inside the previous feed's LY window? SR inside the next feed's LY window?  LY flavour: headless / head\n");
     std::vector<std::array<float, 6>> ts;
     for (StreamTrace &t : trace_) {
         std::array<float, 6> a{};
@@ -539,8 +549,8 @@
         const auto &a = ts[i];
         const bool fe_in_prev = i > 0 && a[0] * 1e3f < ts[i - 1][3] * 1e3f && a[1] * 1e3f > ts[i - 1][2] * 1e3f;
         const bool sr_in_next = i + 1 < ts.size() && a[5] > ts[i + 1][2] && a[4] < ts[i + 1][3];
-        fprintf(f, "%4zu %5d %2d  %10.1f %10.1f  %10.1f %10.1f  %10.1f %10.1f   %s %s\n", i, trace_[i].m, trace_[i].T, a[0] * 1e3, a[1] * 1e3, a[2] * 1e3, a[3] * 1e3, a[4] * 1e3, a[5] * 1e3,
-                fe_in_prev ? "FE<prevLY" : "-", sr_in_next ? "SR<nextLY" : "-");
+        fprintf(f, "%4zu %5d %2d  %10.1f %10.1f  %10.1f %10.1f  %10.1f %10.1f   %s %s %s\n", i, trace_[i].m, trace_[i].T, a[0] * 1e3, a[1] * 1e3, a[2] * 1e3, a[3] * 1e3, a[4] * 1e3, a[5] * 1e3,
+                fe_in_prev ? "FE<prevLY" : "-", sr_in_next ? "SR<nextLY" : "-", trace_[i].headless ? "headless" : "head");
     }
     fclose(f);
 }
@@ -1237,6 +1247,7 @@
     SwPlan &p = sw_plans_[key];
     build_sw_chain(p, p.one, m, T, false);
     if (ramp_mode_ != 0 && !gclk_) build_sw_chain(p, p.split, m, T, true);
+    if (ramp_mode_ == 1 && !gclk_ && L_.dims.n_layers > 2 * RAMP_R) build_sw_chain(p, p.headless, m, T, true, true);
     return p;
 }
 
@@ -1264,8 +1275,9 @@
     *hosted = h; *eligible = ramp_eligible_.load(std::memory_order_relaxed);
 }
 
-void Engine::build_sw_chain(SwPlan &p, SwPlan::Chain &c, int m, int T, bool ramp)
-{
+void Engine::build_sw_chain(SwPlan &p, SwPlan::Chain &c, int m, int T, bool ramp, bool headless)
+{
+    const bool guard = ramp && ramp_mode_ != 1;
     const NetDims &d = L_.dims;
     const int L = d.n_layers;
     const int par = flight_parity_;
@@ -1284,7 +1296,7 @@
     if (ramp) p.hosts = !window.empty();
     std::vector<GemmArgs> items;
     std::vector<RowArgs> rows;
-    for (int W = 0; W <= T + L; ++W) {
+    for (int W = headless ? RAMP_R + 1 : 0; W <= T + L; ++W) {
         const RampStep *host = nullptr; int wj = 0;
         for (size_t j = 0; j < window.size(); ++j) if (window[j].macro == W) { host = &window[j]; wj = (int)j; }
         if (host && wj == 0) { SwPlan::Batch b; b.off = c.host.size(); b.n = 0; b.macro = W; b.kind = 4; b.roff = c.rhost.size(); b.rn = 0; c.batches.push_back(b); }
@@ -1311,7 +1323,7 @@
             for (int l = 0; l < L; ++l) {
                 const int t = W - 1 - l;
                 if (t < 0 || t >= T) continue;
-                problem(l, t, ramp && W <= RAMP_R ? &ramp_d_->head_live[par] : nullptr);
+                problem(l, t, guard && W <= RAMP_R ? &ramp_d_->head_live[par] : nullptr);
             }
             if (host) {
                 select_parity(1 - par);
@@ -1356,7 +1368,7 @@
 void Engine::free_sw_plans()
 {
     if (!sw_plans_.empty()) LOGI("engine: feed wavefront plans emptied (%zu plans)", sw_plans_.size());
-    for (auto &p : sw_plans_) for (SwPlan::Chain *c : {&p.second.one, &p.second.split}) { if (c->dev) (void)hipFree(c->dev); if (c->rdev) (void)hipFree(c->rdev); }
+    for (auto &p : sw_plans_) for (SwPlan::Chain *c : {&p.second.one, &p.second.split, &p.second.headless}) { if (c->dev) (void)hipFree(c->dev); if (c->rdev) (void)hipFree(c->rdev); }
     sw_graphs_.clear(); sw_plans_.clear();
 }
 
@@ -1368,12 +1380,12 @@
         launch_advance(advance_args(m, T), st);
         encoder_front(0, m * T, step_d_ + 3 * MB, nullptr, st, part == 0 ? ws_fe_ : ws_);
     }
-    if (part < 0 || part == 1) {
+    if (part < 0 || part == 1 || part == 3) {
         static const int cls_of[4] = {T_GATES, T_GEMM_OTHER, T_GEMM_OTHER, T_GEMM_OTHER};
-        const SwPlan::Chain &c = p.layers(part == 1);
+        const SwPlan::Chain &c = part == 3 ? p.headless : p.layers(part == 1);
         for (size_t bi = 0; bi < c.batches.size(); ++bi) {
             const SwPlan::Batch &b = c.batches[bi];
-            if (b.kind == 4) { launch_ramp_latch(ramp_d_, flight_parity_, m, st); continue; }
+            if (b.kind == 4) { launch_ramp_latch(ramp_d_, flight_parity_, m, ramp_word_h_, ramp_mode_ != 1 ? 1 : 0, st); continue; }
             timed_begin(cls_of[b.kind]); launch_gemm_z(c.host.data() + b.off, b.n, c.dev + b.off, st); timed_end(cls_of[b.kind]);
             if (b.rn > 0) { timed_begin(T_ROW); launch_row_z(c.rhost.data() + b.roff, b.rn, c.rdev + b.roff, st); timed_end(T_ROW); }
         }
@@ -1421,8 +1433,10 @@
     if (graphs && !sw_graphs_.find(sw_key(m, T, split ? 1 : 0)))
         capture_both_parities([&]() {
             const SwPlan &pl = sw_plan(m, T);
-            if (split) for (int part = 0; part < 3; ++part) cached_graph(sw_graphs_, sw_key(m, T, 1 + part), on[part], [&]() { run_sw_chain(m, T, false, pl, part, on[part]); });
-            else cached_graph(sw_graphs_, sw_key(m, T), stream_, [&]() { run_sw_chain(m, T, false, pl, -1, stream_); });
+            if (split) {
+                for (int part = 0; part < 3; ++part) cached_graph(sw_graphs_, sw_key(m, T, 1 + part), on[part], [&]() { run_sw_chain(m, T, false, pl, part, on[part]); });
+                if (!pl.headless.batches.empty()) cached_graph(sw_graphs_, sw_key(m, T, 4), on[1], [&]() { run_sw_chain(m, T, false, pl, 3, on[1]); });
+            } else cached_graph(sw_graphs_, sw_key(m, T), stream_, [&]() { run_sw_chain(m, T, false, pl, -1, stream_); });
         });
     if (split) { launch_split_feed(m, T, on[0]); return; }
     general_prologue();
@@ -1432,29 +1446,103 @@
 
 void Engine::launch_split_feed(int m, int T, hipStream_t fe)
 {
+    settle_pending_layers(true, RampDefer::BY_OTHER);
     if (fe == f_stream_) {
         if (m_unseen_by_f_) { join(f_stream_, stream_); m_unseen_by_f_ = false; }
     } else if (f_unseen_by_m_) { join(stream_, f_stream_); f_unseen_by_m_ = false; }
     if (m_unseen_by_s_) { join(s_stream_, stream_); m_unseen_by_s_ = false; }
-    StreamTrace *tr = trace_slot();
-    auto part = [&](int i, hipStream_t st) {
-        if (tr) HIP_CHECK(hipEventRecord(tr->ev[2 * i], st));
-        HIP_CHECK(hipGraphLaunch(sw_graphs_.find(sw_key(m, T, 1 + i)), st));
-        if (tr) HIP_CHECK(hipEventRecord(tr->ev[2 * i + 1], st));
+    PendingFeed pf;
+    pf.m = m; pf.T = T; pf.parity = flight_parity_; pf.tr = trace_slot(); pf.hosts = sw_plan(m, T).hosts;
+    if (pf.tr) HIP_CHECK(hipEventRecord(pf.tr->ev[0], fe));
+    HIP_CHECK(hipGraphLaunch(sw_graphs_.find(sw_key(m, T, 1)), fe));
+    if (pf.tr) HIP_CHECK(hipEventRecord(pf.tr->ev[1], fe));
+    bool offered = false;
+    if (ramp_mode_ != 0) {
+        const bool quiet = fe == f_stream_ && m_quiet_.load(std::memory_order_acquire);
+        offered = ramp_mode_ == 3 ? quiet : ramp_mode_ == 1 && quiet && m_tail_latch_;
+        if (offered) ramp_eligible_.fetch_add(1, std::memory_order_relaxed);
+        launch_ramp_ready(ramp_d_, flight_parity_, m, T, offered ? 1 : 0, ramp_mode_ != 1 ? 1 : 0, fe);
+        ++ramp_gen_h_;
+    }
+    if (fe == f_stream_) {
+        pf.fe_done = join_ev_[join_pos_++ % join_ev_.size()];
+        HIP_CHECK(hipEventRecord(pf.fe_done, f_stream_));
+    } else m_unseen_by_f_ = true;
+    std::lock_guard<std::mutex> g(defer_mu_);
+    const bool defer = ramp_mode_ == 1 && offered;
+    if (defer) pend_ = pf;
+    const uint64_t word = ramp_word_h_ ? __atomic_load_n(ramp_word_h_, __ATOMIC_ACQUIRE) : 0;
+    const bool open = defer_.launch(ramp_gen_h_, defer, word, [&](RampDefer::Flavour f) { enqueue_split_layers(pf, f == RampDefer::HEADLESS); });
+    defer_open_.store(open, std::memory_order_release);
+}
+
+void Engine::enqueue_split_layers(const PendingFeed &f, bool headless)
+{
+    StreamTrace *tr = f.tr;
+    auto graph = [&](int part) {
+        const hipGraphExec_t g = sw_graphs_.find(GraphCache::Key{f.m, f.T, f.parity * 8 + part});
+        if (!g) { LOGE("engine: split feed %d x %d, parity %d: graph %d is missing", f.m, f.T, f.parity, part); abort(); }
+        return g;
     };
-    part(0, fe);
-    if (ramp_mode_ != 0) {
-        const bool hostable = ramp_mode_ == 1 && fe == f_stream_ && m_quiet_.load(std::memory_order_acquire);
-        if (hostable) ramp_eligible_.fetch_add(1, std::memory_order_relaxed);
-        launch_ramp_ready(ramp_d_, flight_parity_, m, T, hostable ? 1 : 0, fe);
-    }
-    if (fe == f_stream_) { join(stream_, f_stream_); f_unseen_by_m_ = false; }
-    part(1, stream_);
-    if (ramp_mode_ != 0) m_quiet_.store(true, std::memory_order_release);
-    join(s_stream_, stream_); part(2, s_stream_);
-    if (tr) { tr->m = m; tr->T = T; tr->used = true; }
+    if (f.fe_done) { HIP_CHECK(hipStreamWaitEvent(stream_, f.fe_done, 0)); f_unseen_by_m_ = false; }
+    if (tr) HIP_CHECK(hipEventRecord(tr->ev[2], stream_));
+    HIP_CHECK(hipGraphLaunch(graph(headless ? 4 : 2), stream_));
+    if (tr) HIP_CHECK(hipEventRecord(tr->ev[3], stream_));
+    if (ramp_mode_ != 0) { m_tail_latch_ = f.hosts; m_quiet_.store(true, std::memory_order_release); }
+    join(s_stream_, stream_);
+    if (tr) HIP_CHECK(hipEventRecord(tr->ev[4], s_stream_));
+    HIP_CHECK(hipGraphLaunch(graph(3), s_stream_));
+    if (tr) { HIP_CHECK(hipEventRecord(tr->ev[5], s_stream_)); tr->m = f.m; tr->T = f.T; tr->headless = headless; tr->used = true; }
     s_unseen_by_m_ = true; flight_tail_s_ = true;
-    if (fe != f_stream_) m_unseen_by_f_ = true;
+    if (f.closed) {
+        if (f.pass_bytes) join(s_stream_, f_stream_);
+        enqueue_flight_tail(s_stream_, f.parity, f.rec_base, f.rec_pos, f.conf_spans);
+    }
+}
+
+static inline void cpu_relax()
+{
+#if defined(__x86_64__) || defined(__i386__)
+    __builtin_ia32_pause();
+#else
+    std::this_thread::yield();
+#endif
+}
+
+bool Engine::settle_pending_layers(bool wait, RampDefer::Who who)
+{
+    if (!defer_open_.load(std::memory_order_acquire)) return true;
+    std::lock_guard<std::mutex> g(defer_mu_);
+    if (!defer_.pending()) return true;
+    (void)hipSetDevice(cfg_.device);
+    bool m_idle = false;
+    for (unsigned spins = 0;; ++spins) {
+        const uint64_t word = __atomic_load_n(ramp_word_h_, __ATOMIC_ACQUIRE);
+        if (defer_.poll(word, who, [&](RampDefer::Flavour f) { enqueue_split_layers(pend_, f == RampDefer::HEADLESS); })) {
+            pend_ = PendingFeed();
+            defer_open_.store(false, std::memory_order_release);
+            return true;
+        }
+        if (!wait) return false;
+        if (m_idle) { LOGE("engine: the layer stream is idle and no latch reported generation %u (word %llx)", defer_.wanted(), (unsigned long long)word); abort(); }
+        if ((spins & 1023u) == 1023u) {
+            const hipError_t e = hipStreamQuery(stream_);
+            if (e == hipSuccess) m_idle = true; else if (e != hipErrorNotReady) HIP_CHECK(e); else (void)hipGetLastError();
+        }
+        for (int i = 0; i < 16; ++i) cpu_relax();
+    }
+}
+
+bool Engine::deferred_flight(int parity)
+{
+    std::lock_guard<std::mutex> g(defer_mu_);
+    return defer_.pending() && pend_.closed && pend_.parity == parity;
+}
+
+void Engine::ramp_defer_counts(uint64_t *headless, uint64_t *by_wait, uint64_t *by_other)
+{
+    std::lock_guard<std::mutex> g(defer_mu_);
+    *headless = defer_.headless; *by_wait = defer_.settled_by[RampDefer::BY_WAIT]; *by_other = defer_.settled_by[RampDefer::BY_OTHER];
 }
 
 void Engine::run_layer_major(int m, int T, bool dump_logits)
@@ -1687,6 +1775,7 @@
 void Engine::begin_flight()
 {
     HIP_CHECK(hipSetDevice(cfg_.device));
+    settle_pending_layers(true, RampDefer::BY_OTHER);
     const int p = flight_parity_ = next_parity_; next_parity_ ^= 1;
     if (flight_open_[p]) { HIP_CHECK(hipEventSynchronize(flight_done_[p])); flight_open_[p] = false; }
     if (conf_q_.has_pending() || bias_q_.has_pending() || opt_q_.has_pending() || lm_q_.has_pending()) apply_slot_tables();
@@ -1751,6 +1840,16 @@
 {
     HIP_CHECK(hipSetDevice(cfg_.device));
     std::lock_guard<std::mutex> cg(capture_mu_);
+    settle_pending_layers(false, RampDefer::BY_OTHER);
+    {
+        std::lock_guard<std::mutex> g(defer_mu_);
+        if (defer_.pending()) {
+            pend_.closed = true; pend_.pass_bytes = pass_bytes_flight_; pend_.rec_base = rec_base_; pend_.rec_pos = rec_pos_; pend_.conf_spans.swap(conf_spans_);
+            pass_bytes_flight_ = false; conf_spans_.clear();
+            flight_open_[flight_parity_] = true;
+            return flight_parity_;
+        }
+    }
     hipStream_t tail = s_stream_;
     if (!(flight_tail_s_ && s_unseen_by_m_)) {
         tail = stream_;
@@ -1758,19 +1857,25 @@
         if (s_unseen_by_m_) { join(stream_, s_stream_); s_unseen_by_m_ = false; }
     } else if (pass_bytes_flight_) join(s_stream_, f_stream_);
     pass_bytes_flight_ = false;
-    if (rec_pos_ > rec_base_) HIP_CHECK(hipMemcpyAsync(rec_h_ + rec_base_, rec_d_ + rec_base_, (rec_pos_ - rec_base_) * sizeof(StepRecord), hipMemcpyDeviceToHost, tail));
-    for (const auto &sp : conf_spans_) {
+    enqueue_flight_tail(tail, flight_parity_, rec_base_, rec_pos_, conf_spans_);
+    conf_spans_.clear();
+    flight_open_[flight_parity_] = true;
+    return flight_parity_;
+}
+
+void Engine::enqueue_flight_tail(hipStream_t tail, int parity, size_t rec_base, size_t rec_pos, const std::vector<std::pair<size_t, size_t>> &conf_spans)
+{
+    if (rec_pos > rec_base) HIP_CHECK(hipMemcpyAsync(rec_h_ + rec_base, rec_d_ + rec_base, (rec_pos - rec_base) * sizeof(StepRecord), hipMemcpyDeviceToHost, tail));
+    for (const auto &sp : conf_spans) {
         HIP_CHECK(hipMemcpyAsync(conf_h_ + sp.first, conf_d_ + sp.first, sp.second * sizeof(ConfRecord), hipMemcpyDeviceToHost, tail));
         conf_copied_.fetch_add(sp.second, std::memory_order_relaxed);
     }
-    conf_spans_.clear();
-    HIP_CHECK(hipEventRecord(flight_done_[flight_parity_], tail));
-    flight_open_[flight_parity_] = true;
-    return flight_parity_;
+    HIP_CHECK(hipEventRecord(flight_done_[parity], tail));
 }
 
 bool Engine::flight_done(int parity)
 {
+    if (!settle_pending_layers(false, RampDefer::BY_WAIT) && deferred_flight(parity)) return false;
     const hipError_t e = hipEventQuery(flight_done_[parity]);
     if (e == hipSuccess) return true;
     if (e != hipErrorNotReady) HIP_CHECK(e);
@@ -1781,6 +1886,14 @@
 void Engine::wait_flight(int parity)
 {
     HIP_CHECK(hipSetDevice(cfg_.device));
+    while (!settle_pending_layers(false, RampDefer::BY_WAIT)) {
+        if (deferred_flight(parity)) { settle_pending_layers(true, RampDefer::BY_WAIT); break; }
+        const hipError_t e = hipEventQuery(flight_done_[parity]);
+        if (e == hipSuccess) break;
+        if (e != hipErrorNotReady) HIP_CHECK(e);
+        (void)hipGetLastError();
+        for (int i = 0; i < 16; ++i) cpu_relax();
+    }
     HIP_CHECK(hipEventSynchronize(flight_done_[parity]));
     if (profiling_) sync();
 }
diff --git a/april_asr_amd/csrc/engine.h b/april_asr_amd/csrc/engine.h
--- a/april_asr_amd/csrc/engine.h
+++ b/april_asr_amd/csrc/engine.h
@@ -18,6 +18,7 @@
 #include "input_format.h"
 #include "kernels.h"
 #include "host_pool.h"
+#include "ramp_defer.h"
 #include "slot_queue.h"
 #include "staging_layout.h"
 #include "model_loader.h"
@@ -259,6 +260,7 @@
     void gates_clock_by_n(double *ms4, long *launches4) const { for (int i = 0; i < 4; ++i) { ms4[i] = gclk_ms_n_[i]; launches4[i] = gclk_launches_n_[i]; } }
     KernelTiming timing(int cls) const { return timing_[cls]; }
     void ramp_counts(uint64_t *hosted, uint64_t *eligible);
+    void ramp_defer_counts(uint64_t *headless, uint64_t *by_wait, uint64_t *by_other);
     void reset_timing();
     enum { T_GATES = 0, T_GEMM_OTHER = 1, T_ROW = 2, T_CONV = 3, T_FBANK = 4, T_DEC = 5, T_RESAMPLE = 6, T_DECODE = 7, T_VAD = 8, T_DTMF = 9, T_TONE = 10,
            T_SNAP_GATHER = 11, T_SNAP_SCATTER = 12, T_COUNT = 13 };
@@ -296,21 +298,22 @@
         struct Chain { std::vector<GemmArgs> host; GemmArgs *dev = nullptr; std::vector<Batch> batches; std::vector<RowArgs> rhost; RowArgs *rdev = nullptr; };
         Chain one;
         Chain split;
+        Chain headless;
         bool hosts = false;
         const Chain &layers(bool split_feed) const { return split_feed && !split.batches.empty() ? split : one; }
         std::vector<std::pair<int, long>> stamp_slots; std::vector<int> stamp_n;
     };
-    GraphCache::Key graph_key(int m, int T = 0, int part = 0) const { return {m, T, flight_parity_ * 4 + part}; }
+    GraphCache::Key graph_key(int m, int T = 0, int part = 0) const { return {m, T, flight_parity_ * 8 + part}; }
     GraphCache::Key sw_key(int m, int T, int part = 0) const { return graph_key(gclk_ ? -m : m, T, part); }
     SwPlan &sw_plan(int m, int T);
-    void build_sw_chain(SwPlan &p, SwPlan::Chain &c, int m, int T, bool ramp);
+    void build_sw_chain(SwPlan &p, SwPlan::Chain &c, int m, int T, bool ramp, bool headless = false);
     void free_sw_plans();
     void run_sw_chain(int m, int T, bool dump_logits, const SwPlan &p, int part, hipStream_t st);
     int stage_step(int m, int T, const int *slots, const int *ring_tails, const int *now_ms); void read_back_logits(int k, int rows, float *out);
     template <typename Chain> hipGraphExec_t cached_graph(GraphCache &cache, const GraphCache::Key &key, hipStream_t st, Chain &&chain);
     template <typename Capture> void capture_both_parities(Capture &&capture);
     void run_feed_wavefront(int m, int T, bool dump_logits); void run_layer_major(int m, int T, bool dump_logits); void launch_split_feed(int m, int T, hipStream_t fe);
-    struct StreamTrace { hipEvent_t ev[6] = {nullptr, nullptr, nullptr, nullptr, nullptr, nullptr}; int m = 0, T = 0; bool used = false; };
+    struct StreamTrace { hipEvent_t ev[6] = {nullptr, nullptr, nullptr, nullptr, nullptr, nullptr}; int m = 0, T = 0; bool used = false, headless = false; };
     std::deque<StreamTrace> trace_; hipEvent_t trace_base_ = nullptr;
     StreamTrace *trace_slot();
     void dump_stream_trace();
@@ -391,7 +394,19 @@
     int ramp_mode_ = 1;
     RampState *ramp_d_ = nullptr;
     std::atomic<bool> m_quiet_{false};
-    void m_touched() { m_quiet_.store(false, std::memory_order_release); }
+    void m_touched() { settle_pending_layers(true, RampDefer::BY_OTHER); m_quiet_.store(false, std::memory_order_release); }
+    struct PendingFeed {
+        int m = 0, T = 0, parity = 0; hipEvent_t fe_done = nullptr; StreamTrace *tr = nullptr; bool hosts = false;
+        bool closed = false, pass_bytes = false; size_t rec_base = 0, rec_pos = 0; std::vector<std::pair<size_t, size_t>> conf_spans;
+    };
+    RampDefer defer_; PendingFeed pend_; std::mutex defer_mu_; std::atomic<bool> defer_open_{false};
+    unsigned long long *ramp_word_h_ = nullptr;
+    uint32_t ramp_gen_h_ = 0;
+    bool m_tail_latch_ = false;
+    bool settle_pending_layers(bool wait, RampDefer::Who who);
+    bool deferred_flight(int parity);
+    void enqueue_split_layers(const PendingFeed &f, bool headless);
+    void enqueue_flight_tail(hipStream_t tail, int parity, size_t rec_base, size_t rec_pos, const std::vector<std::pair<size_t, size_t>> &conf_spans);
     std::atomic<uint64_t> ramp_eligible_{0};
     float *xb_buf_[2] = {nullptr, nullptr}, *u_buf_[2] = {nullptr, nullptr}, *ff_buf_[2] = {nullptr, nullptr};
     uint16_t *xb16_buf_[2] = {nullptr, nullptr}, *u16_buf_[2] = {nullptr, nullptr}, *ff16_buf_[2] = {nullptr, nullptr};
@@ -440,7 +455,7 @@
     GraphCache step_graphs_{"chunk step", 256};
     GraphCache lm_graphs_{"layer-major chain", 32};
     GraphCache lm_search_graphs_{"long-feed search", 64};
-    GraphCache sw_graphs_{"feed wavefront", 4 * 64};
+    GraphCache sw_graphs_{"feed wavefront", 5 * 64};
     size_t sw_plan_cap_ = 64;
     std::map<GraphCache::Key, SwPlan> sw_plans_;
     hipStream_t lm_stream_ = nullptr;
diff --git a/april_asr_amd/csrc/kernels.h b/april_asr_amd/csrc/kernels.h
--- a/april_asr_amd/csrc/kernels.h
+++ b/april_asr_amd/csrc/kernels.h
@@ -115,8 +115,8 @@
     unsigned hosted;
 };
 constexpr int RAMP_MAX_M = 0xFFFFF, RAMP_MAX_T = 0xFF;
-void launch_ramp_ready(RampState *rs, int q, int m, int T, int hostable, hipStream_t s);
-void launch_ramp_latch(RampState *rs, int p, int m, hipStream_t s);
+void launch_ramp_ready(RampState *rs, int q, int m, int T, int hostable, int guard, hipStream_t s);
+void launch_ramp_latch(RampState *rs, int p, int m, unsigned long long *report, int guard, hipStream_t s);
 
 struct StepRecord { int32_t idx; float max_val; float blank_val; uint32_t flags; };
 constexpr int kConfMaxAlt = 8;
diff --git a/april_asr_amd/csrc/kernels_misc.hip b/april_asr_amd/csrc/kernels_misc.hip
--- a/april_asr_amd/csrc/kernels_misc.hip
+++ b/april_asr_amd/csrc/kernels_misc.hip
@@ -89,10 +89,10 @@
     }
 }
 
-__global__ __launch_bounds__(64) void ramp_ready_kernel(RampState *rs, int q, int m, int T, int hostable)
+__global__ __launch_bounds__(64) void ramp_ready_kernel(RampState *rs, int q, int m, int T, int hostable, int guard)
 {
     if (threadIdx.x != 0) return;
-    __hip_atomic_store(&rs->head_live[q], 1, __ATOMIC_RELAXED, __HIP_MEMORY_SCOPE_AGENT);
+    if (guard) __hip_atomic_store(&rs->head_live[q], 1, __ATOMIC_RELAXED, __HIP_MEMORY_SCOPE_AGENT);
     const unsigned g = __hip_atomic_load(&rs->generation, __ATOMIC_RELAXED, __HIP_MEMORY_SCOPE_AGENT) + 1u;
     __hip_atomic_store(&rs->generation, g, __ATOMIC_RELAXED, __HIP_MEMORY_SCOPE_AGENT);
     __builtin_amdgcn_fence(__ATOMIC_RELEASE, "agent");
@@ -101,7 +101,7 @@
     __hip_atomic_store(&rs->ready[q], rec, __ATOMIC_RELAXED, __HIP_MEMORY_SCOPE_AGENT);
 }
 
-__global__ __launch_bounds__(64) void ramp_latch_kernel(RampState *rs, int p, int m)
+__global__ __launch_bounds__(64) void ramp_latch_kernel(RampState *rs, int p, int m, unsigned long long *report, int guard)
 {
     if (threadIdx.x != 0) return;
     const unsigned long long mine = __hip_atomic_load(&rs->ready[p], __ATOMIC_RELAXED, __HIP_MEMORY_SCOPE_AGENT);
@@ -111,20 +111,21 @@
     const bool host = (unsigned)(next >> 32) == g + 1u && next_m == m && (int)((mine >> 12) & RAMP_MAX_M) == m && (next & 1ull) != 0;
     if (host) {
         __builtin_amdgcn_fence(__ATOMIC_ACQUIRE, "agent");
-        __hip_atomic_store(&rs->head_live[1 - p], 0, __ATOMIC_RELAXED, __HIP_MEMORY_SCOPE_AGENT);
+        if (guard) __hip_atomic_store(&rs->head_live[1 - p], 0, __ATOMIC_RELAXED, __HIP_MEMORY_SCOPE_AGENT);
         rs->hosted += 1u;
     }
     for (int j = 1; j <= RAMP_R; ++j)
         for (int t = 0; t < RAMP_R; ++t) rs->guest_live[p][j - 1][t] = (host && t < j && t < next_T) ? 1 : 0;
-}
-
-void launch_ramp_ready(RampState *rs, int q, int m, int T, int hostable, hipStream_t s)
-{
-    hipLaunchKernelGGL(ramp_ready_kernel, dim3(1), dim3(64), 0, s, rs, q, m, T, hostable);
-}
-void launch_ramp_latch(RampState *rs, int p, int m, hipStream_t s)
-{
-    hipLaunchKernelGGL(ramp_latch_kernel, dim3(1), dim3(64), 0, s, rs, p, m);
+    if (report) __hip_atomic_store(report, ((unsigned long long)(g + 1u) << 32) | (host ? 1ull : 0ull), __ATOMIC_RELEASE, __HIP_MEMORY_SCOPE_SYSTEM);
+}
+
+void launch_ramp_ready(RampState *rs, int q, int m, int T, int hostable, int guard, hipStream_t s)
+{
+    hipLaunchKernelGGL(ramp_ready_kernel, dim3(1), dim3(64), 0, s, rs, q, m, T, hostable, guard);
+}
+void launch_ramp_latch(RampState *rs, int p, int m, unsigned long long *report, int guard, hipStream_t s)
+{
+    hipLaunchKernelGGL(ramp_latch_kernel, dim3(1), dim3(64), 0, s, rs, p, m, report, guard);
 }
 
 __device__ __forceinline__ void dec_embed_row(const DecEmbedParams &p, int tok0, int tok1, float *out)
diff --git a/april_asr_amd/csrc/ramp_api.cc b/april_asr_amd/csrc/ramp_api.cc
--- a/april_asr_amd/csrc/ramp_api.cc
+++ b/april_asr_amd/csrc/ramp_api.cc
@@ -29,5 +29,12 @@
     model->m.engines[(size_t)device_index]->ramp_counts(ramp_hosted, ramp_eligible);
     return 0;
 }
+int aprilx_model_ramp_stats2(AprilASRModel model, int device_index, uint64_t out[5])
+{
+    if (!model || device_index < 0 || device_index >= (int)model->m.engines.size() || !out) return -1;
+    model->m.engines[(size_t)device_index]->ramp_counts(&out[0], &out[1]);
+    model->m.engines[(size_t)device_index]->ramp_defer_counts(&out[2], &out[3], &out[4]);
+    return 0;
+}
 
 }
diff --git a/april_asr_amd/csrc/ramp_defer.h b/april_asr_amd/csrc/ramp_defer.h
--- /dev/null
+++ b/april_asr_amd/csrc/ramp_defer.h
@@ -0,0 +1,41 @@
+#pragma once
+#include <cstdint>
+
+namespace aprilx {
+
+inline uint64_t ramp_outcome_word(uint32_t generation, bool hosted) { return ((uint64_t)generation << 32) | (hosted ? 1u : 0u); }
+
+struct RampDefer {
+    enum Flavour { WITH_HEAD = 0, HEADLESS = 1 };
+    enum Who { BY_WAIT = 0, BY_OTHER = 1 };
+
+    bool pending() const { return pending_; }
+    uint32_t wanted() const { return want_; }
+    uint64_t deferred = 0, headless = 0, settled_by[2] = {0, 0};
+
+    template <typename Enqueue> bool launch(uint32_t gen, bool latch_in_front, uint64_t word_now, Enqueue &&enqueue)
+    {
+        if (pending_) return true;
+        if (!latch_in_front) { enqueue(WITH_HEAD); return false; }
+        pending_ = true; want_ = gen; ++deferred;
+        return !poll(word_now, BY_OTHER, enqueue);
+    }
+
+    template <typename Enqueue> bool poll(uint64_t word_now, Who who, Enqueue &&enqueue)
+    {
+        if (!pending_) return true;
+        if ((uint32_t)(word_now >> 32) != want_) return false;
+        pending_ = false;
+        const Flavour f = (word_now & 1u) ? HEADLESS : WITH_HEAD;
+        if (f == HEADLESS) ++headless;
+        ++settled_by[who];
+        enqueue(f);
+        return true;
+    }
+
+private:
+    bool pending_ = false;
+    uint32_t want_ = 0;
+};
+
+}
diff --git a/include/aprilx_engine.h b/include/aprilx_engine.h
--- a/include/aprilx_engine.h
+++ b/include/aprilx_engine.h
@@ -292,6 +292,7 @@
 } AprilxStats;
 APRIL_EXPORT void aprilx_model_stats(AprilASRModel model, int device_index, AprilxStats *out);
 APRIL_EXPORT int aprilx_model_ramp_stats(AprilASRModel model, int device_index, uint64_t *ramp_hosted, uint64_t *ramp_eligible);
+APRIL_EXPORT int aprilx_model_ramp_stats2(AprilASRModel model, int device_index, uint64_t out[5]);
 APRIL_EXPORT int aprilx_model_feed_latency(AprilASRModel model, int device_index, double *out_ms, int cap, int reset);
 APRIL_EXPORT void aprilx_model_profile(AprilASRModel model, int enable);
 
```

New measurement: 20510 (median of 6 runs). 2.4% higher.
